# fritzsedlazeck/Sniffles

Hardware: NVIDIA H100
Metric: aligned long-read Gbp/s through lead->cluster->consensus (higher is better)
Workload: dtype int32

## Files before the change

### sniffles_b200/csrc/api.cu

```cuda
#include <algorithm>
#include <climits>
#include <cstdio>
#include <cstdlib>
#include <cstring>
#include <string>
#include <vector>
#include <dlfcn.h>
#include <omp.h>

#include "common.cuh"
#include "prims.cuh"
#include "extract.cuh"
#include "cluster.cuh"
#include "consensus.cuh"
#include "poa.cuh"
#include "combine.cuh"
#include "ingest.cuh"
#include "bgzf_write.cuh"
#include "genotype.cuh"
#include "reference.cuh"

template <bool Pinned> struct Buf {
    void* p = nullptr; size_t cap = 0;
    Buf() = default;
    Buf(const Buf&) = delete; Buf& operator=(const Buf&) = delete;
    ~Buf() { release(); }
    int ensure(size_t bytes) {
        if (bytes <= cap) return 0;
        release();
        size_t want = bytes + bytes / 8 + 256;
        if ((Pinned ? cudaMallocHost(&p, want) : cudaMalloc(&p, want)) != cudaSuccess) { p = nullptr; cudaGetLastError(); return 1; }
        cap = want; return 0;
    }
    template <class T> T* as() { return reinterpret_cast<T*>(p); }
    void reset() { release(); }
private:
    void release() { if (p) { if (Pinned) cudaFreeHost(p); else cudaFree(p); } p = nullptr; cap = 0; }
};
using DevBuf = Buf<false>;
using HostBuf = Buf<true>;
struct Carver {
    uint8_t* base = nullptr; size_t off = 0;
    template <class T> T* take(size_t n) { const size_t o = off; off += (n * sizeof(T) + 255) & ~(size_t)255; return base ? reinterpret_cast<T*>(base + o) : nullptr; }
};
template <bool Pinned, class Lay> static int carve(Buf<Pinned>& buf, Lay&& lay) {
    Carver m; lay(m);
    if (buf.ensure(m.off + 256)) return 1;
    Carver a; a.base = buf.template as<uint8_t>(); lay(a);
    return 0;
}

constexpr int MAX_TIMINGS = 64;

struct Id128 { char b[128]; };
struct NcclApi {
    void* h = nullptr; bool tried = false;
    int (*GetUniqueId)(void*) = nullptr; int (*CommInitRank)(void**, int, Id128, int) = nullptr;
    int (*CommDestroy)(void*) = nullptr; int (*AllGather)(const void*, void*, size_t, int, void*, cudaStream_t) = nullptr; const char* (*GetErrorString)(int) = nullptr;
};
static NcclApi g_nccl;
static bool nccl_load(std::string* err) {
    if (g_nccl.tried) { if (!g_nccl.AllGather && err) *err = "NCCL is not available in this process"; return g_nccl.AllGather != nullptr; }
    g_nccl.tried = true;
    void* h = dlopen(nullptr, RTLD_NOW | RTLD_GLOBAL);
    if (!h || !dlsym(h, "ncclAllGather")) { h = nullptr; const char* names[] = { "libnccl.so.2", "libnccl.so" }; for (const char* n : names) { h = dlopen(n, RTLD_NOW | RTLD_GLOBAL); if (h) break; } }
    if (!h) { if (err) *err = "libnccl.so.2 not found"; return false; }
    g_nccl.h = h;
    g_nccl.GetUniqueId = (int (*)(void*))dlsym(h, "ncclGetUniqueId");
    g_nccl.CommInitRank = (int (*)(void**, int, Id128, int))dlsym(h, "ncclCommInitRank");
    g_nccl.CommDestroy = (int (*)(void*))dlsym(h, "ncclCommDestroy");
    g_nccl.AllGather = (int (*)(const void*, void*, size_t, int, void*, cudaStream_t))dlsym(h, "ncclAllGather");
    g_nccl.GetErrorString = (const char* (*)(int))dlsym(h, "ncclGetErrorString");
    if (!g_nccl.GetUniqueId || !g_nccl.CommInitRank || !g_nccl.CommDestroy || !g_nccl.AllGather) { g_nccl.AllGather = nullptr; if (err) *err = "NCCL symbols missing"; return false; }
    return true;
}

struct Caps { unsigned long long lead = 0, cand = 0, cand_lead = 0, rn = 0, alt = 0, scr16 = 0, item = 0, tile = 0, req = 0, req16 = 0; };

struct snfb_ctx {
    int device = 0; cudaStream_t st = nullptr, st_copy = nullptr, st_side = nullptr; cudaEvent_t ev_b = nullptr, ev_mid = nullptr, ev_fork = nullptr, ev_join = nullptr; std::string err;
    snfb_config cfg{}; bool have_cfg = false;
    bool loaded = false, on_device = false, seq_on_demand = false; const uint8_t* h_seq = nullptr; uint32_t evt_min = 0;
    uint64_t n_rec = 0, n_cigar = 0, n_var = 0, n_seq = 0; uint32_t n_task = 0, n_contig = 0, n_tr = 0, n_mask = 0;
    const snfb_rec* d_rec = nullptr; const uint16_t* d_cigar = nullptr; const uint8_t* d_var = nullptr; const uint8_t* d_seq = nullptr;
    DevBuf b_rec, b_cigar, b_var, b_seq, b_task, b_contig, b_tr, b_trp, b_mask, b_mask_off, b_mask_task;
    HostBuf h_c16, h_rec16;
    DevBuf b_comp, b_raw, b_ing, b_ing_work; HostBuf h_ing; uint64_t ing_sizes[8] = {0, 0, 0, 0, 0, 0, 0, 0}; bool from_bam = false;
    DevBuf b_zin, b_zslot, b_zout, b_zwork;
    DevBuf b_gt;
    DevBuf b_ref, b_ref_work; std::vector<refseq::Contig> ref_ctg; bool have_ref = false;
    HostBuf h_ref_runs, h_ref_coff, h_ref_out; uint64_t ref_n_runs = 0;
    std::vector<snfb_task> tasks;
    Caps cap; bool force_no_cuts = false;
    DevBuf b_ctr, arena_r, arena_l, arena_c;
    int32_t* rec_pos; int32_t* rec_end; uint8_t* rec_flags; double* rec_nm; uint32_t* rec_nlead; uint32_t* rec_lead_off; uint32_t* sa_list; extract::RecScan* scanrec; extract::RecClip* clip; int32_t* rec_big;
    uint32_t* task_first; uint32_t* task_last; uint32_t* task_reads; unsigned long long* task_cov; int32_t* task_span; double* task_nm; double* nm_part; unsigned* nm_cnt; extract::Seg* sa_seg; uint32_t* scan_tmp_r;
    snfb_lead* leads; extract::Event* ev_buf; snfb_lead* sorted_leads; uint32_t* radix_hist;
    cluster::B B{};
    consensus::C Cc{}; consensus::SeqReq* seq_req; uint32_t* arena_off; uint8_t* seq_arena;
    HostBuf h_seq_req, h_seq_arena; uint64_t seq_h2d_bytes = 0;
    bool stage_a_done = false, stage_b_done = false, stage_c_done = false;
    HostBuf h_ctr_buf; DevCounters* h_mid = nullptr; DevCounters* h_fin = nullptr; uint32_t* h_work = nullptr;
    HostBuf h_leads, h_task_reads, h_task_nm, h_rec_nm, h_cand, h_cand_leads, h_rnames, h_rn_off, h_task_cov, h_task_cov_raw, h_alt, h_cov_bins;
    void* comm = nullptr; int rank = 0, nranks = 1; DevBuf b_gsend, b_grecv; HostBuf h_gather, h_gather_out; unsigned long long gather_cap = 0;
    cudaEvent_t ev[MAX_TIMINGS + 1]; const char* ev_name[MAX_TIMINGS + 1]; uint64_t ev_bytes[MAX_TIMINGS + 1]; int n_ev = 0; int n_ev_load = 0; uint64_t launches = 0; uint64_t reruns = 0;
};

static uint32_t evt_need(const snfb_ctx* ctx) {
    if (!ctx->have_cfg) return SNFB_CIGAR16_EVT_MIN;
    int t = ctx->cfg.minsvlen_screen < 1 ? 1 : ctx->cfg.minsvlen_screen;
    if ((ctx->cfg.qc_nm_measure || ctx->cfg.phase) && t > 11) t = 11;
    return (uint32_t)(t < (int)SNFB_CIGAR16_EVT_MIN ? t : (int)SNFB_CIGAR16_EVT_MIN);
}
static void ctx_fail(snfb_ctx* ctx, const char* what, const char* msg) { ctx->err = std::string(what) + ": " + msg; }
static int fail(snfb_ctx* ctx, const std::string& m) { ctx->err = m; return 1; }

static void mark(snfb_ctx* ctx, const char* name, uint64_t bytes = 0) {
    if (ctx->n_ev >= MAX_TIMINGS) return;
    cudaEventRecord(ctx->ev[ctx->n_ev], ctx->st);
    ctx->ev_name[ctx->n_ev] = name; ctx->ev_bytes[ctx->n_ev] = bytes; ++ctx->n_ev;
}
static int grid_for(unsigned long long n, int threads) { unsigned long long g = (n + threads - 1) / threads; if (g < 1) g = 1; if (g > (uint64_t)NUM_SMS * 32) g = (uint64_t)NUM_SMS * 32; return (int)g; }
static int bits_for(uint32_t n) { int b = 0; while ((1ull << b) < n) ++b; return b; }

__global__ void k_gather_leads(const snfb_lead* __restrict__ leads, const uint32_t* __restrict__ sval, snfb_lead* __restrict__ out, const unsigned long long* n_ptr, unsigned long long cap) {
    const unsigned long long n = *n_ptr < cap ? *n_ptr : cap;
    for (unsigned long long i = blockIdx.x * (unsigned long long)blockDim.x + threadIdx.x; i < n; i += (unsigned long long)gridDim.x * blockDim.x) out[i] = leads[sval[i]];
}
__global__ void k_cov_bins(const int32_t* __restrict__ rec_pos, const int32_t* __restrict__ rec_end, const uint8_t* __restrict__ rec_flags, uint32_t lo, uint32_t hi,
                           int binsize, long long contig_len, long long nbins, unsigned long long* __restrict__ acc) {
    for (unsigned long long i = lo + blockIdx.x * (unsigned long long)blockDim.x + threadIdx.x; i < hi; i += (unsigned long long)gridDim.x * blockDim.x) {
        if (!(rec_flags[i] & extract::RF_PASS)) continue;
        long long a = rec_pos[i], e = rec_end[i]; if (a < 0) a = 0; if (e > contig_len) e = contig_len;
        if (e <= a) continue;
        for (long long bb = a / binsize; bb <= (e - 1) / binsize && bb < nbins; ++bb) {
            const long long s0 = bb * binsize, s1 = s0 + binsize;
            const long long o0 = a > s0 ? a : s0, o1 = e < s1 ? e : s1;
            if (o1 > o0) atomicAdd(&acc[bb], (unsigned long long)(o1 - o0));
        }
    }
}


struct GatherHdr { unsigned long long n_cand, n_alt, n_rn, n_leads, need_bytes, overflow, pad0, pad1; };
__host__ __device__ inline void gather_offsets(const GatherHdr& h, unsigned long long off[6]) {
    auto al = [](unsigned long long x) { return (x + 15ull) & ~15ull; };
    off[0] = sizeof(GatherHdr); off[1] = al(off[0] + h.n_cand * sizeof(snfb_cand)); off[2] = al(off[1] + h.n_alt); off[3] = al(off[2] + 8 * h.n_rn);
    off[4] = al(off[3] + 4 * h.n_cand); off[5] = al(off[4] + h.n_leads * sizeof(snfb_lead));
}
__device__ inline void copy16(uint8_t* dst, const uint8_t* src, unsigned long long nbytes) {
    const unsigned long long n16 = (nbytes + 15) >> 4;
    for (unsigned long long i = blockIdx.x * (unsigned long long)blockDim.x + threadIdx.x; i < n16; i += (unsigned long long)gridDim.x * blockDim.x)
        reinterpret_cast<uint4*>(dst)[i] = reinterpret_cast<const uint4*>(src)[i];
}
__global__ void k_gather_pack(const DevCounters* ctr, const snfb_cand* cand, const uint8_t* alt, const uint64_t* rnames, const uint32_t* rn_off, const snfb_lead* leads, int with_leads,
                              uint8_t* slot, unsigned long long cap) {
    GatherHdr h; h.n_cand = ctr->n_cand; h.n_alt = ctr->n_alt_bytes; h.n_rn = ctr->n_rnames; h.n_leads = with_leads ? ctr->n_cand_leads : 0ull; h.pad0 = h.pad1 = 0;
    unsigned long long off[6]; gather_offsets(h, off);
    h.need_bytes = off[5]; h.overflow = off[5] > cap ? 1ull : 0ull;
    if (blockIdx.x == 0 && threadIdx.x == 0) *reinterpret_cast<GatherHdr*>(slot) = h;
    if (h.overflow) return;
    copy16(slot + off[0], reinterpret_cast<const uint8_t*>(cand), h.n_cand * sizeof(snfb_cand));
    copy16(slot + off[1], alt, h.n_alt);
    copy16(slot + off[2], reinterpret_cast<const uint8_t*>(rnames), 8 * h.n_rn);
    copy16(slot + off[3], reinterpret_cast<const uint8_t*>(rn_off), 4 * h.n_cand);
    if (with_leads) copy16(slot + off[4], reinterpret_cast<const uint8_t*>(leads), h.n_leads * sizeof(snfb_lead));
}
__global__ void k_gather_merge(const uint8_t* recv, unsigned long long cap, int nranks, int with_leads, uint8_t* out, unsigned long long out_cap, unsigned long long* out_layout ) {
    GatherHdr tot{}; bool ovf = false;
    for (int r = 0; r < nranks; ++r) { const GatherHdr* h = reinterpret_cast<const GatherHdr*>(recv + (size_t)r * cap); tot.n_cand += h->n_cand; tot.n_alt += h->n_alt; tot.n_rn += h->n_rn; tot.n_leads += h->n_leads; ovf = ovf || h->overflow; }
    auto al = [](unsigned long long x) { return (x + 255ull) & ~255ull; };
    const unsigned long long o_hdr = 0, o_cand = al((unsigned long long)nranks * sizeof(GatherHdr)), o_alt = al(o_cand + tot.n_cand * sizeof(snfb_cand)), o_rn = al(o_alt + tot.n_alt), o_ro = al(o_rn + 8 * tot.n_rn),
                             o_leads = al(o_ro + 4 * (tot.n_cand + 1)), o_end = al(o_leads + tot.n_leads * sizeof(snfb_lead));
    const bool fits = !ovf && o_end <= out_cap;
    if (blockIdx.x == 0 && threadIdx.x == 0) { out_layout[0] = o_cand; out_layout[1] = o_alt; out_layout[2] = o_rn; out_layout[3] = o_ro; out_layout[4] = o_leads; out_layout[5] = o_end; out_layout[6] = fits ? 0 : 1; out_layout[7] = tot.n_cand; }
    if (!fits) return;
    const unsigned long long tid = blockIdx.x * (unsigned long long)blockDim.x + threadIdx.x, nthr = (unsigned long long)gridDim.x * blockDim.x;
    unsigned long long b_cand = 0, b_alt = 0, b_rn = 0, b_leads = 0;
    for (int r = 0; r < nranks; ++r) {
        const uint8_t* slot = recv + (size_t)r * cap; const GatherHdr h = *reinterpret_cast<const GatherHdr*>(slot);
        unsigned long long off[6]; gather_offsets(h, off);
        if (tid == 0) reinterpret_cast<GatherHdr*>(out + o_hdr)[r] = h;
        const snfb_cand* sc = reinterpret_cast<const snfb_cand*>(slot + off[0]); snfb_cand* dc = reinterpret_cast<snfb_cand*>(out + o_cand) + b_cand;
        for (unsigned long long i = tid; i < h.n_cand; i += nthr) { snfb_cand c = sc[i]; if (c.alt_off >= 0) c.alt_off += (int)b_alt; if (with_leads) { c.lead_off += (int)b_leads; c.long_off += (int)b_leads; } dc[i] = c; }
        for (unsigned long long i = tid; i < h.n_alt; i += nthr) (out + o_alt + b_alt)[i] = (slot + off[1])[i];
        const uint64_t* sr = reinterpret_cast<const uint64_t*>(slot + off[2]); uint64_t* dr = reinterpret_cast<uint64_t*>(out + o_rn) + b_rn;
        for (unsigned long long i = tid; i < h.n_rn; i += nthr) dr[i] = sr[i];
        const uint32_t* so = reinterpret_cast<const uint32_t*>(slot + off[3]); uint32_t* dof = reinterpret_cast<uint32_t*>(out + o_ro) + b_cand;
        for (unsigned long long i = tid; i < h.n_cand; i += nthr) dof[i] = so[i] + (uint32_t)b_rn;
        if (with_leads) { const uint4* sl = reinterpret_cast<const uint4*>(slot + off[4]); uint4* dl = reinterpret_cast<uint4*>(out + o_leads) + 4 * b_leads; for (unsigned long long i = tid; i < 4 * h.n_leads; i += nthr) dl[i] = sl[i]; }
        b_cand += h.n_cand; b_alt += h.n_alt; b_rn += h.n_rn; b_leads += h.n_leads;
    }
    if (tid == 0) reinterpret_cast<uint32_t*>(out + o_ro)[tot.n_cand] = (uint32_t)tot.n_rn;
}

static void launch_inflate(snfb_ctx* ctx, const ingest::BgzfBlock* d_blk, unsigned nb, ingest::IngestCounters* d_ctr) {
    const size_t smem = ingest::INF_SMEM_BYTES;
    const unsigned per_block = ingest::INF_WARPS * (32 / ingest::INF_LANES);
    const unsigned resident = (unsigned)std::max<size_t>(1, std::min<size_t>(8, (220 * 1024) / (smem + 1024)));
    const unsigned grid = std::min<unsigned>((nb + per_block - 1) / per_block, (unsigned)NUM_SMS * resident);
    launch(ctx->launches, ingest::k_inflate, grid, ingest::INF_WARPS * 32, smem, ctx->st, ctx->b_comp.as<uint8_t>(), d_blk, nb, ctx->b_raw.as<uint8_t>(), d_ctr);
}

extern "C" {

int snfb_version(void) { return SNFB_ABI_VERSION; }
size_t snfb_sizeof(int which) {
    switch (which) { case 0: return sizeof(snfb_rec); case 1: return sizeof(snfb_task); case 2: return sizeof(snfb_contig); case 3: return sizeof(snfb_records);
                     case 4: return sizeof(snfb_config); case 5: return sizeof(snfb_lead); case 6: return sizeof(snfb_cand); case 7: return sizeof(snfb_gather_view);
                     case 8: return sizeof(snfb_gt_in); case 9: return sizeof(snfb_gt_out);
                     case 10: return sizeof(snfb_ref_contig); case 11: return sizeof(snfb_ref_input); case 12: return sizeof(snfb_ref_query); default: return 0; }
}

uint64_t snfb_hash_name(const char* s, size_t n) {
    uint64_t h = 0xcbf29ce484222325ull; for (size_t i = 0; i < n; ++i) { h ^= (uint8_t)s[i]; h *= 0x100000001b3ull; } return h;
}

int snfb_ctx_create(int device, snfb_ctx** out) {
    if (!out) return 1;
    *out = nullptr;
    int ndev = 0;
    if (cudaGetDeviceCount(&ndev) != cudaSuccess || ndev <= 0 || device < 0 || device >= ndev) return 2;
    if (cudaSetDevice(device) != cudaSuccess) return 3;
    snfb_ctx* ctx = new snfb_ctx();
    ctx->device = device;
    if (cudaStreamCreateWithFlags(&ctx->st, cudaStreamNonBlocking) != cudaSuccess || cudaStreamCreateWithFlags(&ctx->st_copy, cudaStreamNonBlocking) != cudaSuccess
        || cudaStreamCreateWithFlags(&ctx->st_side, cudaStreamNonBlocking) != cudaSuccess) { delete ctx; return 4; }
    cudaEventCreateWithFlags(&ctx->ev_b, cudaEventDisableTiming); cudaEventCreateWithFlags(&ctx->ev_mid, cudaEventDisableTiming);
    cudaEventCreateWithFlags(&ctx->ev_fork, cudaEventDisableTiming); cudaEventCreateWithFlags(&ctx->ev_join, cudaEventDisableTiming);
    for (int i = 0; i <= MAX_TIMINGS; ++i) cudaEventCreate(&ctx->ev[i]);
    if (ctx->h_ctr_buf.ensure(2 * sizeof(DevCounters) + 256) || ctx->b_ctr.ensure(sizeof(DevCounters) + 64)) { delete ctx; return 5; }
    ctx->h_mid = ctx->h_ctr_buf.as<DevCounters>(); ctx->h_fin = ctx->h_mid + 1; ctx->h_work = reinterpret_cast<uint32_t*>(ctx->h_fin + 1);
    memset(ctx->h_ctr_buf.p, 0, 2 * sizeof(DevCounters) + 256);
    cudaFuncSetAttribute(cluster::k_cluster_warp<cluster::SMALL_CAP, cluster::CWS_WARPS, false>, cudaFuncAttributeMaxDynamicSharedMemorySize, (int)cluster::CwCfg<cluster::SMALL_CAP, cluster::CWS_WARPS>::smem);
    cudaFuncSetAttribute(cluster::k_cluster_warp<cluster::WARP_CAP, cluster::CWM_WARPS, true>, cudaFuncAttributeMaxDynamicSharedMemorySize, (int)cluster::CwCfg<cluster::WARP_CAP, cluster::CWM_WARPS>::smem);
    cudaFuncSetAttribute(cluster::k_cluster_block, cudaFuncAttributeMaxDynamicSharedMemorySize, (int)cluster::CB_SMEM);
    cudaFuncSetAttribute(bgzfw::k_deflate, cudaFuncAttributeMaxDynamicSharedMemorySize, (int)bgzfw::DEF_SMEM_BYTES);
    *out = ctx; return 0;
}

void snfb_ctx_destroy(snfb_ctx* ctx) {
    if (!ctx) return;
    cudaSetDevice(ctx->device);
    cudaStreamSynchronize(ctx->st); cudaStreamSynchronize(ctx->st_copy); cudaStreamSynchronize(ctx->st_side);
    if (ctx->comm && g_nccl.CommDestroy) g_nccl.CommDestroy(ctx->comm);
    for (int i = 0; i <= MAX_TIMINGS; ++i) cudaEventDestroy(ctx->ev[i]);
    cudaEventDestroy(ctx->ev_b); cudaEventDestroy(ctx->ev_mid); cudaEventDestroy(ctx->ev_fork); cudaEventDestroy(ctx->ev_join);
    cudaStreamDestroy(ctx->st_side); cudaStreamDestroy(ctx->st_copy); cudaStreamDestroy(ctx->st);
    delete ctx;
}

const char* snfb_last_error(snfb_ctx* ctx) { return ctx ? ctx->err.c_str() : "null context"; }

int snfb_set_config(snfb_ctx* ctx, const snfb_config* cfg) {
    if (!ctx || !cfg) return 1;
    ctx->force_no_cuts = false;
    if (cfg->consensus_kmer_len != 6) return fail(ctx, "consensus_kmer_len must be 6 (the reference fixes it, config.py:550)");
    if (cfg->cluster_binsize <= 0 || cfg->cluster_resplit_binsize <= 0 || cfg->coverage_binsize <= 0) return fail(ctx, "bin sizes must be positive");
    ctx->cfg = *cfg; ctx->have_cfg = true; ctx->stage_a_done = ctx->stage_b_done = ctx->stage_c_done = false; return 0;
}

static bool c16_offsets(const snfb_rec* rec_in, uint64_t n_rec, const uint32_t* cigar32, std::vector<uint64_t>& off) {
    off.assign(n_rec + 1, 0);
    const uint8_t* raw = reinterpret_cast<const uint8_t*>(cigar32);
    bool bad = false;
    #pragma omp parallel for schedule(static) reduction(|| : bad)
    for (long long i = 0; i < (long long)n_rec; ++i) {
        long long ref; int b = 0;
        const uint32_t w = ingest::c16_convert<1>(raw, 4ull * rec_in[i].cigar_off, rec_in[i].n_cigar, nullptr, 0, 0, &ref, &b);
        bad = bad || b; off[i + 1] = (w + 7) & ~7ull;
    }
    if (bad) return false;
    for (uint64_t i = 0; i < n_rec; ++i) off[i + 1] += off[i];
    return true;
}
static void c16_fill(const snfb_rec* rec_in, uint64_t n_rec, const uint32_t* cigar32, const std::vector<uint64_t>& off, snfb_rec* rec_out, uint16_t* out16, uint32_t evt_min) {
    const uint8_t* raw = reinterpret_cast<const uint8_t*>(cigar32);
    #pragma omp parallel for schedule(static)
    for (long long i = 0; i < (long long)n_rec; ++i) {
        uint16_t* dst = out16 + off[i]; const uint64_t span = off[i + 1] - off[i];
        long long ref; int bad = 0;
        const uint64_t k = ingest::c16_convert<1>(raw, 4ull * rec_in[i].cigar_off, rec_in[i].n_cigar, dst, evt_min, 0, &ref, &bad);
        if (k < span) memset(dst + k, 0, 2 * (span - k));
        snfb_rec r = rec_in[i]; r.n_cigar = (uint32_t)k; r.cigar_off = off[i];
        rec_out[i] = r;
    }
    memset(out16 + off[n_rec], 0, 16);
}
uint64_t snfb_pack_cigar16(const snfb_rec* rec_in, uint64_t n_rec, const uint32_t* cigar32, snfb_rec* rec_out, uint16_t* out16, uint64_t out_cap, uint32_t evt_min) {
    if (n_rec && (!rec_in || !cigar32)) return UINT64_MAX;
    if (evt_min == 0) evt_min = SNFB_CIGAR16_EVT_MIN;
    std::vector<uint64_t> off;
    if (!c16_offsets(rec_in, n_rec, cigar32, off)) return UINT64_MAX;
    const uint64_t total = off[n_rec] + 8;
    if (!out16) return total;
    if (!rec_out || out_cap < total) return UINT64_MAX;
    c16_fill(rec_in, n_rec, cigar32, off, rec_out, out16, evt_min);
    return total;
}

static int check_tables(snfb_ctx* ctx, const snfb_records* R) {
    for (uint32_t t = 0; t < R->n_task; ++t) {
        const snfb_task& k = R->task[t];
        if (k.tr_n < 0 || k.tr_off < 0 || (uint64_t)k.tr_off + (uint64_t)k.tr_n > R->n_tr) return fail(ctx, "task table: tandem-repeat range outside tr[]");
        if (R->n_contig && (k.contig < 0 || (uint32_t)k.contig >= R->n_contig)) return fail(ctx, "task table: contig index out of range");
        if (k.contig_len < 0 || k.start > k.end) return fail(ctx, "task table: bad region");
        if ((long long)k.contig_len >= ((long long)1 << 26) * (long long)(ctx->have_cfg ? ctx->cfg.cluster_binsize : 100)) return fail(ctx, "contig too long for the bin field of the sort key (contig_len / cluster_binsize must stay below 2^26)");
    }
    if (R->n_mask && R->mask && R->mask_task_off) {
        for (uint32_t t = 0; t < R->n_task; ++t) if (R->mask_task_off[t] > R->mask_task_off[t + 1] || R->mask_task_off[t + 1] > R->n_mask) return fail(ctx, "mask_task_off must be non-decreasing and end at n_mask");
        for (uint32_t t = 0; t < R->n_task; ++t)
            for (uint32_t m = R->mask_task_off[t]; m < R->mask_task_off[t + 1]; ++m) {
                const uint32_t k = m - R->mask_task_off[t];
                if (R->mask[2 * m] > R->mask[2 * m + 1]) return fail(ctx, "N mask of task " + std::to_string(t) + ": run " + std::to_string(k) + " has start > end");
                if (k && R->mask[2 * m] < R->mask[2 * m - 1]) return fail(ctx, "N mask of task " + std::to_string(t) + ": run " + std::to_string(k) + " starts before run " + std::to_string(k - 1) + " ends (runs must be sorted and disjoint)");
            }
    }
    return 0;
}
static int upload_tables(snfb_ctx* ctx, const snfb_records* R) {
    ctx->tasks.assign(R->task, R->task + R->n_task);
    if (ctx->b_task.ensure(sizeof(snfb_task) * R->n_task) || ctx->b_contig.ensure(sizeof(snfb_contig) * (R->n_contig + 1)) || ctx->b_tr.ensure(8 * ((size_t)R->n_tr + 1)) || ctx->b_trp.ensure(4 * ((size_t)R->n_tr + 1)))
        return fail(ctx, "out of device memory for the task tables");
    CUDA_TRY(cudaMemcpyAsync(ctx->b_task.p, R->task, sizeof(snfb_task) * R->n_task, cudaMemcpyHostToDevice, ctx->st));
    if (R->n_contig) CUDA_TRY(cudaMemcpyAsync(ctx->b_contig.p, R->contig, sizeof(snfb_contig) * R->n_contig, cudaMemcpyHostToDevice, ctx->st));
    if (R->n_tr) {
        std::vector<int32_t> pm(R->n_tr);
        for (uint32_t t = 0; t < R->n_task; ++t) { int32_t m = INT32_MIN; for (int k = 0; k < R->task[t].tr_n; ++k) { const int idx = R->task[t].tr_off + k; if (R->tr[2 * idx + 1] > m) m = R->tr[2 * idx + 1]; pm[idx] = m; } }
        CUDA_TRY(cudaMemcpyAsync(ctx->b_tr.p, R->tr, 8 * (size_t)R->n_tr, cudaMemcpyHostToDevice, ctx->st));
        CUDA_TRY(cudaMemcpyAsync(ctx->b_trp.p, pm.data(), 4 * (size_t)R->n_tr, cudaMemcpyHostToDevice, ctx->st));
        CUDA_TRY(cudaStreamSynchronize(ctx->st));
    }
    ctx->n_mask = (R->mask && R->mask_task_off) ? R->n_mask : 0;
    if (ctx->n_mask) {
        std::vector<uint32_t> mt(ctx->n_mask);
        for (uint32_t t = 0; t < R->n_task; ++t) for (uint32_t m = R->mask_task_off[t]; m < R->mask_task_off[t + 1] && m < ctx->n_mask; ++m) mt[m] = t;
        if (ctx->b_mask.ensure(8 * (size_t)ctx->n_mask) || ctx->b_mask_off.ensure(4 * ((size_t)R->n_task + 1)) || ctx->b_mask_task.ensure(4 * (size_t)ctx->n_mask)) return fail(ctx, "out of device memory (N mask)");
        CUDA_TRY(cudaMemcpyAsync(ctx->b_mask.p, R->mask, 8 * (size_t)ctx->n_mask, cudaMemcpyHostToDevice, ctx->st));
        CUDA_TRY(cudaMemcpyAsync(ctx->b_mask_off.p, R->mask_task_off, 4 * ((size_t)R->n_task + 1), cudaMemcpyHostToDevice, ctx->st));
        CUDA_TRY(cudaMemcpyAsync(ctx->b_mask_task.p, mt.data(), 4 * (size_t)ctx->n_mask, cudaMemcpyHostToDevice, ctx->st));
        CUDA_TRY(cudaStreamSynchronize(ctx->st));
    }
    return 0;
}

int snfb_load_records(snfb_ctx* ctx, const snfb_records* R) {
    if (!ctx || !R) return 1;
    cudaSetDevice(ctx->device);
    ctx->loaded = false; ctx->stage_a_done = ctx->stage_b_done = ctx->stage_c_done = false; ctx->force_no_cuts = false;
    if (R->n_task == 0 || R->n_task > 65535) return fail(ctx, "n_task must be in 1..65535");
    if (R->n_rec >= (1ull << 28)) return fail(ctx, "too many records in one block (2^28)");
    if (!R->task || (R->n_rec && (!R->rec || !R->cigar))) return fail(ctx, "null table in the record block");
    if (check_tables(ctx, R)) return 1;
    ctx->n_rec = R->n_rec; ctx->n_cigar = R->n_cigar; ctx->n_var = R->n_var; ctx->n_seq = R->n_seq;
    ctx->n_task = R->n_task; ctx->n_contig = R->n_contig; ctx->n_tr = R->n_tr; ctx->on_device = R->on_device == SNFB_MEM_DEVICE; ctx->seq_on_demand = R->on_device == SNFB_MEM_HOST_SEQ_ON_DEMAND; ctx->h_seq = ctx->seq_on_demand ? R->seq : nullptr;
    ctx->n_ev = 0;
    const snfb_rec* src_rec = R->rec; const uint16_t* src_cigar = reinterpret_cast<const uint16_t*>(R->cigar); uint64_t n_words = R->n_cigar;
    if (R->cigar_fmt == SNFB_CIGAR_BAM32) {
        if (R->on_device == SNFB_MEM_DEVICE) return fail(ctx, "device-resident records must carry CIGAR16 (convert with snfb_pack_cigar16)");
        for (uint64_t i = 0; i < R->n_rec; ++i) if (R->rec[i].cigar_off + (uint64_t)R->rec[i].n_cigar > R->n_cigar) return fail(ctx, "a record's CIGAR lies outside the cigar arena");
        std::vector<uint64_t> off;
        if (!c16_offsets(R->rec, R->n_rec, reinterpret_cast<const uint32_t*>(R->cigar), off)) return fail(ctx, "a CIGAR holds an operation the path does not know");
        const uint64_t need = off[R->n_rec] + 8;
        if (ctx->h_c16.ensure(2 * need + 16) || ctx->h_rec16.ensure(sizeof(snfb_rec) * (R->n_rec + 1))) return fail(ctx, "out of pinned memory for the CIGAR16 conversion");
        c16_fill(R->rec, R->n_rec, reinterpret_cast<const uint32_t*>(R->cigar), off, ctx->h_rec16.as<snfb_rec>(), ctx->h_c16.as<uint16_t>(), evt_need(ctx));
        src_rec = ctx->h_rec16.as<snfb_rec>(); src_cigar = ctx->h_c16.as<uint16_t>(); n_words = need;
        ctx->evt_min = evt_need(ctx);
    } else if (R->cigar_fmt != SNFB_CIGAR_16) return fail(ctx, "unknown cigar_fmt");
    else ctx->evt_min = R->cigar_evt_min ? R->cigar_evt_min : SNFB_CIGAR16_EVT_MIN;
    if (n_words & 7) return fail(ctx, "a CIGAR16 arena must be padded to a multiple of 8 words");
    ctx->n_cigar = n_words;
    mark(ctx, "h2d_records", sizeof(snfb_rec) * R->n_rec + 2 * n_words + R->n_var + (R->on_device == SNFB_MEM_HOST_SEQ_ON_DEMAND ? 0 : R->n_seq));
    if (ctx->on_device) {
        ctx->d_rec = R->rec; ctx->d_cigar = src_cigar; ctx->d_var = R->var; ctx->d_seq = R->seq;
    } else {
        if (ctx->b_rec.ensure(sizeof(snfb_rec) * (R->n_rec + 1)) || ctx->b_cigar.ensure(2 * (n_words + 16)) || ctx->b_var.ensure(R->n_var + 16) || (!ctx->seq_on_demand && ctx->b_seq.ensure(R->n_seq + 16)))
            return fail(ctx, "out of device memory for the record block");
        CUDA_TRY(cudaMemcpyAsync(ctx->b_rec.p, src_rec, sizeof(snfb_rec) * R->n_rec, cudaMemcpyHostToDevice, ctx->st));
        CUDA_TRY(cudaMemcpyAsync(ctx->b_cigar.p, src_cigar, 2 * n_words, cudaMemcpyHostToDevice, ctx->st));
        CUDA_TRY(cudaMemcpyAsync(ctx->b_var.p, R->var, R->n_var, cudaMemcpyHostToDevice, ctx->st));
        if (!ctx->seq_on_demand) CUDA_TRY(cudaMemcpyAsync(ctx->b_seq.p, R->seq, R->n_seq, cudaMemcpyHostToDevice, ctx->st));
        ctx->d_rec = ctx->b_rec.as<snfb_rec>(); ctx->d_cigar = ctx->b_cigar.as<uint16_t>(); ctx->d_var = ctx->b_var.as<uint8_t>(); ctx->d_seq = ctx->b_seq.as<uint8_t>();
    }
    if (upload_tables(ctx, R)) return 1;
    mark(ctx, nullptr);
    ctx->n_ev_load = ctx->n_ev;
    ctx->loaded = true; return 0;
}


static int walk_bgzf(snfb_ctx* ctx, const uint8_t* z, uint64_t n, std::vector<ingest::BgzfBlock>& blocks, std::vector<uint64_t>& cstart, uint64_t* raw_len) {
    uint64_t o = 0, uo = 0;
    while (o < n) {
        if (o + 18 > n || z[o] != 0x1f || z[o + 1] != 0x8b || z[o + 2] != 8 || !(z[o + 3] & 4)) return fail(ctx, "not a BGZF block (gzip member with an extra field expected)");
        const uint32_t xlen = z[o + 10] | (z[o + 11] << 8);
        if (o + 12 + xlen > n) return fail(ctx, "truncated BGZF header");
        uint32_t bsize = 0; uint64_t e = o + 12; const uint64_t xend = o + 12 + xlen;
        while (e + 4 <= xend) { const uint32_t slen = z[e + 2] | (z[e + 3] << 8); if (z[e] == 66 && z[e + 1] == 67 && slen == 2 && e + 6 <= xend) bsize = (z[e + 4] | (z[e + 5] << 8)) + 1u; e += 4 + slen; }
        if (!bsize || bsize < 12 + xlen + 8 || o + bsize > n) return fail(ctx, "BGZF block without a BC field or truncated");
        ingest::BgzfBlock b; b.in_off = o + 12 + xlen; b.in_len = bsize - 12 - xlen - 8;
        memcpy(&b.crc, z + o + bsize - 8, 4); memcpy(&b.isize, z + o + bsize - 4, 4); b.out_off = uo; b._pad = 0;
        if (b.isize > 65536u) return fail(ctx, "BGZF block claims more than 64 KiB of data");
        blocks.push_back(b); cstart.push_back(o);
        uo += b.isize; o += bsize;
    }
    *raw_len = uo; return 0;
}
static int inflate_to_device(snfb_ctx* ctx, const uint8_t* z, uint64_t n, std::vector<uint64_t>& cstart, std::vector<ingest::BgzfBlock>& blocks, uint64_t* raw_len, const char* h2d_mark = "h2d_bgzf") {
    if (walk_bgzf(ctx, z, n, blocks, cstart, raw_len)) return 1;
    if (*raw_len >= (1ull << 36)) return fail(ctx, "more than 64 GiB of inflated BAM in one ingest call: split the task list");
    if (ctx->b_comp.ensure(n + 64) || ctx->b_raw.ensure(*raw_len + 64)) return fail(ctx, "out of device memory for the BGZF bytes / the inflated stream");
    mark(ctx, h2d_mark, n);
    CUDA_TRY(cudaMemcpyAsync(ctx->b_comp.p, z, n, cudaMemcpyHostToDevice, ctx->st));
    CUDA_TRY(cudaMemsetAsync(ctx->b_comp.as<uint8_t>() + n, 0, 64, ctx->st));
    CUDA_TRY(cudaMemsetAsync(ctx->b_raw.as<uint8_t>() + *raw_len, 0, 64, ctx->st));
    return 0;
}

static int inflate_failed(snfb_ctx* ctx, const ingest::IngestCounters& hc, const std::vector<uint64_t>& cstart) {
    const unsigned long long first = ~hc.first_bad_inv, b = first >> 8, code = first & 255u;
    return fail(ctx, "inflate: " + std::to_string(hc.bad_blocks) + " BGZF block(s) failed to decode (first: block " + std::to_string(b) + ", code " + std::to_string(code)
                     + (code == ingest::INF_CRC_MISMATCH ? ", CRC32 mismatch" : "") + ", at byte " + std::to_string(cstart[b]) + " of the buffer)");
}

int snfb_inflate_bgzf(snfb_ctx* ctx, const uint8_t* bgzf, uint64_t n_bytes, uint8_t* out, uint64_t out_cap, uint64_t* out_len) {
    if (!ctx || !bgzf || !out_len) return 1;
    cudaSetDevice(ctx->device);
    std::vector<ingest::BgzfBlock> blocks; std::vector<uint64_t> cstart; uint64_t raw_len = 0;
    ctx->n_ev = 0;
    if (inflate_to_device(ctx, bgzf, n_bytes, cstart, blocks, &raw_len)) return 1;
    *out_len = raw_len;
    const size_t nb = blocks.size();
    ingest::IngestCounters* d_ctr = nullptr; ingest::BgzfBlock* d_blk = nullptr;
    if (carve(ctx->b_ing, [&](Carver& c) { d_ctr = c.take<ingest::IngestCounters>(1); d_blk = c.take<ingest::BgzfBlock>(nb + 1); })) return fail(ctx, "out of device memory (ingest tables)");
    CUDA_TRY(cudaMemsetAsync(d_ctr, 0, sizeof(ingest::IngestCounters), ctx->st));
    CUDA_TRY(cudaMemcpyAsync(d_blk, blocks.data(), sizeof(ingest::BgzfBlock) * nb, cudaMemcpyHostToDevice, ctx->st));
    mark(ctx, "inflate", n_bytes + raw_len);
    if (nb) launch_inflate(ctx, d_blk, (unsigned)nb, d_ctr);
    mark(ctx, nullptr);
    ingest::IngestCounters hc;
    CUDA_TRY(cudaMemcpyAsync(&hc, d_ctr, sizeof(hc), cudaMemcpyDeviceToHost, ctx->st));
    CUDA_TRY(cudaStreamSynchronize(ctx->st));
    if (hc.bad_blocks) return inflate_failed(ctx, hc, cstart);
    if (out) {
        if (out_cap < raw_len) return fail(ctx, "snfb_inflate_bgzf: output buffer too small");
        CUDA_TRY(cudaMemcpy(out, ctx->b_raw.p, raw_len, cudaMemcpyDeviceToHost));
    }
    return 0;
}

int snfb_deflate_bgzf(snfb_ctx* ctx, const uint8_t* in, uint64_t n_in, uint8_t* out, uint64_t out_cap, uint64_t* out_len, uint64_t* coffset) {
    if (!ctx || !out_len || (n_in && (!in || !out))) return 1;
    cudaSetDevice(ctx->device);
    const uint64_t nb = (n_in + deflate::BLOCK_IN - 1) / deflate::BLOCK_IN;
    if (nb > 65535) return fail(ctx, "snfb_deflate_bgzf: more than 65535 BGZF blocks (~4 GiB) in one call: split the input");
    if (out_cap < nb * deflate::MEMBER_MAX) return fail(ctx, "snfb_deflate_bgzf: out_cap must be at least ceil(n_in / 0xff00) * 65536");
    ctx->n_ev = 0;
    *out_len = 0;
    if (nb == 0) return 0;
    const unsigned grid = (unsigned)std::min<uint64_t>(nb, (uint64_t)NUM_SMS);
    uint32_t *sizes = nullptr, *offs = nullptr, *tmp = nullptr; unsigned long long* total = nullptr; uint16_t* scratch = nullptr;
    auto lay = [&](Carver& c) { sizes = c.take<uint32_t>(nb + 1); offs = c.take<uint32_t>(nb + 1); tmp = c.take<uint32_t>(prims::scan_tmp_elems(nb));
                                total = c.take<unsigned long long>(1); scratch = c.take<uint16_t>(2ull * deflate::BLOCK_IN * grid); };
    if (ctx->b_zin.ensure(n_in + 64) || ctx->b_zslot.ensure(nb * deflate::MEMBER_MAX) || ctx->b_zout.ensure(nb * deflate::MEMBER_MAX) || carve(ctx->b_zwork, lay))
        return fail(ctx, "out of device memory (BGZF compression)");
    cudaStream_t st = ctx->st;
    mark(ctx, "h2d_deflate", n_in);
    CUDA_TRY(cudaMemcpyAsync(ctx->b_zin.p, in, n_in, cudaMemcpyHostToDevice, st));
    mark(ctx, "deflate", n_in);
    launch(ctx->launches, bgzfw::k_deflate, grid, bgzfw::DEF_THREADS, bgzfw::DEF_SMEM_BYTES, st, ctx->b_zin.as<const uint8_t>(), (unsigned long long)n_in, (unsigned)nb, scratch,
           ctx->b_zslot.as<uint8_t>(), sizes);
    prims::exclusive_scan(ctx->launches, sizes, offs, tmp, nullptr, nb, total, st);
    launch(ctx->launches, bgzfw::k_pack, (unsigned)std::min<uint64_t>(nb, (uint64_t)NUM_SMS * 16), 256, 0, st, ctx->b_zslot.as<const uint8_t>(), sizes, offs, (unsigned)nb, ctx->b_zout.as<uint8_t>());
    mark(ctx, "d2h_deflate", 0);
    unsigned long long n_out = 0;
    std::vector<uint32_t> h_offs(nb);
    CUDA_TRY(cudaMemcpyAsync(&n_out, total, sizeof(n_out), cudaMemcpyDeviceToHost, st));
    CUDA_TRY(cudaMemcpyAsync(h_offs.data(), offs, 4 * nb, cudaMemcpyDeviceToHost, st));
    CUDA_TRY(cudaStreamSynchronize(st));
    CUDA_TRY(cudaMemcpyAsync(out, ctx->b_zout.p, n_out, cudaMemcpyDeviceToHost, st));
    mark(ctx, nullptr);
    CUDA_TRY(cudaStreamSynchronize(st));
    CUDA_TRY(cudaGetLastError());
    if (coffset) for (uint64_t k = 0; k < nb; ++k) coffset[k] = h_offs[k];
    *out_len = n_out;
    return 0;
}

int snfb_load_bam(snfb_ctx* ctx, const snfb_bam_input* in) {
    if (!ctx || !in) return 1;
    cudaSetDevice(ctx->device);
    ctx->loaded = false; ctx->from_bam = false; ctx->stage_a_done = ctx->stage_b_done = ctx->stage_c_done = false; ctx->force_no_cuts = false;
    if (in->n_task == 0 || in->n_task > 65535) return fail(ctx, "n_task must be in 1..65535");
    if (!in->task || (in->n_bytes && !in->bgzf) || (in->n_span && !in->span)) return fail(ctx, "null table in the BAM input");
    snfb_records T; memset(&T, 0, sizeof(T));
    T.n_task = in->n_task; T.n_contig = in->n_contig; T.n_tr = in->n_tr; T.n_mask = in->n_mask; T.task = in->task; T.contig = in->contig; T.tr = in->tr; T.mask = in->mask; T.mask_task_off = in->mask_task_off;
    if (check_tables(ctx, &T)) return 1;
    ctx->n_ev = 0;
    std::vector<ingest::BgzfBlock> blocks; std::vector<uint64_t> cstart; uint64_t raw_len = 0;
    if (inflate_to_device(ctx, in->bgzf, in->n_bytes, cstart, blocks, &raw_len)) return 1;
    const size_t nb = blocks.size(); const uint64_t ns = in->n_span;
    std::vector<ingest::Span> spans(ns);
    for (uint64_t i = 0; i < ns; ++i) {
        const snfb_bam_span& sp = in->span[i];
        if (sp.task >= in->n_task) return fail(ctx, "span: task index out of range");
        auto resolve = [&](uint64_t c, uint32_t u, uint64_t* out) -> bool {
            if (c == in->n_bytes) { *out = raw_len; return u == 0; }
            auto it = std::lower_bound(cstart.begin(), cstart.end(), c);
            if (it == cstart.end() || *it != c) return false;
            const ingest::BgzfBlock& b = blocks[(size_t)(it - cstart.begin())];
            if (u > b.isize) return false;
            *out = b.out_off + u; return true;
        };
        uint64_t ub = 0, ue = 0;
        if (!resolve(sp.cbeg, sp.ubeg, &ub) || !resolve(sp.cend, sp.uend, &ue) || ue < ub) return fail(ctx, "span: a virtual offset does not name a BGZF block of the buffer");
        if (i && spans[i - 1].task > sp.task) return fail(ctx, "spans must be listed task by task");
        if (i && spans[i - 1].task == sp.task && spans[i - 1].uend > ub) return fail(ctx, "spans of a task must be in file order and must not overlap");
        spans[i].ubeg = ub; spans[i].uend = ue; spans[i].task = sp.task; spans[i]._pad = 0;
    }
    if (upload_tables(ctx, &T)) return 1;
    ingest::IngestCounters* d_ctr = nullptr; ingest::BgzfBlock* d_blk = nullptr; ingest::Span* d_span = nullptr; uint32_t* span_cnt = nullptr; uint32_t* span_base = nullptr; uint32_t* scan_tmp0 = nullptr;
    if (carve(ctx->b_ing, [&](Carver& c) { d_ctr = c.take<ingest::IngestCounters>(1); d_blk = c.take<ingest::BgzfBlock>(nb + 1); d_span = c.take<ingest::Span>(ns + 1); span_cnt = c.take<uint32_t>(ns + 1);
                                           span_base = c.take<uint32_t>(ns + 1); scan_tmp0 = c.take<uint32_t>(prims::scan_tmp_elems(ns + 1) + 16); }))
        return fail(ctx, "out of device memory (ingest tables)");
    cudaStream_t st = ctx->st; const uint8_t* raw = ctx->b_raw.as<uint8_t>();
    CUDA_TRY(cudaMemsetAsync(d_ctr, 0, sizeof(ingest::IngestCounters), st));
    CUDA_TRY(cudaMemcpyAsync(d_blk, blocks.data(), sizeof(ingest::BgzfBlock) * nb, cudaMemcpyHostToDevice, st));
    if (ns) CUDA_TRY(cudaMemcpyAsync(d_span, spans.data(), sizeof(ingest::Span) * ns, cudaMemcpyHostToDevice, st));
    mark(ctx, "inflate", in->n_bytes + raw_len);
    if (nb) launch_inflate(ctx, d_blk, (unsigned)nb, d_ctr);
    mark(ctx, "walk_records", 0);
    if (ns) {
        launch(ctx->launches, ingest::k_walk, (unsigned)((ns + 127) / 128), 128, 0, st, raw, raw_len, d_span, (unsigned)ns, 0, span_cnt, nullptr, nullptr, 0, d_ctr);
        prims::exclusive_scan(ctx->launches, span_cnt, span_base, scan_tmp0, nullptr, ns, &d_ctr->n_raw, st);
    }
    if (ctx->h_ing.ensure(2 * sizeof(ingest::IngestCounters))) return fail(ctx, "out of pinned memory");
    ingest::IngestCounters* hc = ctx->h_ing.as<ingest::IngestCounters>();
    CUDA_TRY(cudaMemcpyAsync(hc, d_ctr, sizeof(*hc), cudaMemcpyDeviceToHost, st));
    CUDA_TRY(cudaStreamSynchronize(st));
    if (hc->bad_blocks) return inflate_failed(ctx, *hc, cstart);
    if (hc->bad_chain) return fail(ctx, "BAM record chain broken in " + std::to_string(hc->bad_chain) + " span(s): a span does not start or end on a record boundary, or the data is truncated");
    const uint64_t n_raw = hc->n_raw;
    if (n_raw >= (1ull << 28)) return fail(ctx, "too many records in one block (2^28)");
    ingest::RawRec* recs = nullptr; uint32_t *keep = nullptr, *idx = nullptr, *groups = nullptr, *grp_off = nullptr, *var16 = nullptr, *var_off = nullptr, *seq16 = nullptr, *seq_off = nullptr, *scan_tmp = nullptr;
    if (carve(ctx->b_ing_work, [&](Carver& c) { recs = c.take<ingest::RawRec>(n_raw + 1); keep = c.take<uint32_t>(n_raw + 1); idx = c.take<uint32_t>(n_raw + 1); groups = c.take<uint32_t>(n_raw + 1); grp_off = c.take<uint32_t>(n_raw + 1);
                                                var16 = c.take<uint32_t>(n_raw + 1); var_off = c.take<uint32_t>(n_raw + 1); seq16 = c.take<uint32_t>(n_raw + 1); seq_off = c.take<uint32_t>(n_raw + 1); scan_tmp = c.take<uint32_t>(prims::scan_tmp_elems(n_raw + 1) + 16); }))
        return fail(ctx, "out of device memory (ingest work arrays)");
    const uint32_t evt = evt_need(ctx);
    uint64_t n_rec = 0, n_groups = 0, n_var16 = 0, n_seq16 = 0;
    if (n_raw) {
        const unsigned warp_grid = (unsigned)std::min<uint64_t>((n_raw + 7) / 8, (uint64_t)NUM_SMS * 16);
        launch(ctx->launches, ingest::k_walk, (unsigned)((ns + 127) / 128), 128, 0, st, raw, raw_len, d_span, (unsigned)ns, 1, span_cnt, span_base, recs, n_raw, d_ctr);
        mark(ctx, "parse_records", 0);
        launch(ctx->launches, ingest::k_parse, (unsigned)((n_raw + 127) / 128), 128, 0, st, raw, recs, (unsigned)n_raw, ctx->b_task.as<snfb_task>(), d_ctr);
        mark(ctx, "record_sizes", 0);
        launch(ctx->launches, ingest::k_rec_sizes, warp_grid, 256, 0, st, raw, recs, (unsigned)n_raw, ctx->b_task.as<snfb_task>(), evt, keep, groups, var16, seq16, d_ctr);
        prims::exclusive_scan(ctx->launches, keep, idx, scan_tmp, nullptr, n_raw, &d_ctr->n_keep, st);
        prims::exclusive_scan(ctx->launches, groups, grp_off, scan_tmp, nullptr, n_raw, &d_ctr->n_groups, st);
        prims::exclusive_scan(ctx->launches, var16, var_off, scan_tmp, nullptr, n_raw, &d_ctr->n_var, st);
        prims::exclusive_scan(ctx->launches, seq16, seq_off, scan_tmp, nullptr, n_raw, &d_ctr->n_seq16, st);
        CUDA_TRY(cudaMemcpyAsync(hc, d_ctr, sizeof(*hc), cudaMemcpyDeviceToHost, st));
        CUDA_TRY(cudaStreamSynchronize(st));
        if (hc->malformed || hc->bad_cigar) return fail(ctx, std::to_string(hc->malformed) + " malformed BAM record(s), " + std::to_string(hc->bad_cigar) + " with a CIGAR operation the path does not know");
        n_rec = hc->n_keep; n_groups = hc->n_groups; n_var16 = hc->n_var; n_seq16 = hc->n_seq16;
    }
    const uint64_t n_words = 8 * n_groups + 8;
    if (ctx->b_rec.ensure(sizeof(snfb_rec) * (n_rec + 1)) || ctx->b_cigar.ensure(2 * (n_words + 16)) || ctx->b_var.ensure(16 * n_var16 + 16) || ctx->b_seq.ensure(16 * n_seq16 + 16))
        return fail(ctx, "out of device memory for the record block");
    mark(ctx, "pack_records", sizeof(snfb_rec) * n_rec + 2 * n_words + 16 * n_var16 + 16 * n_seq16);
    CUDA_TRY(cudaMemsetAsync(ctx->b_cigar.as<uint16_t>() + 8 * n_groups, 0, 2 * 24, st));
    if (n_raw) {
        const unsigned warp_grid = (unsigned)std::min<uint64_t>((n_raw + 7) / 8, (uint64_t)NUM_SMS * 16);
        launch(ctx->launches, ingest::k_pack, warp_grid, 256, 0, st, raw, recs, (unsigned)n_raw, evt, keep, idx, grp_off, groups, var_off, seq_off, ctx->b_rec.as<snfb_rec>(), ctx->b_cigar.as<uint16_t>(), ctx->b_var.as<uint8_t>(), ctx->b_seq.as<uint8_t>());
    }
    mark(ctx, nullptr);
    ctx->n_ev_load = ctx->n_ev;
    ctx->n_rec = n_rec; ctx->n_cigar = n_words; ctx->n_var = 16 * n_var16; ctx->n_seq = 16 * n_seq16; ctx->n_task = in->n_task; ctx->n_contig = in->n_contig; ctx->n_tr = in->n_tr;
    ctx->on_device = false; ctx->seq_on_demand = false; ctx->h_seq = nullptr; ctx->evt_min = evt;
    ctx->d_rec = ctx->b_rec.as<snfb_rec>(); ctx->d_cigar = ctx->b_cigar.as<uint16_t>(); ctx->d_var = ctx->b_var.as<uint8_t>(); ctx->d_seq = ctx->b_seq.as<uint8_t>();
    ctx->ing_sizes[0] = n_rec; ctx->ing_sizes[1] = n_words; ctx->ing_sizes[2] = 16 * n_var16; ctx->ing_sizes[3] = 16 * n_seq16; ctx->ing_sizes[4] = n_raw; ctx->ing_sizes[5] = nb; ctx->ing_sizes[6] = raw_len; ctx->ing_sizes[7] = in->n_bytes;
    CUDA_TRY(cudaStreamSynchronize(st));
    ctx->loaded = true; ctx->from_bam = true; return 0;
}

int snfb_ingest_sizes(snfb_ctx* ctx, uint64_t out[8]) {
    if (!ctx || !out || !ctx->from_bam) return 1;
    for (int i = 0; i < 8; ++i) out[i] = ctx->ing_sizes[i];
    return 0;
}
int snfb_ingest_fetch(snfb_ctx* ctx, snfb_rec* rec, uint16_t* cigar16, uint8_t* var, uint8_t* seq) {
    if (!ctx || !ctx->from_bam || !ctx->loaded) return ctx ? fail(ctx, "snfb_ingest_fetch: no block built by snfb_load_bam") : 1;
    cudaSetDevice(ctx->device);
    if (rec && ctx->n_rec) CUDA_TRY(cudaMemcpy(rec, ctx->d_rec, sizeof(snfb_rec) * ctx->n_rec, cudaMemcpyDeviceToHost));
    if (cigar16 && ctx->n_cigar) CUDA_TRY(cudaMemcpy(cigar16, ctx->d_cigar, 2 * ctx->n_cigar, cudaMemcpyDeviceToHost));
    if (var && ctx->n_var) CUDA_TRY(cudaMemcpy(var, ctx->d_var, ctx->n_var, cudaMemcpyDeviceToHost));
    if (seq && ctx->n_seq) CUDA_TRY(cudaMemcpy(seq, ctx->d_seq, ctx->n_seq, cudaMemcpyDeviceToHost));
    return 0;
}

}

static void carve_r(snfb_ctx* ctx, Carver& c) {
    const size_t n = ctx->n_rec + 1, nt = ctx->n_task;
    ctx->rec_pos = c.take<int32_t>(n); ctx->rec_end = c.take<int32_t>(n); ctx->rec_flags = c.take<uint8_t>(n); ctx->rec_nm = c.take<double>(n); ctx->rec_nlead = c.take<uint32_t>(n); ctx->rec_lead_off = c.take<uint32_t>(n);
    ctx->sa_list = c.take<uint32_t>(n); ctx->scanrec = c.take<extract::RecScan>(n); ctx->clip = c.take<extract::RecClip>(n); ctx->rec_big = c.take<int32_t>(n);
    ctx->task_first = c.take<uint32_t>(nt); ctx->task_last = c.take<uint32_t>(nt); ctx->task_reads = c.take<uint32_t>(nt); ctx->task_cov = c.take<unsigned long long>(nt); ctx->task_span = c.take<int32_t>(nt); ctx->task_nm = c.take<double>(nt);
    const size_t cpt = (ctx->n_rec + extract::NM_CHUNK - 1) / extract::NM_CHUNK + 1;
    ctx->nm_part = c.take<double>(cpt * nt + 1); ctx->nm_cnt = c.take<unsigned>(cpt * nt + 1);
    ctx->sa_seg = c.take<extract::Seg>((size_t)extract::MAXSEG * extract::SA_THREADS * extract::SA_BLOCKS);
    ctx->scan_tmp_r = c.take<uint32_t>(prims::scan_tmp_elems(n) + 16);
}
static void carve_l(snfb_ctx* ctx, Carver& c) {
    const size_t n = (size_t)ctx->cap.lead + 8; cluster::B& b = ctx->B;
    ctx->leads = c.take<snfb_lead>(n); ctx->ev_buf = c.take<extract::Event>(n); ctx->sorted_leads = c.take<snfb_lead>(n);
    b.key0 = c.take<uint64_t>(n); b.val0 = c.take<uint32_t>(n); b.key1 = c.take<uint64_t>(n); b.val1 = c.take<uint32_t>(n); b.flag = c.take<uint32_t>(n); b.scan = c.take<uint32_t>(n);
    b.scan_tmp = c.take<uint32_t>(prims::scan_tmp_elems(std::max<unsigned long long>(n, prims::radix_hist_elems(n))) + 16);
    ctx->radix_hist = c.take<uint32_t>(prims::radix_hist_elems(n) + 16);
    b.bin_start = c.take<uint32_t>(n); b.bin_nl = c.take<uint32_t>(n); b.bin_nlong = c.take<uint32_t>(n); b.bin_kept = c.take<uint32_t>(n); b.bin_hap = c.take<uint32_t>(3 * n);
    b.kl_off = c.take<uint32_t>(n); b.kll_off = c.take<uint32_t>(n); b.kb_idx = c.take<uint32_t>(n); b.kl = c.take<uint32_t>(n); b.kll = c.take<uint32_t>(n); b.kleads = c.take<snfb_lead>(n); b.klleads = c.take<snfb_lead>(n);
    b.kb_bin = c.take<uint32_t>(n); b.kb_lead_off = c.take<uint32_t>(n); b.kb_lead_n = c.take<uint32_t>(n); b.kb_long_off = c.take<uint32_t>(n); b.kb_long_n = c.take<uint32_t>(n); b.kb_seed = c.take<int32_t>(n); b.kb_chain = c.take<uint32_t>(n); b.kb_repeat = c.take<uint8_t>(n);
    b.seg_start = c.take<uint32_t>(n); b.c_next = c.take<uint32_t>(n); b.c_last = c.take<uint32_t>(n); b.c_sd = c.take<double>(n); b.c_mean = c.take<double>(n); b.c_rep = c.take<uint8_t>(n);
    b.seg_sd_last = c.take<double>(n); b.seg_maxsd_first = c.take<double>(n); b.cl_first = c.take<uint32_t>(n); b.cl_last = c.take<uint32_t>(n); b.cl_rep = c.take<uint8_t>(n); b.big_list = c.take<uint32_t>(n); b.mid_list = c.take<uint32_t>(n);
    b.g_khi = c.take<uint64_t>(n); b.g_klo = c.take<uint64_t>(n); b.g_u32 = c.take<uint32_t>((size_t)cluster::coop::NU32 * n);
    b.ord = c.take<uint32_t>(n); b.st_leads = c.take<snfb_lead>(n); b.st_plo = c.take<uint32_t>(n); b.st_pn = c.take<uint32_t>(n); b.st_rn = c.take<uint64_t>(n); b.cand_tmp = c.take<snfb_cand>(n); b.sub_valid = c.take<uint8_t>(n);
    b.cl_nsub = c.take<uint32_t>(n); b.cl_nvalid = c.take<uint32_t>(n); b.cl_nlead = c.take<uint32_t>(n); b.cl_nrn = c.take<uint32_t>(n); b.cl_cand_base = c.take<uint32_t>(n); b.cl_lead_base = c.take<uint32_t>(n); b.cl_rn_base = c.take<uint32_t>(n);
    ctx->arena_off = c.take<uint32_t>(n);
}
static void carve_c(snfb_ctx* ctx, Carver& c) {
    const Caps& k = ctx->cap; cluster::B& b = ctx->B; consensus::C& cc = ctx->Cc;
    b.cand = c.take<snfb_cand>(k.cand + 1); b.cand_leads = c.take<snfb_lead>(k.cand_lead + 1); b.out_plo = c.take<uint32_t>(k.cand_lead + 1); b.out_pn = c.take<uint32_t>(k.cand_lead + 1);
    b.rnames = c.take<uint64_t>(k.rn + 1); b.rn_off_out = c.take<uint32_t>(k.cand + 2);
    cc.plan_best = c.take<uint32_t>(k.cand + 1); cc.plan_nother = c.take<uint32_t>(k.cand + 1); cc.plan_otot = c.take<uint32_t>(k.cand + 1); cc.alt_len = c.take<uint32_t>(k.cand + 1); cc.scr_len = c.take<uint32_t>(k.cand + 1);
    cc.alt_off = c.take<uint32_t>(k.cand + 1); cc.scr_off = c.take<uint32_t>(k.cand + 1); cc.work_big = c.take<uint32_t>(k.cand + 1); cc.work_small = c.take<uint32_t>(k.cand + 1); cc.work_ctr = c.take<uint32_t>(64);
    cc.items_big = c.take<consensus::C::Item>(k.item + 1); cc.items_small = c.take<consensus::C::Item>(k.item + 1); cc.tiles = c.take<uint2>(k.tile + 1);
    cc.alt = c.take<uint8_t>(k.alt + 64); cc.scr = c.take<uint8_t>(k.scr16 * 16 + 64);
    ctx->seq_req = c.take<consensus::SeqReq>(k.req + 1); ctx->seq_arena = c.take<uint8_t>(k.req16 * 16 + 64);
}
static int ensure_arenas(snfb_ctx* ctx) {
    if (carve(ctx->arena_r, [&](Carver& c) { carve_r(ctx, c); })) return fail(ctx, "out of device memory (per-record arrays)");
    if (carve(ctx->arena_l, [&](Carver& c) { carve_l(ctx, c); })) return fail(ctx, "out of device memory (per-lead arrays)");
    if (carve(ctx->arena_c, [&](Carver& c) { carve_c(ctx, c); })) return fail(ctx, "out of device memory (candidate / consensus arrays)");
    return 0;
}

static void bind_inputs(snfb_ctx* ctx) {
    cluster::B& b = ctx->B;
    b.leads = ctx->leads; b.rec = ctx->d_rec; b.task = ctx->b_task.as<snfb_task>(); b.contig = ctx->b_contig.as<snfb_contig>();
    b.tr = ctx->n_tr ? ctx->b_tr.as<int32_t>() : nullptr; b.tr_pmax = ctx->b_trp.as<int32_t>();
    b.rec_pos = ctx->rec_pos; b.rec_end = ctx->rec_end; b.rec_flags = ctx->rec_flags; b.rec_nm = ctx->rec_nm; b.rec_nlead = ctx->rec_nlead; b.rec_lead_off = ctx->rec_lead_off;
    b.task_first = ctx->task_first; b.task_last = ctx->task_last; b.task_maxspan = ctx->task_span;
    b.mask = ctx->n_mask ? ctx->b_mask.as<int32_t>() : nullptr; b.mask_task_off = ctx->n_mask ? ctx->b_mask_off.as<uint32_t>() : nullptr;
    b.n_task = ctx->n_task; b.n_bound = ctx->cap.lead; b.ctr = ctx->b_ctr.as<DevCounters>(); b.cfg = ctx->cfg;
    b.cut_gap = ctx->force_no_cuts ? INT_MAX : cluster::break_gap(ctx->cfg);
    b.cand_cap = ctx->cap.cand; b.cand_lead_cap = ctx->cap.cand_lead; b.rn_cap = ctx->cap.rn;
    consensus::C& c = ctx->Cc;
    c.cand = b.cand; c.cand_rw = b.cand; c.cand_leads = b.cand_leads; c.out_plo = b.out_plo; c.out_pn = b.out_pn; c.ord = b.ord; c.kleads = b.kleads; c.rec = ctx->d_rec; c.seq = ctx->d_seq; c.arena_off = nullptr;
    c.cand_cap = ctx->cap.cand; c.ctr = b.ctr; c.cfg = ctx->cfg; c.item_cap = ctx->cap.item; c.tile_cap = ctx->cap.tile; c.alt_cap = ctx->cap.alt; c.scr_cap16 = ctx->cap.scr16;
}

static int enqueue_stage_a(snfb_ctx* ctx) {
    const uint64_t nrec = ctx->n_rec; const uint32_t nt = ctx->n_task; const snfb_config& cf = ctx->cfg; cluster::B& b = ctx->B;
    DevCounters* ctr = b.ctr; cudaStream_t st = ctx->st;
    CUDA_TRY(cudaMemsetAsync(ctr, 0, sizeof(DevCounters), st));
    CUDA_TRY(cudaMemsetAsync(ctx->task_first, 0, 4 * nt, st)); CUDA_TRY(cudaMemsetAsync(ctx->task_last, 0, 4 * nt, st));
    CUDA_TRY(cudaMemsetAsync(ctx->task_reads, 0, 4 * nt, st)); CUDA_TRY(cudaMemsetAsync(ctx->task_cov, 0, 8 * nt, st)); CUDA_TRY(cudaMemsetAsync(ctx->task_span, 0, 4 * nt, st));
    CUDA_TRY(cudaMemsetAsync(ctx->task_nm, 0, 8 * nt, st));
    extract::WalkParams S{};
    S.scan = ctx->scanrec; S.n_rec = (uint32_t)nrec; S.cigar = ctx->d_cigar; S.task = b.task;
    S.rec_end = ctx->rec_end; S.rec_nlead = ctx->rec_nlead; S.rec_big = ctx->rec_big;
    S.ev = ctx->ev_buf; S.ev_cap = ctx->cap.lead; S.n_ev = &ctr->n_ev; S.ctr = ctr; S.minsv = cf.minsvlen_screen;
    if (evt_need(ctx) < ctx->evt_min) {
        if (ctx->on_device) return fail(ctx, "the device-resident CIGAR16 arena was packed with a larger event length than the configuration needs: repack with snfb_pack_cigar16(evt_min)");
        launch(ctx->launches, extract::k_reflag, NUM_SMS * 8, 256, 0, st, const_cast<uint16_t*>(ctx->d_cigar), ctx->n_cigar, evt_need(ctx));
        ctx->evt_min = evt_need(ctx);
    }
    mark(ctx, "k_rec_index");
    if (nrec) {
        extract::IndexParams I{};
        I.rec = ctx->d_rec; I.cigar = ctx->d_cigar; I.task = b.task; I.n_rec = (uint32_t)nrec; I.n_task = nt; I.rec_pos = ctx->rec_pos; I.task_first = ctx->task_first; I.task_last = ctx->task_last;
        I.scan = ctx->scanrec; I.clip = ctx->clip; I.rec_end = ctx->rec_end; I.rec_flags = ctx->rec_flags; I.rec_nm = ctx->rec_nm; I.rec_nlead = ctx->rec_nlead; I.ctr = ctr;
        I.mapq_min = cf.mapq; I.alen_min = cf.min_alignment_length; I.excl = cf.exclude_flags; I.want_nm = (cf.qc_nm_measure || cf.phase) ? 1 : 0;
        I.n_cigar = ctx->n_cigar; I.n_var = ctx->n_var; I.n_seq = ctx->n_seq; I.check_seq = ctx->seq_on_demand ? 0 : 1;
        I.sa_list = ctx->sa_list; I.n_sa = &ctr->n_sa;
        launch(ctx->launches, extract::k_rec_index, (unsigned)((nrec + 255) / 256), 256, 0, st, I);
        mark(ctx, "k_scan", 2 * ctx->n_cigar);
        if (nrec >= extract::WALK_WIDE_MIN) launch(ctx->launches, extract::k_cigar_walk<32>, extract::WALK_BLOCKS, extract::WALK_THREADS, 0, st, S);
        else launch(ctx->launches, extract::k_cigar_walk<1>, extract::WALK_BLOCKS, extract::WALK_THREADS, 0, st, S);
        mark(ctx, "k_rec_post");
        extract::PostParams Q{};
        Q.scan = I.scan; Q.clip = I.clip; Q.task = b.task; Q.n_rec = (uint32_t)nrec; Q.rec_end = ctx->rec_end; Q.rec_big = ctx->rec_big; Q.rec_nm = ctx->rec_nm;
        Q.task_reads = ctx->task_reads; Q.task_cov_bp = ctx->task_cov; Q.task_maxspan = ctx->task_span;
        launch(ctx->launches, extract::k_rec_post, (unsigned)((nrec + 255) / 256), 256, 0, st, Q);
        mark(ctx, "k_emit");
        extract::EmitParams E{};
        E.rec = ctx->d_rec; E.clip = ctx->clip; E.var = ctx->d_var; E.ev = S.ev; E.n_ev = S.n_ev; E.ev_cap = ctx->cap.lead;
        E.leads = ctx->leads; E.ctr = ctr; E.maxlen = cf.dev_seq_cache_maxlen; E.detect_large_ins = cf.detect_large_ins; E.longinslen = (double)cf.long_ins_length / 2.0;
        launch(ctx->launches, extract::k_emit, NUM_SMS * 16, 128, 0, st, E);
        mark(ctx, "k_sa");
        extract::SaParams A{};
        A.rec = ctx->d_rec; A.clip = ctx->clip; A.var = ctx->d_var; A.task = b.task; A.contig = b.contig; A.n_contig = ctx->n_contig;
        A.sa_list = ctx->sa_list; A.n_sa = &ctr->n_sa; A.rec_end = ctx->rec_end; A.rec_nlead = ctx->rec_nlead; A.leads = E.leads; A.lead_cap = ctx->cap.lead; A.ctr = ctr; A.cfg = cf; A.seg_scratch = ctx->sa_seg;
        launch(ctx->launches, extract::k_sa, extract::SA_BLOCKS, extract::SA_THREADS, 0, st, A);
        mark(ctx, "k_task_nm");
        const int cpt = (int)((nrec + extract::NM_CHUNK - 1) / extract::NM_CHUNK);
        launch(ctx->launches, extract::k_nm_partial, dim3(cpt, nt), 256, 0, st, ctx->rec_flags, ctx->rec_nm, ctx->task_first, ctx->task_last, ctx->nm_part, ctx->nm_cnt);
        launch(ctx->launches, extract::k_task_nm, nt, 256, 0, st, ctx->task_first, ctx->task_last, ctx->nm_part, ctx->nm_cnt, cpt, ctx->task_nm);
    }
    mark(ctx, "scan_rec_leads");
    prims::exclusive_scan(ctx->launches, ctx->rec_nlead, ctx->rec_lead_off, ctx->scan_tmp_r, nullptr, nrec, &ctr->n_leads, st);
    const unsigned long long nb = b.n_bound; const int g = grid_for(nb, 256);
    mark(ctx, "sort_leads");
    launch(ctx->launches, cluster::k_scatter_keys, g, 256, 0, st, b);
    prims::RadixTemp rt{ ctx->radix_hist, b.scan_tmp };
    bool first = true;
    prims::radix_sort(ctx->launches, b.key0, b.val0, b.key1, b.val1, rt, &ctr->n_leads, nb, cluster::TASK_SHIFT + bits_for(ctx->n_task), &first, st);
    b.skey = first ? b.key0 : b.key1; b.sval = first ? b.val0 : b.val1;
    mark(ctx, "bins");
    launch(ctx->launches, cluster::k_bin_heads, g, 256, 0, st, b);
    prims::exclusive_scan(ctx->launches, b.flag, b.scan, b.scan_tmp, &ctr->n_leads, nb, &ctr->n_bins, st);
    launch(ctx->launches, cluster::k_bin_build, g, 256, 0, st, b);
    launch(ctx->launches, cluster::k_bin_stats, g, 256, 0, st, b);
    mark(ctx, nullptr);
    CUDA_TRY(cudaGetLastError());
    return 0;
}

static int enqueue_stage_b(snfb_ctx* ctx) {
    cluster::B& b = ctx->B; DevCounters* ctr = b.ctr; cudaStream_t st = ctx->st;
    const unsigned long long nb = b.n_bound; const int g = grid_for(nb, 128);
    mark(ctx, "kept_bins");
    prims::exclusive_scan(ctx->launches, b.bin_nl, b.kl_off, b.scan_tmp, &ctr->n_bins, nb, &ctr->n_kl, st);
    prims::exclusive_scan(ctx->launches, b.bin_nlong, b.kll_off, b.scan_tmp, &ctr->n_bins, nb, &ctr->n_kll, st);
    prims::exclusive_scan(ctx->launches, b.bin_kept, b.kb_idx, b.scan_tmp, &ctr->n_bins, nb, &ctr->n_kbins, st);
    launch(ctx->launches, cluster::k_kbin_build, g, 128, 0, st, b);
    launch(ctx->launches, cluster::k_gather_kept, grid_for(nb, 256), 256, 0, st, b);
    mark(ctx, "merge_chains");
    launch(ctx->launches, cluster::k_seg_heads, g, 128, 0, st, b);
    prims::exclusive_scan(ctx->launches, b.flag, b.scan, b.scan_tmp, &ctr->n_kbins, nb, &ctr->n_segs, st);
    launch(ctx->launches, cluster::k_seg_build, g, 128, 0, st, b);
    launch(ctx->launches, cluster::k_merge, g, 128, 0, st, b);
    launch(ctx->launches, cluster::k_verify_cuts, g, 128, 0, st, b);
    prims::exclusive_scan(ctx->launches, b.flag, b.scan, b.scan_tmp, &ctr->n_kbins, nb, &ctr->n_clusters, st);
    launch(ctx->launches, cluster::k_cluster_build, g, 128, 0, st, b);
    mark(ctx, "cluster_call");
    CUDA_TRY(cudaEventRecord(ctx->ev_fork, st)); CUDA_TRY(cudaStreamWaitEvent(ctx->st_side, ctx->ev_fork, 0));
    launch(ctx->launches, cluster::k_cluster_block, NUM_SMS, cluster::CB_THREADS, cluster::CB_SMEM, ctx->st_side, b);
    launch(ctx->launches, cluster::k_cluster_warp<cluster::WARP_CAP, cluster::CWM_WARPS, true>, NUM_SMS * 2, cluster::CWM_WARPS * 32, cluster::CwCfg<cluster::WARP_CAP, cluster::CWM_WARPS>::smem, ctx->st_side, b);
    CUDA_TRY(cudaEventRecord(ctx->ev_join, ctx->st_side));
    launch(ctx->launches, cluster::k_cluster_warp<cluster::SMALL_CAP, cluster::CWS_WARPS, false>, NUM_SMS * 4, cluster::CWS_WARPS * 32, cluster::CwCfg<cluster::SMALL_CAP, cluster::CWS_WARPS>::smem, st, b);
    CUDA_TRY(cudaStreamWaitEvent(st, ctx->ev_join, 0));
    mark(ctx, "emit_cands");
    prims::exclusive_scan(ctx->launches, b.cl_nvalid, b.cl_cand_base, b.scan_tmp, &ctr->n_clusters, nb, &ctr->n_cand, st);
    prims::exclusive_scan(ctx->launches, b.cl_nlead, b.cl_lead_base, b.scan_tmp, &ctr->n_clusters, nb, &ctr->n_cand_leads, st);
    prims::exclusive_scan(ctx->launches, b.cl_nrn, b.cl_rn_base, b.scan_tmp, &ctr->n_clusters, nb, &ctr->n_rnames, st);
    launch(ctx->launches, cluster::k_emit_cands, NUM_SMS * 8, 128, 0, st, b);
    mark(ctx, "coverage");
    if (ctx->n_mask) launch(ctx->launches, cluster::k_mask_bp, grid_for((unsigned long long)ctx->n_mask * 32, 128), 128, 0, st, b, ctx->b_mask_task.as<uint32_t>(), ctx->n_mask, ctx->task_cov);
    launch(ctx->launches, cluster::k_coverage, NUM_SMS * 32, 128, 0, st, b);
    consensus::C& c = ctx->Cc;
    CUDA_TRY(cudaMemsetAsync(c.work_ctr, 0, 64, st));
    mark(ctx, "consensus_plan");
    launch(ctx->launches, consensus::k_plan, grid_for(ctx->cap.cand, 128), 128, 0, st, c);
    prims::exclusive_scan(ctx->launches, c.alt_len, c.alt_off, b.scan_tmp, &ctr->n_cand, ctx->cap.cand, &ctr->n_alt_bytes, st);
    prims::exclusive_scan(ctx->launches, c.scr_len, c.scr_off, b.scan_tmp, &ctr->n_cand, ctx->cap.cand, &ctr->n_seq_bytes, st);
    launch(ctx->launches, consensus::k_plan_finish, grid_for(ctx->cap.cand, 128), 128, 0, st, c);
    mark(ctx, nullptr);
    CUDA_TRY(cudaGetLastError());
    return 0;
}

static int enqueue_stage_c(snfb_ctx* ctx) {
    cluster::B& b = ctx->B; consensus::C& c = ctx->Cc; DevCounters* ctr = b.ctr; cudaStream_t st = ctx->st;
    c.seq = ctx->d_seq; c.arena_off = nullptr; ctx->seq_h2d_bytes = 0;
    if (ctx->seq_on_demand) {
        mark(ctx, "seq_requests");
        launch(ctx->launches, consensus::k_seq_requests, grid_for(ctx->cap.cand, 128), 128, 0, st, c, ctx->seq_req, ctx->cap.req, ctx->arena_off, &ctr->n_req, &ctr->n_req_units);
        mark(ctx, nullptr);
        CUDA_TRY(cudaMemcpyAsync(ctx->h_fin, ctr, sizeof(DevCounters), cudaMemcpyDeviceToHost, st));
        CUDA_TRY(cudaStreamSynchronize(st));
        const unsigned long long nreq = ctx->h_fin->n_req, nunits = ctx->h_fin->n_req_units;
        if (nreq <= ctx->cap.req && nunits <= ctx->cap.req16 && nreq) {
            if (ctx->h_seq_req.ensure(sizeof(consensus::SeqReq) * (nreq + 1)) || ctx->h_seq_arena.ensure(nunits * 16 + 64)) return fail(ctx, "out of pinned memory (seq arena)");
            CUDA_TRY(cudaMemcpyAsync(ctx->h_seq_req.p, ctx->seq_req, sizeof(consensus::SeqReq) * nreq, cudaMemcpyDeviceToHost, st));
            CUDA_TRY(cudaStreamSynchronize(st));
            const consensus::SeqReq* rq = ctx->h_seq_req.as<consensus::SeqReq>(); uint8_t* dst = ctx->h_seq_arena.as<uint8_t>(); const uint8_t* src = ctx->h_seq; const uint64_t nseq = ctx->n_seq;
            #pragma omp parallel for schedule(static, 256)
            for (long long i = 0; i < (long long)nreq; ++i) {
                unsigned long long s0 = rq[i].src; unsigned long long nbytes = rq[i].nbytes; if (s0 > nseq) s0 = nseq; if (s0 + nbytes > nseq) nbytes = nseq - s0;
                memcpy(dst + (size_t)rq[i].dst16 * 16, src + s0, (size_t)nbytes);
            }
            mark(ctx, "h2d_seq_slices", nunits * 16);
            CUDA_TRY(cudaMemcpyAsync(ctx->seq_arena, ctx->h_seq_arena.p, nunits * 16, cudaMemcpyHostToDevice, st));
            mark(ctx, nullptr);
            ctx->seq_h2d_bytes = nunits * 16;
        }
        c.seq = ctx->seq_arena; c.arena_off = ctx->arena_off;
    }
    mark(ctx, "consensus");
    launch(ctx->launches, consensus::k_prep, NUM_SMS * 8, 128, 0, st, c);
    mark(ctx, "consensus_align");
    launch(ctx->launches, consensus::k_align, NUM_SMS * 7, consensus::ALIGN_WARPS * 32, 0, st, c);
    mark(ctx, "consensus_vote");
    launch(ctx->launches, consensus::k_vote, NUM_SMS * 16, consensus::VOTE_THREADS, 0, st, c);
    mark(ctx, nullptr);
    CUDA_TRY(cudaGetLastError());
    return 0;
}

static void initial_caps(snfb_ctx* ctx) {
    Caps& k = ctx->cap;
    const unsigned long long nrec = ctx->n_rec;
    const unsigned long long lead = std::max<unsigned long long>(1ull << 16, nrec) + (unsigned long long)extract::WALK_BLOCKS * (extract::WALK_THREADS / 32) * extract::WALK_SLOTS
                                    + (unsigned long long)extract::SA_BLOCKS * extract::SA_THREADS * extract::SLOT_CHUNK / 4;
    if (k.lead < lead) k.lead = lead;
    if (k.cand < k.lead / 8 + 1024) k.cand = k.lead / 8 + 1024;
    if (k.cand_lead < k.lead / 2 + 1024) k.cand_lead = k.lead / 2 + 1024;
    if (k.rn < k.lead / 2 + 1024) k.rn = k.lead / 2 + 1024;
    if (k.alt < (4ull << 20)) k.alt = 4ull << 20;
    if (k.scr16 < (2ull << 20)) k.scr16 = 2ull << 20;
    if (k.item < k.cand_lead / 2 + 1024) k.item = k.cand_lead / 2 + 1024;
    if (k.tile < k.cand + 4096) k.tile = k.cand + 4096;
    if (ctx->seq_on_demand) { if (k.req < k.cand_lead / 2 + 1024) k.req = k.cand_lead / 2 + 1024; if (k.req16 < (1ull << 20)) k.req16 = 1ull << 20; }
    else { if (k.req < 16) k.req = 16; if (k.req16 < 16) k.req16 = 16; }
}
static unsigned long long grown(unsigned long long need) { return need + need / 4 + 1024; }
static bool caps_fit(snfb_ctx* ctx, const DevCounters& c, const uint32_t* work, int upto) {
    Caps& k = ctx->cap; bool ok = true;
    const unsigned long long need_lead = std::max(c.n_slots, c.n_leads);
    if (need_lead > k.lead || c.lead_overflow) { k.lead = std::max(grown(need_lead), k.lead + k.lead / 2); ok = false; }
    if (upto >= 2) {
        if (c.n_cand > k.cand) { k.cand = grown(c.n_cand); ok = false; }
        if (c.n_cand_leads > k.cand_lead) { k.cand_lead = grown(c.n_cand_leads); ok = false; }
        if (c.n_rnames > k.rn) { k.rn = grown(c.n_rnames); ok = false; }
        if (c.n_alt_bytes > k.alt) { k.alt = grown(c.n_alt_bytes); ok = false; }
        if (c.n_seq_bytes > k.scr16) { k.scr16 = grown(c.n_seq_bytes); ok = false; }
        const unsigned long long items = std::max(work[4], work[5]);
        if (items > k.item) { k.item = grown(items); ok = false; }
        if (work[8] > k.tile) { k.tile = grown(work[8]); ok = false; }
    }
    if (upto >= 3) {
        if (c.n_req > k.req) { k.req = grown(c.n_req); ok = false; }
        if (c.n_req_units > k.req16) { k.req16 = grown(c.n_req_units); ok = false; }
        if (ok && c.scratch_overflow) { ok = false; k.alt = grown(k.alt); k.scr16 = grown(k.scr16); }
    } else if (ok && c.scratch_overflow) { ok = false; k.cand_lead = grown(k.cand_lead); k.rn = grown(k.rn); }
    return ok;
}

static int fill_lead_view(snfb_ctx* ctx, snfb_lead_view* out) {
    const DevCounters& c = *ctx->h_fin; const unsigned long long nl = c.n_leads; const uint32_t nt = ctx->n_task;
    if (ctx->h_leads.ensure(sizeof(snfb_lead) * (nl + 1)) || ctx->h_task_reads.ensure(4 * nt) || ctx->h_task_nm.ensure(8 * nt) || ctx->h_rec_nm.ensure(8 * (ctx->n_rec + 1)))
        return fail(ctx, "out of memory for the lead view");
    if (nl) {
        launch(ctx->launches, k_gather_leads, grid_for(nl, 256), 256, 0, ctx->st, ctx->leads, ctx->B.sval, ctx->sorted_leads, &ctx->B.ctr->n_leads, ctx->cap.lead);
        CUDA_TRY(cudaMemcpyAsync(ctx->h_leads.p, ctx->sorted_leads, sizeof(snfb_lead) * nl, cudaMemcpyDeviceToHost, ctx->st));
    }
    CUDA_TRY(cudaMemcpyAsync(ctx->h_task_reads.p, ctx->task_reads, 4 * nt, cudaMemcpyDeviceToHost, ctx->st));
    CUDA_TRY(cudaMemcpyAsync(ctx->h_task_nm.p, ctx->task_nm, 8 * nt, cudaMemcpyDeviceToHost, ctx->st));
    if (ctx->n_rec) CUDA_TRY(cudaMemcpyAsync(ctx->h_rec_nm.p, ctx->rec_nm, 8 * ctx->n_rec, cudaMemcpyDeviceToHost, ctx->st));
    CUDA_TRY(cudaStreamSynchronize(ctx->st));
    out->n_leads = nl; out->leads = ctx->h_leads.as<snfb_lead>();
    out->task_read_count = ctx->h_task_reads.as<uint32_t>(); out->task_mean_nm = ctx->h_task_nm.as<double>(); out->rec_nm = ctx->h_rec_nm.as<double>();
    uint64_t np = 0; for (uint32_t t = 0; t < nt; ++t) np += out->task_read_count[t];
    out->n_pass = np; out->soft_errors = c.soft_errors;
    return 0;
}
static int enqueue_cand_copies(snfb_ctx* ctx, const DevCounters& c, cudaStream_t stream) {
    cluster::B& b = ctx->B; const uint32_t nt = ctx->n_task;
    if (ctx->h_cand.ensure(sizeof(snfb_cand) * (c.n_cand + 1)) || ctx->h_cand_leads.ensure(sizeof(snfb_lead) * (c.n_cand_leads + 1)) || ctx->h_rnames.ensure(8 * (c.n_rnames + 1)) || ctx->h_rn_off.ensure(4 * (c.n_cand + 2))
        || ctx->h_task_cov.ensure(8 * nt) || ctx->h_task_cov_raw.ensure(8 * nt)) return fail(ctx, "out of pinned memory for the candidate view");
    if (c.n_cand) { CUDA_TRY(cudaMemcpyAsync(ctx->h_cand.p, b.cand, sizeof(snfb_cand) * c.n_cand, cudaMemcpyDeviceToHost, stream)); CUDA_TRY(cudaMemcpyAsync(ctx->h_rn_off.p, b.rn_off_out, 4 * c.n_cand, cudaMemcpyDeviceToHost, stream)); }
    if (c.n_cand_leads) CUDA_TRY(cudaMemcpyAsync(ctx->h_cand_leads.p, b.cand_leads, sizeof(snfb_lead) * c.n_cand_leads, cudaMemcpyDeviceToHost, stream));
    if (c.n_rnames) CUDA_TRY(cudaMemcpyAsync(ctx->h_rnames.p, b.rnames, 8 * c.n_rnames, cudaMemcpyDeviceToHost, stream));
    CUDA_TRY(cudaMemcpyAsync(ctx->h_task_cov_raw.p, ctx->task_cov, 8 * nt, cudaMemcpyDeviceToHost, stream));
    return 0;
}
static void finish_cand_view(snfb_ctx* ctx, const DevCounters& c, snfb_cand_view* out) {
    const uint32_t nt = ctx->n_task;
    ctx->h_rn_off.as<uint32_t>()[c.n_cand] = (uint32_t)c.n_rnames;
    double* cm = ctx->h_task_cov.as<double>(); const unsigned long long* cov = ctx->h_task_cov_raw.as<unsigned long long>();
    for (uint32_t t = 0; t < nt; ++t) cm[t] = ctx->tasks[t].contig_len > 0 ? (double)cov[t] / (double)ctx->tasks[t].contig_len : 0.0;
    out->n_cand = c.n_cand; out->cand = ctx->h_cand.as<snfb_cand>(); out->n_cand_leads = c.n_cand_leads; out->cand_leads = ctx->h_cand_leads.as<snfb_lead>();
    out->rnames = ctx->h_rnames.as<uint64_t>(); out->rnames_off = ctx->h_rn_off.as<uint32_t>(); out->task_coverage_mean = cm; out->unverified_breaks = c.unverified_breaks;
}

static const char* fatal_counter(const DevCounters& c) {
    if (c.bad_records) return "the record block is malformed: a record points outside its task table or arenas";
    if (c.unsorted) return "records are not coordinate sorted inside a task";
    if (c.ordinal_overflow) return "a read carries more than 65535 SV signatures (16-bit lead ordinal)";
    return nullptr;
}
static int run_pipeline(snfb_ctx* ctx, int upto, snfb_lead_view* leads, snfb_cand_view* cands, snfb_seq_view* seqs) {
    if (!ctx->loaded) return fail(ctx, "no records loaded");
    if (!ctx->have_cfg) return fail(ctx, "snfb_set_config was not called");
    cudaSetDevice(ctx->device);
    for (uint32_t t = 0; t < ctx->n_task; ++t) if ((long long)ctx->tasks[t].contig_len / ctx->cfg.cluster_binsize >= (1ll << 26)) return fail(ctx, "contig_len / cluster_binsize must stay below 2^26 (bin field of the sort key)");
    initial_caps(ctx);
    ctx->stage_a_done = ctx->stage_b_done = ctx->stage_c_done = false;
    for (int attempt = 0; ; ++attempt) {
        if (attempt == 6) return fail(ctx, "buffer capacities did not converge");
        if (ensure_arenas(ctx)) return 1;
        bind_inputs(ctx);
        ctx->n_ev = ctx->n_ev_load;
        cudaStream_t st = ctx->st; DevCounters* ctr = ctx->B.ctr;
        if (enqueue_stage_a(ctx)) return 1;
        bool mid = false, copies = false;
        if (upto >= 2) {
            if (enqueue_stage_b(ctx)) return 1;
            CUDA_TRY(cudaEventRecord(ctx->ev_b, st)); CUDA_TRY(cudaStreamWaitEvent(ctx->st_copy, ctx->ev_b, 0));
            CUDA_TRY(cudaMemcpyAsync(ctx->h_mid, ctr, sizeof(DevCounters), cudaMemcpyDeviceToHost, ctx->st_copy));
            CUDA_TRY(cudaMemcpyAsync(ctx->h_work, ctx->Cc.work_ctr, 64, cudaMemcpyDeviceToHost, ctx->st_copy));
            CUDA_TRY(cudaEventRecord(ctx->ev_mid, ctx->st_copy));
            mid = true;
        }
        if (upto >= 3 && !ctx->seq_on_demand) { if (enqueue_stage_c(ctx)) return 1; }
        if (mid) {
            CUDA_TRY(cudaEventSynchronize(ctx->ev_mid));
            if (const char* m = fatal_counter(*ctx->h_mid)) { cudaStreamSynchronize(st); return fail(ctx, m); }
            if (!caps_fit(ctx, *ctx->h_mid, ctx->h_work, 2)) { CUDA_TRY(cudaStreamSynchronize(st)); ++ctx->reruns; continue; }
            if (ctx->h_mid->unverified_breaks && !ctx->force_no_cuts) { CUDA_TRY(cudaStreamSynchronize(st)); ctx->force_no_cuts = true; ++ctx->reruns; continue; }
            if (cands) { if (enqueue_cand_copies(ctx, *ctx->h_mid, ctx->st_copy)) return 1; copies = true; }
            if (upto >= 3 && ctx->seq_on_demand) { if (enqueue_stage_c(ctx)) return 1; }
        }
        if (upto >= 3 && seqs) {
            const unsigned long long na = ctx->h_mid->n_alt_bytes;
            if (ctx->h_alt.ensure(na + 16)) return fail(ctx, "out of pinned memory for the ALT arena");
            if (na) CUDA_TRY(cudaMemcpyAsync(ctx->h_alt.p, ctx->Cc.alt, na, cudaMemcpyDeviceToHost, st));
        }
        CUDA_TRY(cudaMemcpyAsync(ctx->h_fin, ctr, sizeof(DevCounters), cudaMemcpyDeviceToHost, st));
        CUDA_TRY(cudaMemcpyAsync(ctx->h_work + 16, ctx->Cc.work_ctr, 64, cudaMemcpyDeviceToHost, st));
        CUDA_TRY(cudaStreamSynchronize(st));
        if (copies) CUDA_TRY(cudaStreamSynchronize(ctx->st_copy));
        CUDA_TRY(cudaGetLastError());
        if (const char* m = fatal_counter(*ctx->h_fin)) return fail(ctx, m);
        if (!caps_fit(ctx, *ctx->h_fin, upto >= 2 ? ctx->h_work + 16 : ctx->h_work, upto)) { ++ctx->reruns; continue; }
        break;
    }
    ctx->stage_a_done = true; ctx->stage_b_done = upto >= 2; ctx->stage_c_done = upto >= 3;
    if (leads) { memset(leads, 0, sizeof *leads); if (fill_lead_view(ctx, leads)) return 1; }
    if (cands) { memset(cands, 0, sizeof *cands); finish_cand_view(ctx, *ctx->h_fin, cands); }
    if (seqs) { memset(seqs, 0, sizeof *seqs); seqs->n_alt_bytes = ctx->h_fin->n_alt_bytes; seqs->alt = ctx->h_alt.as<uint8_t>(); }
    return 0;
}

extern "C" {

int snfb_extract_leads(snfb_ctx* ctx, snfb_lead_view* out) {
    if (!ctx) return 1;
    return run_pipeline(ctx, 1, out, nullptr, nullptr);
}
int snfb_cluster_call(snfb_ctx* ctx, snfb_cand_view* out) {
    if (!ctx) return 1;
    if (!ctx->stage_a_done) return fail(ctx, "snfb_extract_leads must run first");
    return run_pipeline(ctx, 2, nullptr, out, nullptr);
}
int snfb_consensus(snfb_ctx* ctx, snfb_seq_view* out) {
    if (!ctx) return 1;
    if (!ctx->stage_b_done) return fail(ctx, "snfb_cluster_call must run first");
    snfb_seq_view tmp; return run_pipeline(ctx, 3, nullptr, nullptr, out ? out : &tmp);
}
int snfb_run(snfb_ctx* ctx, snfb_lead_view* leads, snfb_cand_view* cands, snfb_seq_view* seqs) {
    if (!ctx) return 1;
    snfb_seq_view tmp; return run_pipeline(ctx, 3, leads, cands, seqs ? seqs : &tmp);
}

int snfb_last_timings(snfb_ctx* ctx, const char** names, float* ms, uint64_t* bytes, int cap) {
    if (!ctx) return 0;
    cudaSetDevice(ctx->device);
    cudaStreamSynchronize(ctx->st);
    int n = 0;
    for (int i = 0; i + 1 < ctx->n_ev && n < cap; ++i) {
        if (!ctx->ev_name[i]) continue;
        float t = 0; if (cudaEventElapsedTime(&t, ctx->ev[i], ctx->ev[i + 1]) != cudaSuccess) t = -1.f;
        names[n] = ctx->ev_name[i]; ms[n] = t; if (bytes) bytes[n] = ctx->ev_bytes[i]; ++n;
    }
    if (ctx->n_ev - ctx->n_ev_load >= 2 && n < cap) {
        float t = 0; if (cudaEventElapsedTime(&t, ctx->ev[ctx->n_ev_load], ctx->ev[ctx->n_ev - 1]) != cudaSuccess) t = -1.f;
        names[n] = "total"; ms[n] = t; if (bytes) bytes[n] = 0; ++n;
    }
    return n;
}

int snfb_device_candidates(snfb_ctx* ctx, void** dptr, uint64_t* n_cand) {
    if (!ctx || !ctx->stage_b_done) return 1;
    if (dptr) *dptr = ctx->B.cand; if (n_cand) *n_cand = ctx->h_fin->n_cand; return 0;
}
int snfb_device_alt(snfb_ctx* ctx, void** dptr, uint64_t* n_bytes) {
    if (!ctx || !ctx->stage_c_done) return 1;
    if (dptr) *dptr = ctx->Cc.alt; if (n_bytes) *n_bytes = ctx->h_fin->n_alt_bytes; return 0;
}
uint64_t snfb_launch_count(snfb_ctx* ctx) { return ctx ? ctx->launches : 0; }
double snfb_selftest_sqrt_frac(uint64_t p_hi, uint64_t p_lo, uint64_t q, int slow) { const u128 P = ((u128)p_hi << 64) | p_lo; return slow ? sqrt_frac_rn_slow(P, q) : sqrt_frac_rn(P, q); }
uint64_t snfb_rerun_count(snfb_ctx* ctx) { return ctx ? ctx->reruns : 0; }
int snfb_pin_host(void* p, size_t bytes) { return cudaHostRegister(p, bytes, cudaHostRegisterDefault) == cudaSuccess ? 0 : 1; }
int snfb_unpin_host(void* p) { return cudaHostUnregister(p) == cudaSuccess ? 0 : 1; }

int snfb_nccl_unique_id(void* out128) {
    std::string e; if (!out128 || !nccl_load(&e)) return 1;
    Id128 id; memset(&id, 0, sizeof id);
    if (g_nccl.GetUniqueId(&id) != 0) return 2;
    memcpy(out128, &id, 128); return 0;
}
int snfb_comm_init(snfb_ctx* ctx, const void* unique_id128, int rank, int nranks) {
    if (!ctx || !unique_id128 || nranks < 1 || rank < 0 || rank >= nranks) return 1;
    std::string e; if (!nccl_load(&e)) return fail(ctx, "NCCL: " + e);
    cudaSetDevice(ctx->device);
    if (ctx->comm) { g_nccl.CommDestroy(ctx->comm); ctx->comm = nullptr; }
    Id128 id; memcpy(&id, unique_id128, 128);
    const int rc = g_nccl.CommInitRank(&ctx->comm, nranks, id, rank);
    if (rc != 0) { ctx->comm = nullptr; return fail(ctx, std::string("ncclCommInitRank: ") + (g_nccl.GetErrorString ? g_nccl.GetErrorString(rc) : "error")); }
    ctx->rank = rank; ctx->nranks = nranks; ctx->gather_cap = 0; return 0;
}
int snfb_allgather_candidates(snfb_ctx* ctx, uint32_t flags, snfb_gather_view* out) {
    if (!ctx || !out) return 1;
    if (!ctx->stage_c_done) return fail(ctx, "snfb_run must run first");
    if (ctx->nranks > 1 && !ctx->comm) return fail(ctx, "snfb_comm_init was not called");
    cudaSetDevice(ctx->device);
    const int nr = ctx->nranks, with_leads = (flags & SNFB_GATHER_LEADS) ? 1 : 0; cudaStream_t st = ctx->st; cluster::B& b = ctx->B;
    memset(out, 0, sizeof *out);
    unsigned long long* h_layout = nullptr; GatherHdr* h_hdr = nullptr; uint64_t* rank_n = nullptr;
    if (carve(ctx->h_gather, [&](Carver& c) { h_layout = c.take<unsigned long long>(8); h_hdr = c.take<GatherHdr>(nr); rank_n = c.take<uint64_t>(nr); })) return fail(ctx, "out of pinned memory (gather)");
    for (int attempt = 0; attempt < 4; ++attempt) {
        if (ctx->gather_cap == 0) {
            const DevCounters& c = *ctx->h_fin; GatherHdr h{}; h.n_cand = c.n_cand; h.n_alt = c.n_alt_bytes; h.n_rn = c.n_rnames; h.n_leads = with_leads ? c.n_cand_leads : 0;
            unsigned long long off[6]; gather_offsets(h, off);
            unsigned long long mx = off[5];
            if (nr > 1) {
                if (ctx->b_gsend.ensure(256) || ctx->b_grecv.ensure(8 * (size_t)nr + 256)) return fail(ctx, "out of device memory (gather)");
                CUDA_TRY(cudaMemcpyAsync(ctx->b_gsend.p, &off[5], 8, cudaMemcpyHostToDevice, st));
                if (g_nccl.AllGather(ctx->b_gsend.p, ctx->b_grecv.p, 8, 0 , ctx->comm, st) != 0) return fail(ctx, "ncclAllGather (sizes) failed");
                std::vector<unsigned long long> all(nr);
                CUDA_TRY(cudaMemcpyAsync(all.data(), ctx->b_grecv.p, 8 * (size_t)nr, cudaMemcpyDeviceToHost, st)); CUDA_TRY(cudaStreamSynchronize(st));
                for (int r = 0; r < nr; ++r) mx = std::max(mx, all[r]);
            }
            ctx->gather_cap = (grown(mx) + 255ull) & ~255ull;
        }
        const unsigned long long cap = ctx->gather_cap, out_cap = (unsigned long long)nr * cap + 4096ull * 8;
        uint8_t* recv = nullptr; uint8_t* merged = nullptr; unsigned long long* d_layout = nullptr;
        if (ctx->b_gsend.ensure(cap + 256) || carve(ctx->b_grecv, [&](Carver& c) { recv = c.take<uint8_t>((size_t)nr * cap); merged = c.take<uint8_t>(out_cap); d_layout = c.take<unsigned long long>(8); }))
            return fail(ctx, "out of device memory (gather)");
        mark(ctx, "allgather");
        launch(ctx->launches, k_gather_pack, NUM_SMS * 4, 256, 0, st, b.ctr, b.cand, ctx->Cc.alt, b.rnames, b.rn_off_out, b.cand_leads, with_leads, nr > 1 ? ctx->b_gsend.as<uint8_t>() : recv, cap);
        if (nr > 1 && g_nccl.AllGather(ctx->b_gsend.p, recv, cap, 0 , ctx->comm, st) != 0) return fail(ctx, "ncclAllGather failed");
        launch(ctx->launches, k_gather_merge, NUM_SMS * 4, 256, 0, st, recv, cap, nr, with_leads, merged, out_cap, d_layout);
        mark(ctx, nullptr);
        CUDA_TRY(cudaMemcpyAsync(h_layout, d_layout, 64, cudaMemcpyDeviceToHost, st));
        CUDA_TRY(cudaMemcpyAsync(h_hdr, recv, sizeof(GatherHdr), cudaMemcpyDeviceToHost, st));
        for (int r = 1; r < nr; ++r) CUDA_TRY(cudaMemcpyAsync(h_hdr + r, recv + (size_t)r * cap, sizeof(GatherHdr), cudaMemcpyDeviceToHost, st));
        CUDA_TRY(cudaStreamSynchronize(st));
        unsigned long long mx = 0; for (int r = 0; r < nr; ++r) mx = std::max(mx, h_hdr[r].need_bytes);
        if (h_layout[6]) { ctx->gather_cap = (grown(mx) + 255ull) & ~255ull; ++ctx->reruns; continue; }
        if (grown(mx) > cap) ctx->gather_cap = (grown(mx) + 255ull) & ~255ull;
        GatherHdr tot{}; for (int r = 0; r < nr; ++r) { tot.n_cand += h_hdr[r].n_cand; tot.n_alt += h_hdr[r].n_alt; tot.n_rn += h_hdr[r].n_rn; tot.n_leads += h_hdr[r].n_leads; }
        for (int r = 0; r < nr; ++r) rank_n[r] = h_hdr[r].n_cand;
        out->n_cand = tot.n_cand; out->n_alt_bytes = tot.n_alt; out->n_rnames = tot.n_rn; out->n_cand_leads = tot.n_leads; out->rank_n_cand = rank_n;
        out->dev_buffer = merged; out->dev_bytes_per_rank = cap;
        if (!(flags & SNFB_GATHER_DEVICE_ONLY)) {
            const unsigned long long total = h_layout[5];
            if (ctx->h_gather_out.ensure(total)) return fail(ctx, "out of pinned memory (gather result)");
            uint8_t* hm = ctx->h_gather_out.as<uint8_t>();
            CUDA_TRY(cudaMemcpyAsync(hm, merged, total, cudaMemcpyDeviceToHost, st)); CUDA_TRY(cudaStreamSynchronize(st));
            out->cand = reinterpret_cast<const snfb_cand*>(hm + h_layout[0]); out->alt = hm + h_layout[1]; out->rnames = reinterpret_cast<const uint64_t*>(hm + h_layout[2]);
            out->rnames_off = reinterpret_cast<const uint32_t*>(hm + h_layout[3]); out->cand_leads = with_leads ? reinterpret_cast<const snfb_lead*>(hm + h_layout[4]) : nullptr;
        }
        return 0;
    }
    return fail(ctx, "gather buffer sizes did not converge");
}

int snfb_poa(snfb_ctx* ctx, const snfb_poa_job* jobs, uint32_t n_jobs, const uint8_t* seqs, uint64_t n_seq_bytes, const int32_t* offs, uint64_t n_offs, uint8_t* out, uint64_t out_bytes, int32_t* out_len) {
    if (!ctx || (n_jobs && (!jobs || !seqs || !offs || !out || !out_len))) return ctx ? fail(ctx, "snfb_poa: null argument") : 1;
    if (n_jobs == 0) return 0;
    cudaSetDevice(ctx->device);
    size_t smax = 0;
    for (uint32_t k = 0; k < n_jobs; ++k) {
        const snfb_poa_job& j = jobs[k];
        if ((uint64_t)j.offs_off + j.n_seq + 1 > n_offs) return fail(ctx, "snfb_poa: offsets outside offs[]");
        const int32_t* o = offs + j.offs_off; int total = 0, maxl = 0;
        for (uint32_t i = 0; i < j.n_seq; ++i) { const int l = o[i + 1] - o[i]; if (l < 0) return fail(ctx, "snfb_poa: decreasing offsets"); total += l; if (l > maxl) maxl = l; }
        if (j.seq_off + (uint64_t)(j.n_seq ? o[j.n_seq] : 0) > n_seq_bytes) return fail(ctx, "snfb_poa: sequences outside seqs[]");
        if (j.out_off + (uint64_t)j.out_cap * (j.mode == 1 ? 2 : 1) > out_bytes) return fail(ctx, "snfb_poa: output outside out[]");
        if (j.mode == 1 && j.n_seq != 2) return fail(ctx, "snfb_poa: the MSA mode takes exactly two sequences");
        const int bw = 2 * j.band + 1 < maxl ? 2 * j.band + 1 : (maxl > 0 ? maxl : 1);
        smax = std::max(smax, poa::scratch_bytes(total, maxl, bw));
    }
    size_t free_b = 0, total_b = 0; cudaMemGetInfo(&free_b, &total_b);
    size_t nblk = std::min<size_t>(n_jobs, NUM_SMS * 2);
    while (nblk > 1 && nblk * smax > free_b / 3) --nblk;
    if (smax > free_b / 2) return fail(ctx, "snfb_poa: a job needs more scratch than the device has free");
    DevBuf d_jobs, d_seqs, d_offs, d_out, d_len, d_scr, d_ctr;
    if (d_jobs.ensure(sizeof(snfb_poa_job) * n_jobs) || d_seqs.ensure(n_seq_bytes + 16) || d_offs.ensure(4 * n_offs + 16) || d_out.ensure(out_bytes + 16) || d_len.ensure(4 * (size_t)n_jobs) || d_scr.ensure(nblk * smax) || d_ctr.ensure(64))
        return fail(ctx, "snfb_poa: out of device memory");
    cudaStream_t st = ctx->st;
    CUDA_TRY(cudaMemcpyAsync(d_jobs.p, jobs, sizeof(snfb_poa_job) * n_jobs, cudaMemcpyHostToDevice, st)); CUDA_TRY(cudaMemcpyAsync(d_seqs.p, seqs, n_seq_bytes, cudaMemcpyHostToDevice, st));
    CUDA_TRY(cudaMemcpyAsync(d_offs.p, offs, 4 * n_offs, cudaMemcpyHostToDevice, st)); CUDA_TRY(cudaMemsetAsync(d_ctr.p, 0, 64, st)); CUDA_TRY(cudaMemsetAsync(d_out.p, 0, out_bytes, st));
    poa::Params P{}; P.jobs = d_jobs.as<poa::Job>(); P.n_jobs = n_jobs; P.seqs = d_seqs.as<uint8_t>(); P.offs = d_offs.as<int>(); P.out = d_out.as<uint8_t>(); P.out_len = d_len.as<int>();
    P.scratch = d_scr.as<uint8_t>(); P.scratch_per_block = smax; P.next_job = d_ctr.as<unsigned>();
    mark(ctx, "poa");
    launch(ctx->launches, poa::k_poa, (unsigned)nblk, poa::THREADS, 0, st, P);
    mark(ctx, nullptr);
    CUDA_TRY(cudaMemcpyAsync(out, d_out.p, out_bytes, cudaMemcpyDeviceToHost, st)); CUDA_TRY(cudaMemcpyAsync(out_len, d_len.p, 4 * (size_t)n_jobs, cudaMemcpyDeviceToHost, st));
    const cudaError_t e = cudaStreamSynchronize(st);
    if (e != cudaSuccess) return fail(ctx, std::string("snfb_poa: ") + cudaGetErrorString(e));
    return 0;
}

int snfb_combine_groups(snfb_ctx* ctx, const snfb_combine_in* in, snfb_combine_out* out) {
    if (!ctx || !in || !out) return ctx ? fail(ctx, "snfb_combine_groups: null argument") : 1;
    if (in->n_cand == 0 || in->n_chain == 0) return 0;
    if (!in->chains || !in->chunks || !in->pos || !in->svlen || !in->sample || !out->cand_group || !out->emit_chunk || !out->emit_ord || !out->cov_non)
        return fail(ctx, "snfb_combine_groups: null array");
    if (in->n_samples == 0 || in->bins_per_block <= 0 || in->cov_binsize <= 0) return fail(ctx, "snfb_combine_groups: bad sample count / coverage geometry");
    { uint64_t c = 0, k = 0;
      for (uint32_t i = 0; i < in->n_chain; ++i) { const snfb_combine_chain& ch = in->chains[i];
          if (ch.cand_off != c || ch.chunk_off != k || ch.n_chunk == 0) return fail(ctx, "snfb_combine_groups: chains do not tile the candidates / chunks");
          uint64_t cc = c;
          for (uint32_t j = 0; j < ch.n_chunk; ++j) { if (k + j >= in->n_chunk) return fail(ctx, "snfb_combine_groups: chunk index out of range"); const snfb_combine_chunk& ck = in->chunks[k + j];
              if ((uint64_t)ck.cand_off != cc || ck.n_cand <= 0 || ck.cov_block < -1 || ck.cov_block >= (int64_t)in->n_cov_block) return fail(ctx, "snfb_combine_groups: bad chunk"); cc += ck.n_cand; }
          if (cc != c + ch.n_cand) return fail(ctx, "snfb_combine_groups: chunk sizes do not add up to the chain");
          if (ch.is_bnd && (!in->mate_contig || !in->mate_pos)) return fail(ctx, "snfb_combine_groups: BND chain without mate arrays");
          c += ch.n_cand; k += ch.n_chunk; }
      if (c != in->n_cand || k != in->n_chunk) return fail(ctx, "snfb_combine_groups: plan does not cover n_cand / n_chunk");
      for (uint32_t i = 0; i < in->n_cand; ++i) if (in->sample[i] >= in->n_samples) return fail(ctx, "snfb_combine_groups: sample index out of range"); }
    cudaSetDevice(ctx->device);
    const size_t n = in->n_cand, S = in->n_samples, W = (S + 31) / 32, ncov = (size_t)in->n_cov_block * S * in->bins_per_block;
    const bool use_alt = in->combine_pctseq != 0.0 && in->alt && in->alt_off && in->alt_len;
    uint32_t max_alt = 16;
    if (use_alt) for (uint32_t i = 0; i < in->n_cand; ++i) { if (in->alt_off[i] + in->alt_len[i] > in->n_alt_bytes) return fail(ctx, "snfb_combine_groups: ALT outside alt[]"); max_alt = std::max(max_alt, in->alt_len[i]); }
    max_alt = (max_alt + 15u) & ~15u;
    const unsigned blocks = (unsigned)std::min<size_t>((in->n_chain + 3) / 4, NUM_SMS * 4);
    DevBuf b_in, b_state, b_out;
    combine::P P{};
    auto lay_in = [&](Carver& c) {
        P.chains = c.take<snfb_combine_chain>(in->n_chain); P.chunks = c.take<snfb_combine_chunk>(in->n_chunk); P.pos = c.take<int32_t>(n); P.svlen = c.take<int32_t>(n); P.sample = c.take<uint32_t>(n);
        P.mate_contig = c.take<int32_t>(n); P.mate_pos = c.take<int32_t>(n); P.block_start = c.take<long long>(in->n_cov_block + 1); P.cov = c.take<int32_t>(ncov + 1);
        if (use_alt) { P.alt = c.take<uint8_t>(in->n_alt_bytes + 16); P.alt_off = c.take<unsigned long long>(n); P.alt_len = c.take<uint32_t>(n); }
    };
    auto lay_state = [&](Carver& c) {
        P.g_pos = c.take<double>(n); P.g_len = c.take<double>(n); P.g_mate = c.take<double>(n); P.g_n = c.take<uint32_t>(n); P.g_mc = c.take<int32_t>(n); P.g_incl = c.take<uint32_t>(n * W); P.act = c.take<uint32_t>(n);
        P.next_chain = c.take<unsigned int>(4); P.g_first = c.take<uint32_t>(n); P.ex_stamp = c.take<uint32_t>(n); if (use_alt) P.hs = c.take<int8_t>((size_t)blocks * 4 * max_alt + 16);
    };
    auto lay_out = [&](Carver& c) { P.cand_group = c.take<uint32_t>(n); P.emit_chunk = c.take<int32_t>(n); P.emit_ord = c.take<uint32_t>(n); P.cov_non = c.take<int32_t>(n * S); };
    if (carve(b_in, lay_in) || carve(b_state, lay_state) || carve(b_out, lay_out)) return fail(ctx, "snfb_combine_groups: out of device memory");
    P.n_chain = in->n_chain; P.n_chunk = in->n_chunk; P.n_cand = in->n_cand; P.n_samples = in->n_samples; P.words = (uint32_t)W;
    P.bins_per_block = in->bins_per_block; P.cov_binsize = in->cov_binsize;
    P.combine_match = in->combine_match; P.combine_match_max = in->combine_match_max; P.cluster_merge_bnd = in->cluster_merge_bnd; P.separate_intra = in->combine_separate_intra; P.overlap_abs = in->combine_overlap_abs;
    cudaStream_t st = ctx->st;
    auto up = [&](const void* dst, const void* src, size_t bytes) { if (bytes && src) CUDA_TRY(cudaMemcpyAsync(const_cast<void*>(dst), src, bytes, cudaMemcpyHostToDevice, st)); return 0; };
    if (up(P.chains, in->chains, sizeof(snfb_combine_chain) * in->n_chain) || up(P.chunks, in->chunks, sizeof(snfb_combine_chunk) * in->n_chunk)
        || up(P.pos, in->pos, 4 * n) || up(P.svlen, in->svlen, 4 * n) || up(P.sample, in->sample, 4 * n) || up(P.mate_contig, in->mate_contig, 4 * n) || up(P.mate_pos, in->mate_pos, 4 * n)
        || up(P.block_start, in->block_start, 8 * (size_t)in->n_cov_block) || up(P.cov, in->cov, 4 * ncov)) return 1;
    P.pctseq = use_alt ? in->combine_pctseq : 0.0; P.max_alt = max_alt;
    if (use_alt && (up(P.alt, in->alt, in->n_alt_bytes) || up(P.alt_off, in->alt_off, 8 * n) || up(P.alt_len, in->alt_len, 4 * n))) return 1;
    CUDA_TRY(cudaMemsetAsync(P.next_chain, 0, 16, st));
    mark(ctx, "combine_groups");
    launch(ctx->launches, combine::k_combine, blocks, 128, 0, st, P);
    mark(ctx, nullptr);
    CUDA_TRY(cudaMemcpyAsync(out->cand_group, P.cand_group, 4 * n, cudaMemcpyDeviceToHost, st)); CUDA_TRY(cudaMemcpyAsync(out->emit_chunk, P.emit_chunk, 4 * n, cudaMemcpyDeviceToHost, st));
    CUDA_TRY(cudaMemcpyAsync(out->emit_ord, P.emit_ord, 4 * n, cudaMemcpyDeviceToHost, st)); CUDA_TRY(cudaMemcpyAsync(out->cov_non, P.cov_non, 4 * n * S, cudaMemcpyDeviceToHost, st));
    const cudaError_t e = cudaStreamSynchronize(st);
    if (e != cudaSuccess) return fail(ctx, std::string("snfb_combine_groups: ") + cudaGetErrorString(e));
    return 0;
}

int snfb_selftest_edit_distance(snfb_ctx* ctx, const uint8_t* bytes, uint64_t n_bytes, const uint64_t* a_off, const uint32_t* a_len, const uint64_t* b_off, const uint32_t* b_len, uint32_t n_pairs, int32_t* out) {
    if (!ctx || !bytes || !a_off || !a_len || !b_off || !b_len || !out) return ctx ? fail(ctx, "snfb_selftest_edit_distance: null argument") : 1;
    if (n_pairs == 0) return 0;
    uint32_t max_len = 16;
    for (uint32_t i = 0; i < n_pairs; ++i) { if (a_off[i] + a_len[i] > n_bytes || b_off[i] + b_len[i] > n_bytes) return fail(ctx, "snfb_selftest_edit_distance: string outside bytes[]"); max_len = std::max(max_len, std::max(a_len[i], b_len[i])); }
    max_len = (max_len + 15u) & ~15u;
    cudaSetDevice(ctx->device);
    const unsigned blocks = (unsigned)std::min<uint32_t>((n_pairs + 3) / 4, NUM_SMS * 4);
    DevBuf d_b, d_o, d_hs, d_out;
    if (d_b.ensure(n_bytes + 16) || d_o.ensure((size_t)n_pairs * 24 + 64) || d_hs.ensure((size_t)blocks * 4 * max_len + 16) || d_out.ensure((size_t)n_pairs * 4)) return fail(ctx, "snfb_selftest_edit_distance: out of device memory");
    unsigned long long* ao = d_o.as<unsigned long long>(); unsigned long long* bo = ao + n_pairs; uint32_t* al = reinterpret_cast<uint32_t*>(bo + n_pairs); uint32_t* bl = al + n_pairs;
    cudaStream_t st = ctx->st;
    CUDA_TRY(cudaMemcpyAsync(d_b.p, bytes, n_bytes, cudaMemcpyHostToDevice, st)); CUDA_TRY(cudaMemcpyAsync(ao, a_off, 8 * (size_t)n_pairs, cudaMemcpyHostToDevice, st)); CUDA_TRY(cudaMemcpyAsync(bo, b_off, 8 * (size_t)n_pairs, cudaMemcpyHostToDevice, st));
    CUDA_TRY(cudaMemcpyAsync(al, a_len, 4 * (size_t)n_pairs, cudaMemcpyHostToDevice, st)); CUDA_TRY(cudaMemcpyAsync(bl, b_len, 4 * (size_t)n_pairs, cudaMemcpyHostToDevice, st));
    launch(ctx->launches, combine::k_edit_selftest, blocks, 128, 0, st, d_b.as<uint8_t>(), ao, al, bo, bl, n_pairs, d_hs.as<int8_t>(), max_len, d_out.as<int>());
    CUDA_TRY(cudaMemcpyAsync(out, d_out.p, 4 * (size_t)n_pairs, cudaMemcpyDeviceToHost, st));
    const cudaError_t e = cudaStreamSynchronize(st);
    if (e != cudaSuccess) return fail(ctx, std::string("snfb_selftest_edit_distance: ") + cudaGetErrorString(e));
    return 0;
}

int snfb_coverage_bins(snfb_ctx* ctx, uint32_t task, int binsize, const double** out, uint64_t* n_bins) {
    if (!ctx || !ctx->stage_a_done) return ctx ? fail(ctx, "snfb_extract_leads must run first") : 1;
    if (task >= ctx->n_task || binsize <= 0 || !out || !n_bins) return fail(ctx, "bad arguments");
    cudaSetDevice(ctx->device);
    const snfb_task& tk = ctx->tasks[task];
    const long long L = tk.contig_len; const long long nb = L > 0 ? (L + binsize - 1) / binsize : 0;
    if (ctx->h_cov_bins.ensure(16 * (size_t)(nb + 1))) return fail(ctx, "out of pinned memory (coverage bins)");
    DevBuf acc; if (acc.ensure(8 * (size_t)(nb + 1))) return fail(ctx, "out of device memory (coverage bins)");
    CUDA_TRY(cudaMemsetAsync(acc.p, 0, 8 * (size_t)(nb + 1), ctx->st));
    uint32_t lohi[2], runs[2] = { 0, 0 };
    CUDA_TRY(cudaMemcpyAsync(&lohi[0], ctx->task_first + task, 4, cudaMemcpyDeviceToHost, ctx->st)); CUDA_TRY(cudaMemcpyAsync(&lohi[1], ctx->task_last + task, 4, cudaMemcpyDeviceToHost, ctx->st));
    if (ctx->n_mask) CUDA_TRY(cudaMemcpyAsync(runs, ctx->b_mask_off.as<uint32_t>() + task, 8, cudaMemcpyDeviceToHost, ctx->st));
    CUDA_TRY(cudaStreamSynchronize(ctx->st));
    if (nb && lohi[1] > lohi[0]) {
        launch(ctx->launches, k_cov_bins, grid_for(lohi[1] - lohi[0], 256), 256, 0, ctx->st, ctx->rec_pos, ctx->rec_end, ctx->rec_flags, lohi[0], lohi[1], binsize, L, nb, acc.as<unsigned long long>());
        if (runs[1] > runs[0]) launch(ctx->launches, cluster::k_mask_bins, grid_for((unsigned long long)(runs[1] - runs[0]) * 32, 128), 128, 0, ctx->st, ctx->B, (int)task, binsize, acc.as<unsigned long long>());
    }
    unsigned long long* raw = reinterpret_cast<unsigned long long*>(ctx->h_cov_bins.as<uint8_t>() + 8 * (size_t)(nb + 1));
    CUDA_TRY(cudaMemcpyAsync(raw, acc.p, 8 * (size_t)nb, cudaMemcpyDeviceToHost, ctx->st));
    CUDA_TRY(cudaStreamSynchronize(ctx->st));
    double* o = ctx->h_cov_bins.as<double>();
    for (long long i = 0; i < nb; ++i) o[i] = (double)raw[i] / (double)binsize;
    *out = o; *n_bins = (uint64_t)nb; return 0;
}

int snfb_genotype_targets(snfb_ctx* ctx, const snfb_gt_in* in, snfb_gt_out* out) {
    if (!ctx || !in || !out) return ctx ? fail(ctx, "snfb_genotype_targets: null argument") : 1;
    if (!ctx->stage_b_done) return fail(ctx, "snfb_genotype_targets: snfb_run or snfb_cluster_call must run first");
    const uint64_t n = in->n;
    if (n == 0) return 0;
    if (!in->task || !in->svtype || !in->pos || !in->svlen || !in->bnd_is_first || !in->mate_contig || !out->match || !out->cov_start || !out->cov_center || !out->cov_end || !out->bnd_no_prev)
        return fail(ctx, "snfb_genotype_targets: null array");
    std::vector<int64_t> prev(n);
    int64_t last = -1;
    for (uint64_t i = 0; i < n; ++i) {
        if (in->task[i] < 0 || (uint32_t)in->task[i] >= ctx->n_task) return fail(ctx, "snfb_genotype_targets: target task out of range");
        if (i && in->task[i] < in->task[i - 1]) return fail(ctx, "snfb_genotype_targets: targets are not ordered by task");
        if (in->svtype[i] < -1 || in->svtype[i] > SNFB_BND) return fail(ctx, "snfb_genotype_targets: target svtype must be SNFB_INS .. SNFB_BND or -1");
        if (i && in->task[i] != in->task[i - 1]) last = -1;
        prev[i] = last;
        if (in->svtype[i] != SNFB_BND) last = (int64_t)i;
    }
    cudaSetDevice(ctx->device);
    const unsigned long long nc = ctx->h_fin->n_cand;
    genotype::P G{}; uint64_t* k1 = nullptr; uint32_t* v1 = nullptr; prims::RadixTemp rt{};
    int32_t* t_in = nullptr; uint64_t* k0 = nullptr; uint32_t* v0 = nullptr;
    auto lay = [&](Carver& c) {
        k0 = c.take<uint64_t>(nc + 1); v0 = c.take<uint32_t>(nc + 1); k1 = c.take<uint64_t>(nc + 1); v1 = c.take<uint32_t>(nc + 1);
        rt.hist = c.take<uint32_t>(prims::radix_hist_elems(nc)); rt.scan_tmp = c.take<uint32_t>(prims::scan_tmp_elems(prims::radix_hist_elems(nc)) + 16);
        t_in = c.take<int32_t>(6 * n); G.prev = c.take<int64_t>(n); G.match = c.take<long long>(n); G.cov_start = c.take<int32_t>(4 * n);
    };
    if (carve(ctx->b_gt, lay)) return fail(ctx, "snfb_genotype_targets: out of device memory");
    G.task = t_in; G.svtype = t_in + n; G.pos = t_in + 2 * n; G.svlen = t_in + 3 * n; G.bnd_is_first = t_in + 4 * n; G.mate_contig = t_in + 5 * n;
    G.cov_center = G.cov_start + n; G.cov_end = G.cov_start + 2 * n; G.bnd_no_prev = G.cov_start + 3 * n;
    cudaStream_t st = ctx->st;
    const int32_t* src[6] = { in->task, in->svtype, in->pos, in->svlen, in->bnd_is_first, in->mate_contig };
    for (int k = 0; k < 6; ++k) CUDA_TRY(cudaMemcpyAsync(t_in + (size_t)k * n, src[k], 4 * n, cudaMemcpyHostToDevice, st));
    CUDA_TRY(cudaMemcpyAsync(const_cast<int64_t*>(G.prev), prev.data(), 8 * n, cudaMemcpyHostToDevice, st));
    ctx->n_ev = 0;
    mark(ctx, "genotype");
    bool first = true;
    if (nc) {
        launch(ctx->launches, genotype::k_cand_keys, grid_for(nc, 256), 256, 0, st, ctx->B.cand, nc, k0, v0);
        prims::radix_sort(ctx->launches, k0, v0, k1, v1, rt, &ctx->B.ctr->n_cand, nc, genotype::KEY_BITS + bits_for(ctx->n_task), &first, st);
    }
    G.b = ctx->B; G.key = first ? k0 : k1; G.val = first ? v0 : v1; G.n_cand = nc; G.n = n;
    G.combine_match = in->combine_match; G.combine_match_max = in->combine_match_max; G.cluster_merge_bnd = ctx->cfg.cluster_merge_bnd;
    launch(ctx->launches, genotype::k_genotype, grid_for(n * 32, 128), 128, 0, st, G);
    mark(ctx, nullptr);
    CUDA_TRY(cudaMemcpyAsync(out->match, G.match, 8 * n, cudaMemcpyDeviceToHost, st));
    int32_t* dst[4] = { out->cov_start, out->cov_center, out->cov_end, out->bnd_no_prev };
    for (int k = 0; k < 4; ++k) CUDA_TRY(cudaMemcpyAsync(dst[k], G.cov_start + (size_t)k * n, 4 * n, cudaMemcpyDeviceToHost, st));
    const cudaError_t e = cudaStreamSynchronize(st);
    if (e != cudaSuccess) return fail(ctx, std::string("snfb_genotype_targets: ") + cudaGetErrorString(e));
    return 0;
}

int snfb_load_reference(snfb_ctx* ctx, const snfb_ref_input* in) {
    if (!ctx || !in) return ctx ? fail(ctx, "snfb_load_reference: null argument") : 1;
    if ((in->n_bytes && !in->bytes) || (in->n_contig && !in->contig)) return fail(ctx, "snfb_load_reference: null table");
    cudaSetDevice(ctx->device);
    ctx->have_ref = false; ctx->ref_n_runs = 0; ctx->n_ev = 0;
    cudaStream_t st = ctx->st;
    uint64_t raw_len = 0;
    if (in->is_bgzf) {
        std::vector<ingest::BgzfBlock> blocks; std::vector<uint64_t> cstart;
        if (inflate_to_device(ctx, in->bytes, in->n_bytes, cstart, blocks, &raw_len, "h2d_ref")) return 1;
        const size_t nb = blocks.size();
        ingest::IngestCounters* d_ctr = nullptr; ingest::BgzfBlock* d_blk = nullptr;
        if (carve(ctx->b_ref_work, [&](Carver& c) { d_ctr = c.take<ingest::IngestCounters>(1); d_blk = c.take<ingest::BgzfBlock>(nb + 1); })) return fail(ctx, "out of device memory (reference inflate tables)");
        CUDA_TRY(cudaMemsetAsync(d_ctr, 0, sizeof(ingest::IngestCounters), st));
        CUDA_TRY(cudaMemcpyAsync(d_blk, blocks.data(), sizeof(ingest::BgzfBlock) * nb, cudaMemcpyHostToDevice, st));
        mark(ctx, "inflate", in->n_bytes + raw_len);
        if (nb) launch_inflate(ctx, d_blk, (unsigned)nb, d_ctr);
        mark(ctx, nullptr);
        ingest::IngestCounters hc;
        CUDA_TRY(cudaMemcpyAsync(&hc, d_ctr, sizeof(hc), cudaMemcpyDeviceToHost, st));
        CUDA_TRY(cudaStreamSynchronize(st));
        if (hc.bad_blocks) { ctx->b_raw.reset(); ctx->b_comp.reset(); inflate_failed(ctx, hc, cstart); ctx->err = "reference " + ctx->err; return 1; }
        ctx->b_comp.reset();
    } else {
        raw_len = in->n_bytes;
        if (ctx->b_raw.ensure(raw_len + 64)) return fail(ctx, "out of device memory for the reference FASTA bytes");
        mark(ctx, "h2d_ref", raw_len);
        CUDA_TRY(cudaMemcpyAsync(ctx->b_raw.p, in->bytes, raw_len, cudaMemcpyHostToDevice, st));
        CUDA_TRY(cudaMemsetAsync(ctx->b_raw.as<uint8_t>() + raw_len, 0, 64, st));
    }
    const uint32_t nc = in->n_contig;
    std::vector<refseq::Contig> ctg(nc); std::vector<refseq::Tile> ut, nt; std::vector<int64_t> first_nt(nc, -1);
    uint64_t total = 0;
    for (uint32_t c = 0; c < nc; ++c) {
        const snfb_ref_contig& k = in->contig[c];
        const std::string who = "snfb_load_reference: contig " + std::to_string(c);
        if (k.length >= (1ull << 31)) { ctx->b_raw.reset(); return fail(ctx, who + " is 2^31 bases or longer"); }
        if (k.length) {
            if (k.linebases == 0) { ctx->b_raw.reset(); return fail(ctx, who + ": LINEBASES is 0"); }
            const bool multi = k.length > k.linebases;
            if (k.linewidth != k.linebases + 1 && k.linewidth != k.linebases + 2 && (multi || k.linewidth != k.linebases)) { ctx->b_raw.reset(); return fail(ctx, who + ": LINEWIDTH must be LINEBASES + 1 or + 2"); }
            const uint64_t last = k.length - 1, end = k.offset + (last / k.linebases) * k.linewidth + last % k.linebases + 1;
            if (end > raw_len || end < k.offset) { ctx->b_raw.reset(); return fail(ctx, who + ": the .fai geometry reaches byte " + std::to_string(end) + " of a " + std::to_string(raw_len) + "-byte file"); }
        }
        total = (total + 15) & ~15ull;
        ctg[c] = refseq::Contig{ k.offset, k.length, total, k.linebases, k.linewidth };
        for (uint64_t p = 0; p < k.length; p += refseq::UNW_TILE) ut.push_back(refseq::Tile{ c, 0, p });
        if (k.length) first_nt[c] = (int64_t)nt.size();
        for (uint64_t p = 0; p < k.length; p += refseq::NR_TILE) nt.push_back(refseq::Tile{ c, 0, p });
        total += k.length;
    }
    if (nt.size() >= (1ull << 31)) { ctx->b_raw.reset(); return fail(ctx, "snfb_load_reference: genome too large"); }
    if (ctx->b_ref.ensure(total + 256)) { ctx->b_raw.reset(); return fail(ctx, "out of device memory for the reference genome"); }
    const size_t nu = ut.size(), nn = nt.size();
    refseq::Contig* d_ctg = nullptr; refseq::Tile* d_ut = nullptr; refseq::Tile* d_nt = nullptr; refseq::Bad* d_bad = nullptr;
    uint32_t *n_s = nullptr, *n_e = nullptr, *o_s = nullptr, *o_e = nullptr, *tmp = nullptr; unsigned long long* tot = nullptr;
    if (carve(ctx->b_ref_work, [&](Carver& c) { d_ctg = c.take<refseq::Contig>(nc + 1); d_ut = c.take<refseq::Tile>(nu + 1); d_nt = c.take<refseq::Tile>(nn + 1); d_bad = c.take<refseq::Bad>(1);
                                                n_s = c.take<uint32_t>(nn + 1); n_e = c.take<uint32_t>(nn + 1); o_s = c.take<uint32_t>(nn + 1); o_e = c.take<uint32_t>(nn + 1);
                                                tmp = c.take<uint32_t>(prims::scan_tmp_elems(nn + 1) + 16); tot = c.take<unsigned long long>(2); }))
        { ctx->b_raw.reset(); return fail(ctx, "out of device memory (reference tables)"); }
    if (nc) CUDA_TRY(cudaMemcpyAsync(d_ctg, ctg.data(), sizeof(refseq::Contig) * nc, cudaMemcpyHostToDevice, st));
    if (nu) CUDA_TRY(cudaMemcpyAsync(d_ut, ut.data(), sizeof(refseq::Tile) * nu, cudaMemcpyHostToDevice, st));
    if (nn) CUDA_TRY(cudaMemcpyAsync(d_nt, nt.data(), sizeof(refseq::Tile) * nn, cudaMemcpyHostToDevice, st));
    const refseq::Bad bad0{ 0ull, ~0ull };
    CUDA_TRY(cudaMemcpyAsync(d_bad, &bad0, sizeof(bad0), cudaMemcpyHostToDevice, st));
    mark(ctx, "ref_unwrap", raw_len + total);
    if (nu) launch(ctx->launches, refseq::k_ref_unwrap, (unsigned)std::min<size_t>(nu, (size_t)NUM_SMS * 8), refseq::UNW_THREADS, 0, st, ctx->b_raw.as<const uint8_t>(), d_ctg, d_ut, (unsigned)nu, ctx->b_ref.as<uint8_t>(), d_bad);
    mark(ctx, "ref_nruns", 2 * total);
    if (nn) {
        launch(ctx->launches, refseq::k_ref_nruns_count, (unsigned)nn, refseq::NR_THREADS, 0, st, ctx->b_ref.as<const uint8_t>(), d_ctg, d_nt, n_s, n_e);
        prims::exclusive_scan(ctx->launches, n_s, o_s, tmp, nullptr, nn, tot, st);
        prims::exclusive_scan(ctx->launches, n_e, o_e, tmp, nullptr, nn, tot + 1, st);
    } else CUDA_TRY(cudaMemsetAsync(tot, 0, 16, st));
    refseq::Bad hb; unsigned long long ht[2];
    CUDA_TRY(cudaMemcpyAsync(&hb, d_bad, sizeof(hb), cudaMemcpyDeviceToHost, st));
    CUDA_TRY(cudaMemcpyAsync(ht, tot, sizeof(ht), cudaMemcpyDeviceToHost, st));
    CUDA_TRY(cudaStreamSynchronize(st));
    ctx->b_raw.reset();
    if (hb.n) return fail(ctx, "snfb_load_reference: " + std::to_string(hb.n) + " line(s) do not match the .fai geometry (first: contig " + std::to_string(hb.first >> 40)
                               + ", line " + std::to_string(hb.first & ((1ull << 40) - 1)) + "): the index does not describe this file");
    if (ht[0] != ht[1]) return fail(ctx, "snfb_load_reference: N-run starts and ends do not pair up");
    const uint64_t nr = ht[0];
    if (ctx->h_ref_runs.ensure(8 * (nr + 1)) || ctx->h_ref_coff.ensure(8 * ((size_t)nc + 1)) || ctx->h_ref_out.ensure(4 * (nn + 1))) return fail(ctx, "out of pinned memory (reference N runs)");
    DevBuf d_runs;
    if (d_runs.ensure(8 * (nr + 1))) return fail(ctx, "out of device memory (reference N runs)");
    if (nn && nr) launch(ctx->launches, refseq::k_ref_nruns_write, (unsigned)nn, refseq::NR_THREADS, 0, st, ctx->b_ref.as<const uint8_t>(), d_ctg, d_nt, o_s, o_e, d_runs.as<int32_t>());
    mark(ctx, nullptr);
    if (nr) CUDA_TRY(cudaMemcpyAsync(ctx->h_ref_runs.p, d_runs.p, 8 * nr, cudaMemcpyDeviceToHost, st));
    uint32_t* h_os = ctx->h_ref_out.as<uint32_t>();
    if (nn) CUDA_TRY(cudaMemcpyAsync(h_os, o_s, 4 * nn, cudaMemcpyDeviceToHost, st));
    CUDA_TRY(cudaStreamSynchronize(st));
    uint64_t* coff = ctx->h_ref_coff.as<uint64_t>();
    coff[nc] = nr;
    for (int64_t c = (int64_t)nc - 1; c >= 0; --c) coff[c] = first_nt[c] >= 0 ? h_os[first_nt[c]] : coff[c + 1];
    ctx->ref_ctg = std::move(ctg); ctx->ref_n_runs = nr; ctx->have_ref = true;
    return 0;
}

int snfb_reference_runs(snfb_ctx* ctx, const int32_t** runs, const uint64_t** contig_off, uint64_t* n_runs) {
    if (!ctx || !runs || !contig_off || !n_runs) return ctx ? fail(ctx, "snfb_reference_runs: null argument") : 1;
    if (!ctx->have_ref) return fail(ctx, "snfb_reference_runs: no reference is loaded (snfb_load_reference)");
    *runs = ctx->h_ref_runs.as<int32_t>(); *contig_off = ctx->h_ref_coff.as<uint64_t>(); *n_runs = ctx->ref_n_runs;
    return 0;
}

int snfb_fetch_reference(snfb_ctx* ctx, const snfb_ref_query* q, uint64_t n, uint8_t* out, uint64_t out_cap) {
    if (!ctx || (n && (!q || !out))) return ctx ? fail(ctx, "snfb_fetch_reference: null argument") : 1;
    if (!ctx->have_ref) return fail(ctx, "snfb_fetch_reference: no reference is loaded (snfb_load_reference)");
    std::vector<refseq::Query> hq(n); uint64_t span = 0;
    for (uint64_t i = 0; i < n; ++i) {
        const snfb_ref_query& x = q[i];
        if (x.contig >= ctx->ref_ctg.size()) return fail(ctx, "snfb_fetch_reference: query " + std::to_string(i) + ": contig index out of range");
        const refseq::Contig& c = ctx->ref_ctg[x.contig];
        if (x.start > c.len || x.length > c.len - x.start) return fail(ctx, "snfb_fetch_reference: query " + std::to_string(i) + " reaches past the end of contig " + std::to_string(x.contig));
        if (x.out_off > out_cap || x.length > out_cap - x.out_off) return fail(ctx, "snfb_fetch_reference: query " + std::to_string(i) + " does not fit out_cap");
        hq[i] = refseq::Query{ c.out_off + x.start, x.length, x.out_off };
        span = std::max<uint64_t>(span, x.out_off + x.length);
    }
    ctx->n_ev = 0;
    if (n == 0) return 0;
    cudaSetDevice(ctx->device);
    refseq::Query* d_q = nullptr; uint8_t* d_out = nullptr;
    if (carve(ctx->b_ref_work, [&](Carver& c) { d_q = c.take<refseq::Query>(n); d_out = c.take<uint8_t>(span + 16); })) return fail(ctx, "snfb_fetch_reference: out of device memory");
    cudaStream_t st = ctx->st;
    CUDA_TRY(cudaMemcpyAsync(d_q, hq.data(), sizeof(refseq::Query) * n, cudaMemcpyHostToDevice, st));
    mark(ctx, "ref_gather", 2 * span);
    launch(ctx->launches, refseq::k_ref_gather, grid_for(n * 32, 256), 256, 0, st, ctx->b_ref.as<const uint8_t>(), d_q, (unsigned long long)n, d_out);
    mark(ctx, nullptr);
    CUDA_TRY(cudaMemcpyAsync(out, d_out, span, cudaMemcpyDeviceToHost, st));
    const cudaError_t e = cudaStreamSynchronize(st);
    if (e != cudaSuccess) return fail(ctx, std::string("snfb_fetch_reference: ") + cudaGetErrorString(e));
    return 0;
}

}
```

### sniffles_b200/csrc/consensus.cuh

```cuda
#pragma once
#include "common.cuh"

namespace consensus {

constexpr int THREADS = 128;
constexpr int TAB = 2048;
constexpr uint8_t DASH = 0xff;
constexpr int MAXHIT = 512, MAXHIT_LIGHT = 384; constexpr uint32_t HEAVY_L = 3000;

struct C {
    const snfb_cand* cand; snfb_cand* cand_rw; const snfb_lead* cand_leads;
    const uint32_t* out_plo; const uint32_t* out_pn;
    const uint32_t* ord; const snfb_lead* kleads;
    const snfb_rec* rec; const uint8_t* seq;
    const uint32_t* arena_off;
    uint32_t* plan_best; uint32_t* plan_nother; uint32_t* plan_otot; uint32_t* alt_len; uint32_t* scr_len; uint32_t* alt_off; uint32_t* scr_off;
    uint8_t* alt; uint8_t* scr; unsigned long long alt_cap, scr_cap16, cand_cap;
    uint32_t* work_big; uint32_t* work_small; uint32_t* work_ctr;
    struct Item { uint32_t cand; uint32_t k; uint32_t row; uint32_t rd_off; };
    Item* items_big; Item* items_small; uint2* tiles; unsigned long long item_cap, tile_cap;
    DevCounters* ctr; snfb_config cfg;
};

__device__ __forceinline__ uint8_t seq_code(const uint8_t* sq, long long q) { const uint8_t v = sq[q >> 1]; return (q & 1) ? (v & 15) : (v >> 4); }

__global__ void k_plan(C c) {
    const unsigned long long nc = c.ctr->n_cand < c.cand_cap ? c.ctr->n_cand : c.cand_cap;
    for (unsigned long long i = blockIdx.x * (unsigned long long)blockDim.x + threadIdx.x; i < nc; i += (unsigned long long)gridDim.x * blockDim.x) {
        uint32_t al = 0, sl = 0;
        if (c.cand[i].svtype == SNFB_INS && !c.cfg.symbolic) {
            const snfb_cand* cd = &c.cand[i]; long nm = 0, bi = -1; long long bd = 0; long long tot = 0;
            for (int k = 0; k < cd->lead_n; ++k) { const snfb_lead* l = &c.cand_leads[cd->lead_off + k]; if (!(l->flags & SNFB_LF_HAS_SEQ)) continue;
                long long a = (long long)l->seq_len - cd->svlen; if (a < 0) a = -a; long long p = (long long)l->ref_start - cd->pos; if (p < 0) p = -p;
                const long long d = 2 * a + 3 * p; if (nm == 0 || d < bd) { bd = d; bi = k; } ++nm; tot += ((long long)l->seq_len + 7) & ~7ll; }
            if (nm > 0) {
                const uint32_t L = (uint32_t)c.cand_leads[cd->lead_off + bi].seq_len; al = L;
                const bool cons = (nm - 1 >= c.cfg.consensus_min_reads) && !c.cfg.no_consensus;
                c.plan_best[i] = (uint32_t)bi; c.plan_nother[i] = cons ? (uint32_t)(nm - 1) : 0u; c.plan_otot[i] = (uint32_t)(tot - ((L + 7u) & ~7u));
                const unsigned long long bytes = cons ? (unsigned long long)tot + 8 + (unsigned long long)(nm - 1) * ((L + 3u) & ~3u) + (unsigned long long)(nm - 1) * 16 + 64 + 16 + TAB * 8 : (unsigned long long)L + 24;
                sl = (uint32_t)((bytes + 15) / 16);
                c.cand_rw[i].alt_len = (int)L;
                const unsigned long long work = (unsigned long long)L * (unsigned long long)nm;
                if (work > 60000ull) c.work_big[atomicAdd(&c.work_ctr[0], 1u)] = (uint32_t)i; else c.work_small[atomicAdd(&c.work_ctr[1], 1u)] = (uint32_t)i;
                if (cons) {
                    const bool heavy = L > HEAVY_L; C::Item* dst = heavy ? c.items_big : c.items_small;
                    const uint32_t base = atomicAdd(&c.work_ctr[heavy ? 4 : 5], (uint32_t)(nm - 1));
                    uint32_t row = 0, ro = 0;
                    for (int k = 0; k < cd->lead_n; ++k) { const snfb_lead* l = &c.cand_leads[cd->lead_off + k]; if (!(l->flags & SNFB_LF_HAS_SEQ) || k == bi) continue;
                        if ((unsigned long long)base + row < c.item_cap) { C::Item it; it.cand = (uint32_t)i; it.k = (uint32_t)k; it.row = row; it.rd_off = ro; dst[base + row] = it; }
                        ++row; ro += ((uint32_t)l->seq_len + 7u) & ~7u; }
                    const uint32_t nt = (L + 4095u) / 4096u; const uint32_t tb = atomicAdd(&c.work_ctr[8], nt);
                    for (uint32_t t = 0; t < nt; ++t) if ((unsigned long long)tb + t < c.tile_cap) c.tiles[tb + t] = make_uint2((uint32_t)i, t);
                }
            }
        }
        c.alt_len[i] = al; c.scr_len[i] = sl;
    }
}

__global__ void k_plan_finish(C c) {
    const unsigned long long nc = c.ctr->n_cand < c.cand_cap ? c.ctr->n_cand : c.cand_cap;
    for (unsigned long long i = blockIdx.x * (unsigned long long)blockDim.x + threadIdx.x; i < nc; i += (unsigned long long)gridDim.x * blockDim.x)
        if (c.scr_len[i]) c.cand_rw[i].alt_off = (int)c.alt_off[i];
}

__device__ __forceinline__ uint32_t nib_swap(uint32_t w) { return ((w & 0x0f0f0f0fu) << 4) | ((w >> 4) & 0x0f0f0f0fu); }
__device__ __forceinline__ uint32_t spread4(uint32_t x) { const uint32_t t = (x | (x << 8)) & 0x00ff00ffu; return (t | (t << 4)) & 0x0f0f0f0fu; }
__device__ __forceinline__ uint2 unpack8(const uint8_t* __restrict__ sq, long long q, int n) {
    const uintptr_t A = (uintptr_t)(sq + (q >> 1));
    const uint32_t* w = reinterpret_cast<const uint32_t*>(A & ~(uintptr_t)3);
    const int qn = (int)((A & 3) << 1) | (int)(q & 1);
    const uint32_t lo = nib_swap(__ldg(w)), hi = qn + n > 8 ? nib_swap(__ldg(w + 1)) : 0u;
    const uint32_t x = __funnelshift_r(lo, hi, 4 * qn);
    return make_uint2(spread4(x & 0xffffu), spread4(x >> 16));
}
__device__ __forceinline__ void unpack_span(const uint8_t* __restrict__ sq, long long off, int len, uint8_t* __restrict__ dst, int tid, int nthr) {
    const int full = ((uintptr_t)dst & 7) == 0 ? (len & ~7) : 0;
    int jb = tid * 8;
    for (; jb + 7 * nthr * 8 < full; jb += 8 * nthr * 8) {
        uint2 v[8];
        #pragma unroll
        for (int u = 0; u < 8; ++u) v[u] = unpack8(sq, off + jb + u * nthr * 8, 8);
        #pragma unroll
        for (int u = 0; u < 8; ++u) *reinterpret_cast<uint2*>(dst + jb + u * nthr * 8) = v[u];
    }
    for (; jb < full; jb += nthr * 8) *reinterpret_cast<uint2*>(dst + jb) = unpack8(sq, off + jb, 8);
    for (; jb < len; jb += nthr * 8) {
        const int n = min(8, len - jb); const uint2 v = unpack8(sq, off + jb, n);
        for (int t = 0; t < n; ++t) dst[jb + t] = (uint8_t)(((t < 4 ? v.x : v.y) >> (8 * (t & 3))) & 15u);
    }
}
__device__ inline void unpack_lead(const C& c, uint32_t cl_index, uint8_t* dst, int tid, int nthr) {
    const uint32_t plo = c.out_plo[cl_index], pn = c.out_pn[cl_index];
    long long o = 0;
    for (uint32_t p = 0; p < pn; ++p) {
        const uint32_t slot = c.ord[plo + p]; const snfb_lead* l = &c.kleads[slot];
        const uint8_t* sq = c.arena_off ? c.seq + (size_t)c.arena_off[slot] * 16 : c.seq + c.rec[l->rec].seq_off;
        unpack_span(sq, c.arena_off ? (l->seq_off & 1) : l->seq_off, l->seq_len, dst + o, tid, nthr);
        o += l->seq_len;
    }
}

__device__ __forceinline__ uint32_t kmer6(const uint8_t* s) { return (uint32_t)s[0] | ((uint32_t)s[1] << 4) | ((uint32_t)s[2] << 8) | ((uint32_t)s[3] << 12) | ((uint32_t)s[4] << 16) | ((uint32_t)s[5] << 20); }
__device__ __forceinline__ uint32_t kmer6_u(const uint8_t* s) {
    const uintptr_t A = (uintptr_t)s; const uint32_t* w = reinterpret_cast<const uint32_t*>(A & ~(uintptr_t)3); const uint32_t sh = (uint32_t)(A & 3) * 8;
    const uint32_t l0 = w[0], l1 = w[1], l2 = sh > 16 ? w[2] : 0u;
    const uint32_t x0 = __funnelshift_r(l0, l1, sh), x1 = __funnelshift_r(l1, l2, sh);
    uint32_t t = x0 & 0x0f0f0f0fu; t = (t | (t >> 4)) & 0x00ff00ffu; t = (t | (t >> 8)) & 0xffffu;
    return t | ((x1 & 15u) << 16) | (((x1 >> 8) & 15u) << 20);
}
__device__ __forceinline__ uint32_t kslot(uint32_t key) { return (key * 2654435761u) >> 21; }

struct SeqReq { unsigned long long src; uint32_t nbytes; uint32_t dst16; };
__global__ void k_seq_requests(C c, SeqReq* req, unsigned long long req_cap, uint32_t* arena_off_rw, unsigned long long* n_req, unsigned long long* n_units) {
    const unsigned long long nc = c.ctr->n_cand < c.cand_cap ? c.ctr->n_cand : c.cand_cap;
    for (unsigned long long i = blockIdx.x * (unsigned long long)blockDim.x + threadIdx.x; i < nc; i += (unsigned long long)gridDim.x * blockDim.x) {
        if (c.scr_len[i] == 0) continue;
        const snfb_cand* cd = &c.cand[i]; const bool cons = c.plan_nother[i] > 0;
        for (int k = 0; k < cd->lead_n; ++k) {
            const snfb_lead* cl = &c.cand_leads[cd->lead_off + k];
            if (!(cl->flags & SNFB_LF_HAS_SEQ) || (!cons && (uint32_t)k != c.plan_best[i])) continue;
            const uint32_t plo = c.out_plo[cd->lead_off + k], pn = c.out_pn[cd->lead_off + k];
            for (uint32_t p = 0; p < pn; ++p) {
                const uint32_t slot = c.ord[plo + p]; const snfb_lead* l = &c.kleads[slot];
                const unsigned long long b0 = (unsigned long long)l->seq_off >> 1, b1 = ((unsigned long long)l->seq_off + l->seq_len + 1) >> 1;
                const uint32_t nb = (uint32_t)(b1 - b0) + 1;
                const unsigned long long u = atomicAdd(n_units, (unsigned long long)((nb + 15) / 16));
                const unsigned long long r = atomicAdd(n_req, 1ULL);
                arena_off_rw[slot] = (uint32_t)u;
                if (r < req_cap) { req[r].src = c.rec[l->rec].seq_off + b0; req[r].nbytes = nb; req[r].dst16 = (uint32_t)u; }
            }
        }
    }
}



__device__ __forceinline__ int match_count(const uint8_t* a, const uint8_t* b, long n) {
    const uint32_t sa = ((uintptr_t)a & 3) * 8, sb = ((uintptr_t)b & 3) * 8;
    const uint32_t* wa = reinterpret_cast<const uint32_t*>((uintptr_t)a & ~(uintptr_t)3); const uint32_t* wb = reinterpret_cast<const uint32_t*>((uintptr_t)b & ~(uintptr_t)3);
    uint32_t alo = wa[0], blo = wb[0]; int mt = 0;
    long q = 0;
    #pragma unroll 2
    for (; q + 4 <= n; q += 4) {
        const uint32_t ahi = *++wa, bhi = *++wb;
        const uint32_t x = __funnelshift_r(alo, ahi, sa) ^ __funnelshift_r(blo, bhi, sb);
        mt += __popc(~(((x & 0x7f7f7f7fu) + 0x7f7f7f7fu) | x) & 0x80808080u);
        alo = ahi; blo = bhi;
    }
    if (q < n) {
        const uint32_t ahi = *++wa, bhi = *++wb;
        const uint32_t x = __funnelshift_r(alo, ahi, sa) ^ __funnelshift_r(blo, bhi, sb);
        mt += __popc(~(((x & 0x7f7f7f7fu) + 0x7f7f7f7fu) | x) & 0x80808080u & ((1u << (8 * (n - q))) - 1u));
    }
    return mt;
}
__device__ __forceinline__ void copy_bytes(uint8_t* dst, const uint8_t* src, long n) {
    long q = 0;
    while (q < n && ((uintptr_t)(dst + q) & 3)) { dst[q] = src[q]; ++q; }
    if (q + 4 <= n) {
        const uint8_t* s0 = src + q; const uint32_t sh = ((uintptr_t)s0 & 3) * 8;
        const uint32_t* ws = reinterpret_cast<const uint32_t*>((uintptr_t)s0 & ~(uintptr_t)3); uint32_t lo = ws[0];
        uint32_t* wd = reinterpret_cast<uint32_t*>(dst + q);
        #pragma unroll 4
        for (; q + 4 <= n; q += 4) { const uint32_t hi = *++ws; *wd++ = __funnelshift_r(lo, hi, sh); lo = hi; }
    }
    for (; q < n; ++q) dst[q] = src[q];
}
__device__ __forceinline__ void fill_dash(uint8_t* dst, long n) {
    long q = 0;
    while (q < n && ((uintptr_t)(dst + q) & 3)) dst[q++] = DASH;
    for (; q + 4 <= n; q += 4) *reinterpret_cast<uint32_t*>(dst + q) = 0xffffffffu;
    for (; q < n; ++q) dst[q] = DASH;
}

__device__ __forceinline__ uint32_t load_u32_unaligned(const uint8_t* p) {
    const uintptr_t A = (uintptr_t)p; const uint32_t* w = reinterpret_cast<const uint32_t*>(A & ~(uintptr_t)3);
    return __funnelshift_r(w[0], w[1], (uint32_t)(A & 3) * 8);
}
template <int G>
__device__ __forceinline__ int group_match(const uint8_t* a, const uint8_t* b, long n, int sub) {
    int mt = 0;
    #pragma unroll 2
    for (long q = 4L * sub; q < n; q += 4L * G) {
        const uint32_t x = load_u32_unaligned(a + q) ^ load_u32_unaligned(b + q);
        uint32_t eq = ~(((x & 0x7f7f7f7fu) + 0x7f7f7f7fu) | x) & 0x80808080u;
        if (n - q < 4) eq &= (1u << (8 * (n - q))) - 1u;
        mt += __popc(eq);
    }
    return mt;
}
template <int G> __device__ __forceinline__ int group_sum(int v) {
    #pragma unroll
    for (int o = G / 2; o > 0; o >>= 1) v += __shfl_xor_sync(FULL, v, o);
    return v;
}
struct WarpGrp {
    static constexpr int NTHR = 32; int tid;
    __device__ __forceinline__ void sync() const { __syncwarp(); }
    __device__ __forceinline__ int excl(int v, int& tot) const {
        int inc = v;
        #pragma unroll
        for (int o = 1; o < 32; o <<= 1) { const int t = __shfl_up_sync(FULL, inc, o); if (tid >= o) inc += t; }
        tot = __shfl_sync(FULL, inc, 31); return inc - v;
    }
    __device__ __forceinline__ int exclmax(int v, int& tot) const {
        int inc = v;
        #pragma unroll
        for (int o = 1; o < 32; o <<= 1) { const int t = __shfl_up_sync(FULL, inc, o); if (tid >= o) inc = max(inc, t); }
        tot = __shfl_sync(FULL, inc, 31); int e = __shfl_up_sync(FULL, inc, 1); if (tid == 0) e = -1; return e;
    }
    __device__ __forceinline__ long sum(long v) const { return (long)__reduce_add_sync(FULL, (unsigned)v); }
};
template <int WARPS>
struct BlockGrp {
    static constexpr int NTHR = WARPS * 32; int tid; int* red;
    __device__ __forceinline__ void sync() const { __syncthreads(); }
    __device__ __forceinline__ int excl(int v, int& tot) const {
        const int lane = tid & 31, w = tid >> 5; int inc = v;
        #pragma unroll
        for (int o = 1; o < 32; o <<= 1) { const int t = __shfl_up_sync(FULL, inc, o); if (lane >= o) inc += t; }
        if (lane == 31) red[w] = inc;
        __syncthreads();
        int base = 0, all = 0;
        #pragma unroll
        for (int k = 0; k < WARPS; ++k) { const int t = red[k]; if (k < w) base += t; all += t; }
        __syncthreads();
        tot = all; return base + inc - v;
    }
    __device__ __forceinline__ int exclmax(int v, int& tot) const {
        const int lane = tid & 31, w = tid >> 5; int inc = v;
        #pragma unroll
        for (int o = 1; o < 32; o <<= 1) { const int t = __shfl_up_sync(FULL, inc, o); if (lane >= o) inc = max(inc, t); }
        int e = __shfl_up_sync(FULL, inc, 1); if (lane == 0) e = -1;
        if (lane == 31) red[w] = inc;
        __syncthreads();
        int all = -1;
        #pragma unroll
        for (int k = 0; k < WARPS; ++k) { const int t = red[k]; if (k < w) e = max(e, t); all = max(all, t); }
        __syncthreads();
        tot = all; return e;
    }
    __device__ __forceinline__ long sum(long v) const {
        const int lane = tid & 31, w = tid >> 5; const int sv = (int)__reduce_add_sync(FULL, (unsigned)v);
        if (lane == 0) red[w] = sv;
        __syncthreads();
        int all = 0;
        #pragma unroll
        for (int k = 0; k < WARPS; ++k) all += red[k];
        __syncthreads();
        return (long)all;
    }
};

template <int G>
__device__ __forceinline__ long segments_pass(const int* hi, const int* hj, int* hcl, int na, long c0, long j0, long L, const uint8_t* rd, const uint8_t* best, int tid, int nthr) {
    const int PER = nthr / G; const int grp = tid / G, sub = tid % G; long span = 0;
    for (int mb = 1; mb < na; mb += PER) {
        const int m = mb + grp; const bool v = m < na;
        long li = 0, lj = 0, i = 0, j = 0; if (v) { li = hi[m - 1]; lj = hj[m - 1]; i = hi[m]; j = hj[m]; }
        long cs = c0 + lj - j0; if (cs > L) cs = L;
        const long d = j - lj; long fwd_j = d; if (cs + fwd_j > L) fwd_j = L - cs;
        const bool el = v && i - li == fwd_j && fwd_j > 0;
        long nc = 0; if (el) { nc = L - 1 - li; if (nc > d) nc = d; if (nc < 0) nc = 0; }
        const int mt = group_sum<G>(group_match<G>(rd + lj + 1, best + li + 1, nc, sub));
        int st = -1; bool second = false;
        if (el) { if (sub == 0) span += d; if (__ddiv_rn((double)mt, (double)d) >= 0.5) { if (cs == li && fwd_j == d && nc == d) st = mt; else second = true; } }
        const int m2 = group_sum<G>(group_match<G>(rd + lj, best + cs, second ? fwd_j : 0, sub));
        if (second) st = m2;
        if (v && sub == 0) hcl[m] = st;
    }
    return span;
}

struct Layout { uint8_t* best; uint8_t* oth; uint8_t* rows; uint8_t* acc; uint32_t Ls; };
__device__ __forceinline__ Layout cand_layout(const C& c, uint32_t ci, uint32_t L, uint32_t no) {
    Layout y; y.best = c.scr + (size_t)c.scr_off[ci] * 16; y.oth = y.best + ((L + 7u) & ~7u);
    y.rows = reinterpret_cast<uint8_t*>(((uintptr_t)(y.oth + c.plan_otot[ci]) + 3) & ~(uintptr_t)3); y.Ls = (L + 3u) & ~3u; y.acc = y.rows + (size_t)no * y.Ls;
    return y;
}
__device__ __forceinline__ uint8_t* cand_table(const C& c, uint32_t ci, uint32_t** keys, int** pos) {
    uint8_t* scr = c.scr + (size_t)c.scr_off[ci] * 16;
    uint8_t* end = scr + (size_t)c.scr_len[ci] * 16;
    *keys = reinterpret_cast<uint32_t*>(end - TAB * 8); *pos = reinterpret_cast<int*>(end - TAB * 4);
    return scr;
}

__global__ void __launch_bounds__(128) k_prep(C c) {
    __shared__ uint32_t s_cand;
    static const char CODE[17] = "=ACMGRSVTWYHKDBN";
    for (;;) {
        __syncthreads();
        if (threadIdx.x == 0) { const uint32_t q = atomicAdd(&c.work_ctr[2], 1u); const uint32_t nb = c.work_ctr[0], ns = c.work_ctr[1];
            s_cand = q < nb ? c.work_big[q] : (q < nb + ns ? c.work_small[q - nb] : 0xffffffffu); }
        __syncthreads();
        const uint32_t ci = s_cand; if (ci == 0xffffffffu) break;
        const uint32_t L = c.alt_len[ci];
        if ((unsigned long long)c.alt_off[ci] + L > c.alt_cap || (unsigned long long)c.scr_off[ci] + c.scr_len[ci] > c.scr_cap16) { if (threadIdx.x == 0) atomicAdd(&c.ctr->scratch_overflow, 1ULL); continue; }
        const snfb_cand cd = c.cand[ci];
        uint32_t* tk; int* tp; uint8_t* best = cand_table(c, ci, &tk, &tp);
        unpack_lead(c, cd.lead_off + c.plan_best[ci], best, threadIdx.x, blockDim.x);
        const uint32_t no = c.plan_nother[ci];
        if (no == 0 || L == 0) { __syncthreads(); uint8_t* out = c.alt + c.alt_off[ci]; for (uint32_t h = threadIdx.x; h < L; h += blockDim.x) out[h] = (uint8_t)CODE[best[h]]; continue; }
        for (int i = threadIdx.x; i < TAB; i += blockDim.x) { tk[i] = 0xffffffffu; tp[i] = -1; }
        __syncthreads();
        const long skip = c.cfg.consensus_kmer_skip_base + (long)__dmul_rn((double)L, c.cfg.consensus_kmer_skip_seqlen_mult);
        for (long i = (long)threadIdx.x * skip; i < (long)L - 6; i += (long)blockDim.x * skip) {
            const uint32_t key = kmer6_u(best + i); uint32_t s = kslot(key);
            for (;;) { const uint32_t old = atomicCAS(&tk[s], 0xffffffffu, key); if (old == 0xffffffffu || old == key) break; s = (s + 1) & (TAB - 1); }
            if (atomicCAS(&tp[s], -1, (int)i) != -1) tp[s] = -2;
        }
    }
}

template <typename G>
__device__ __forceinline__ void align_item(const C& c, const C::Item it, const G g, int* hi, int* hj, int* hcl, int* run_st, int* run_len, int cap) {
    const int tid = g.tid; constexpr int NT = G::NTHR; const int klen = 6;
    const uint32_t ci = it.cand; const uint32_t L = c.alt_len[ci];
    if ((unsigned long long)c.scr_off[ci] + c.scr_len[ci] > c.scr_cap16) return;
    const snfb_cand* cd = &c.cand[ci];
    uint32_t* t_key; int* t_pos; cand_table(c, ci, &t_key, &t_pos);
    const uint32_t no = c.plan_nother[ci];
    const Layout y = cand_layout(c, ci, L, no);
    uint8_t* best = y.best; uint8_t* acc = y.acc;
    const snfb_lead* l = &c.cand_leads[cd->lead_off + it.k];
    const long Lo = l->seq_len; uint8_t* rd = y.oth + it.rd_off; uint8_t* row = y.rows + (size_t)it.row * y.Ls;
    const long skip = c.cfg.consensus_kmer_skip_base + (long)__dmul_rn((double)L, c.cfg.consensus_kmer_skip_seqlen_mult);
    unpack_lead(c, cd->lead_off + it.k, rd, tid, NT);
    g.sync();
    int nh = 0;
    const long nk = Lo - klen > 0 ? (Lo - klen + skip - 1) / skip : 0;
    for (long kb = 0; kb < nk; kb += 4 * NT) {
        uint32_t key[4], sl[4], tk[4]; int ai[4];
        #pragma unroll
        for (int u = 0; u < 4; ++u) { const long kk = kb + u * NT + tid; key[u] = kk < nk ? kmer6_u(rd + kk * skip) : 0u; sl[u] = kslot(key[u]); }
        #pragma unroll
        for (int u = 0; u < 4; ++u) tk[u] = kb + u * NT + tid < nk ? t_key[sl[u]] : 0xffffffffu;
        #pragma unroll
        for (int u = 0; u < 4; ++u) while (tk[u] != 0xffffffffu && tk[u] != key[u]) { sl[u] = (sl[u] + 1) & (TAB - 1); tk[u] = t_key[sl[u]]; }
        #pragma unroll
        for (int u = 0; u < 4; ++u) ai[u] = tk[u] != 0xffffffffu ? t_pos[sl[u]] : -1;
        #pragma unroll
        for (int u = 0; u < 4; ++u) {
            if (kb + (long)u * NT >= nk) break;
            const long j = (kb + u * NT + tid) * skip;
            if (ai[u] >= 0) { long d = ai[u] - j; if (d < 0) d = -d; if (d > klen) ai[u] = -1; }
            int tot; const int off = g.excl(ai[u] >= 0 ? 1 : 0, tot);
            if (ai[u] >= 0) { const int p = nh + off; if (p < cap) { hi[p] = ai[u]; hj[p] = (int)j; } }
            nh += tot;
        }
    }
    if (nh > cap) nh = cap;
    g.sync();
    int na = 0, pm = -1;
    for (int hb = 0; hb < nh; hb += NT) {
        const int h = hb + tid; const int vi = h < nh ? hi[h] : -1, vj = h < nh ? hj[h] : 0;
        int tmax; const int exc = max(g.exclmax(vi, tmax), pm);
        const bool accp = h < nh && vi > exc;
        int tot; const int off = g.excl(accp ? 1 : 0, tot);
        g.sync();
        if (accp) { hi[na + off] = vi; hj[na + off] = vj; }
        na += tot; pm = max(pm, tmax);
        g.sync();
    }
    const long j0 = na ? hj[0] : 0, c0 = (na && j0 > 0) ? hi[0] : 0;
    long span = skip > 12 ? segments_pass<8>(hi, hj, hcl, na, c0, j0, (long)L, rd, best, tid, NT) : segments_pass<1>(hi, hj, hcl, na, c0, j0, (long)L, rd, best, tid, NT);
    span = g.sum(span);
    g.sync();
    {
        int* hr = hi;
        for (int m = tid; m < na; m += NT) { run_st[m] = 0; run_len[m] = 0; }
        g.sync();
        int run_base = 0;
        for (int mb = 1; mb < na; mb += NT) {
            const int m = mb + tid; int st = -1; long len = 0;
            if (m < na) { const long lj = hj[m - 1]; long cs = c0 + lj - j0; if (cs > (long)L) cs = (long)L; len = hj[m] - lj; if (cs + len > (long)L) len = (long)L - cs; st = hcl[m]; }
            int tot; const int rid = run_base + g.excl((m < na && st < 0 && len > 0) ? 1 : 0, tot);
            g.sync();
            if (m < na) { hr[m] = rid; if (st >= 0) { atomicAdd(&run_st[rid], st); atomicAdd(&run_len[rid], (int)len); } }
            run_base += tot;
        }
        g.sync();
        for (int m = 1 + tid; m < na; m += NT) {
            if (hcl[m] < 0) continue;
            const int r = hr[m], ident = run_st[r];
            if (!(__ddiv_rn((double)ident, (double)run_len[r]) > 0.5 && ident > 5)) hcl[m] = -1;
        }
        g.sync();
    }
    {
        long cl = 0; if (na) { cl = c0 + hj[na - 1] - j0; if (cl > (long)L) cl = (long)L; }
        const uint8_t* src0 = rd + (j0 - c0);
        #pragma unroll 4
        for (long X = 4L * tid; X < (long)L; X += 4L * NT) {
            uint32_t v = 0xffffffffu;
            if (X + 4 > c0 && X < cl) {
                v = load_u32_unaligned(src0 + X);
                if (X < c0) v |= (1u << (8 * (c0 - X))) - 1u;
                if (X + 4 > cl) v |= ~((1u << (8 * (cl - X))) - 1u);
            }
            *reinterpret_cast<uint32_t*>(row + X) = v;
        }
        g.sync();
        for (int m = 1 + tid; m < na; m += NT) {
            if (hcl[m] >= 0) continue;
            const long lj = hj[m - 1]; long cs = c0 + lj - j0; if (cs > (long)L) cs = (long)L;
            long len = hj[m] - lj; if (cs + len > (long)L) len = (long)L - cs;
            if (len > 0) fill_dash(row + cs, len);
        }
    }
    if (tid == 0) acc[it.row] = __ddiv_rn((double)span, (double)L) > 0.2;
    g.sync();
}

constexpr int ALIGN_WARPS = 4;
__global__ void __launch_bounds__(ALIGN_WARPS * 32, 7) k_align(C c) {
    __shared__ int sm[5][ALIGN_WARPS * MAXHIT_LIGHT]; __shared__ int s_red[2 * ALIGN_WARPS]; __shared__ uint32_t s_q;
    static_assert(ALIGN_WARPS * MAXHIT_LIGHT >= MAXHIT, "a block item needs MAXHIT entries");
    const int lane = lane_id(), warp = threadIdx.x >> 5;
    const uint32_t nb = (uint32_t)min((unsigned long long)c.work_ctr[4], c.item_cap), ns = (uint32_t)min((unsigned long long)c.work_ctr[5], c.item_cap);
    for (;;) {
        __syncthreads();
        if (threadIdx.x == 0) s_q = atomicAdd(&c.work_ctr[6], 1u);
        __syncthreads();
        const uint32_t q = s_q; if (q >= nb) break;
        BlockGrp<ALIGN_WARPS> g; g.tid = threadIdx.x; g.red = s_red;
        align_item(c, c.items_big[q], g, sm[0], sm[1], sm[2], sm[3], sm[4], ALIGN_WARPS * MAXHIT_LIGHT);
    }
    __syncthreads();
    for (;;) {
        uint32_t q = 0; if (lane == 0) q = atomicAdd(&c.work_ctr[7], 1u);
        q = __shfl_sync(FULL, q, 0);
        if (q >= ns) break;
        WarpGrp g; g.tid = lane; const int o = warp * MAXHIT_LIGHT;
        align_item(c, c.items_small[q], g, sm[0] + o, sm[1] + o, sm[2] + o, sm[3] + o, sm[4] + o, MAXHIT_LIGHT);
    }
}

constexpr int VOTE_LIST = 256;
__device__ __forceinline__ void vote_add(unsigned long long (&cnt)[4], uint32_t code) {
    const unsigned long long inc = 1ull << (16 * (code & 3u)); const uint32_t sel = (code >> 2) & 3u;
    #pragma unroll
    for (int k = 0; k < 4; ++k) cnt[k] += sel == (uint32_t)k ? inc : 0ull;
}
constexpr int VOTE_THREADS = 64;
__global__ void __launch_bounds__(VOTE_THREADS) k_vote(C c) {
    __shared__ uint2 s_tile; __shared__ int s_nacc, s_nlist; __shared__ uint16_t s_rows[VOTE_LIST];
    static const char CODE[17] = "=ACMGRSVTWYHKDBN";
    for (;;) {
        __syncthreads();
        if (threadIdx.x == 0) { const uint32_t q = atomicAdd(&c.work_ctr[9], 1u); s_tile = q < c.work_ctr[8] && q < c.tile_cap ? c.tiles[q] : make_uint2(0xffffffffu, 0); }
        __syncthreads();
        const uint32_t ci = s_tile.x; if (ci == 0xffffffffu) break;
        const uint32_t L = c.alt_len[ci], no = c.plan_nother[ci];
        if ((unsigned long long)c.alt_off[ci] + L > c.alt_cap || (unsigned long long)c.scr_off[ci] + c.scr_len[ci] > c.scr_cap16) continue;
        const Layout y = cand_layout(c, ci, L, no);
        const uint8_t* best = y.best; const uint8_t* rows = y.rows; const uint8_t* acc = y.acc; const uint32_t Ls = y.Ls;
        if (threadIdx.x < 32) {
            int cnt = 0, extra = 0; const uint32_t lim = no < (uint32_t)VOTE_LIST ? no : (uint32_t)VOTE_LIST;
            for (uint32_t r0 = 0; r0 < lim; r0 += 32) { const uint32_t r = r0 + threadIdx.x; const bool a = r < lim && acc[r]; const unsigned bm = __ballot_sync(FULL, a);
                if (a) s_rows[cnt + __popc(bm & lanemask_lt())] = (uint16_t)r; cnt += __popc(bm); }
            for (uint32_t r = lim + threadIdx.x; r < no; r += 32) extra += acc[r] ? 1 : 0;
            extra = (int)__reduce_add_sync(FULL, (unsigned)extra);
            if (threadIdx.x == 0) { s_nlist = cnt; s_nacc = cnt + extra; }
        }
        __syncthreads();
        const double maxal = (double)(1 + s_nacc); const int nlist = s_nlist;
        uint8_t* out = c.alt + c.alt_off[ci];
        const uint32_t h_end = min(L, (s_tile.y + 1u) * 4096u);
        for (uint32_t h = s_tile.y * 4096u + threadIdx.x * 4u; h < h_end; h += blockDim.x * 4u) {
            const uint32_t bw = *reinterpret_cast<const uint32_t*>(best + h);
            if (nlist == s_nacc && nlist < 255) {
                uint32_t cA = 0, cC = 0, cG = 0, cT = 0, cD = 0, multi = 0;
                for (int r0 = 0; r0 < nlist; r0 += 8) {
                    uint32_t cv[8];
                    #pragma unroll
                    for (int u = 0; u < 8; ++u) cv[u] = r0 + u < nlist ? *reinterpret_cast<const uint32_t*>(rows + (size_t)s_rows[r0 + u] * Ls + h) : 0xffffffffu;
                    #pragma unroll
                    for (int u = 0; u < 8; ++u) {
                        const uint32_t hb = cv[u] & 0x80808080u, d1 = hb >> 7, t = cv[u] & ~(hb | (hb - d1));
                        cD += d1; multi |= ((t | 0x10101010u) - 0x01010101u) & t;
                        cA += t & 0x01010101u; cC += (t >> 1) & 0x01010101u; cG += (t >> 2) & 0x01010101u; cT += (t >> 3) & 0x01010101u;
                    }
                }
                const uint32_t padded = (uint32_t)((nlist + 7) & ~7);
                const uint32_t tot = cA + cC + cG + cT + cD;
                const bool best_ok = (((bw | 0x10101010u) - 0x01010101u) & bw) == 0 && ((bw - 0x01010101u) & ~bw & 0x80808080u) == 0;
                if (multi == 0 && best_ok && padded <= 248 && tot == padded * 0x01010101u) {
                    #pragma unroll
                    for (int b2 = 0; b2 < 4; ++b2) {
                        if (h + b2 >= h_end) break;
                        const uint32_t bc = (bw >> (8 * b2)) & 255u; uint32_t res = bc;
                        const int nal = (int)padded - (int)((cD >> (8 * b2)) & 255u);
                        if (!(nal < 2 || __ddiv_rn((double)nal, maxal) < 0.25)) {
                            int v4[4] = { (int)((cA >> (8 * b2)) & 255u), (int)((cC >> (8 * b2)) & 255u), (int)((cG >> (8 * b2)) & 255u), (int)((cT >> (8 * b2)) & 255u) };
                            int t0 = -1, t1 = -1, c0 = 0, nd = 0;
                            #pragma unroll
                            for (int k = 0; k < 4; ++k) { const int v = v4[k] + ((bc >> k) & 1u); if (!v) continue; ++nd; if (v > t0) { t1 = t0; t0 = v; c0 = 1 << k; } else if (v > t1) t1 = v; }
                            if (nd > 1 && t0 - t1 >= 3) res = (uint32_t)c0;
                        }
                        out[h + b2] = (uint8_t)CODE[res];
                    }
                    continue;
                }
            }
            unsigned long long cnt[4][4]; int nal[4];
            #pragma unroll
            for (int b2 = 0; b2 < 4; ++b2) { nal[b2] = 0; cnt[b2][0] = cnt[b2][1] = cnt[b2][2] = cnt[b2][3] = 0; }
            for (int r0 = 0; r0 < nlist; r0 += 8) {
                uint32_t cv[8];
                #pragma unroll
                for (int u = 0; u < 8; ++u) cv[u] = r0 + u < nlist ? *reinterpret_cast<const uint32_t*>(rows + (size_t)s_rows[r0 + u] * Ls + h) : 0xffffffffu;
                #pragma unroll
                for (int u = 0; u < 8; ++u) {
                    #pragma unroll
                    for (int b2 = 0; b2 < 4; ++b2) { const uint32_t cc = (cv[u] >> (8 * b2)) & 255u; if (cc != DASH) { vote_add(cnt[b2], cc); ++nal[b2]; } }
                }
            }
            for (uint32_t r = VOTE_LIST; r < no; ++r) if (acc[r]) {
                const uint32_t v = *reinterpret_cast<const uint32_t*>(rows + (size_t)r * Ls + h);
                #pragma unroll
                for (int b2 = 0; b2 < 4; ++b2) { const uint32_t cc = (v >> (8 * b2)) & 255u; if (cc != DASH) { vote_add(cnt[b2], cc); ++nal[b2]; } }
            }
            #pragma unroll
            for (int b2 = 0; b2 < 4; ++b2) {
                if (h + b2 >= h_end) break;
                const uint32_t bc = (bw >> (8 * b2)) & 255u; uint32_t res = bc;
                if (!(nal[b2] < 2 || __ddiv_rn((double)nal[b2], maxal) < 0.25)) {
                    vote_add(cnt[b2], bc);
                    int t0 = -1, t1 = -1, c0 = 0, nd = 0;
                    #pragma unroll
                    for (int code = 0; code < 16; ++code) { const int v = (int)((cnt[b2][code >> 2] >> (16 * (code & 3))) & 0xffff); if (!v) continue; ++nd; if (v > t0) { t1 = t0; t0 = v; c0 = code; } else if (v > t1) t1 = v; }
                    if (nd > 1 && t0 - t1 >= 3) res = (uint32_t)c0;
                }
                out[h + b2] = (uint8_t)CODE[res];
            }
        }
    }
}

}
```

Baseline: 9749.

## Store consensus reads as 4-bit packed words with per-row dash bitmasks

Consensus scratch now keeps the best and other reads as nibble-packed 32-bit words instead of unpacked bytes. Each aligned row is no longer materialised as a full byte copy; it is described by a per-row descriptor plus a dash bitmask, and bytes are rebuilt on the fly during voting. Matching compares eight bases per word, and voting works on 8-base groups. The aim is to cut scratch memory traffic and footprint, at the cost of extra bit manipulation and atomics when building masks. Consensus kernels are also skipped when the sequence request overflows capacity.

```diff
diff --git a/sniffles_b200/csrc/api.cu b/sniffles_b200/csrc/api.cu
--- a/sniffles_b200/csrc/api.cu
+++ b/sniffles_b200/csrc/api.cu
@@ -772,6 +772,7 @@
 static int enqueue_stage_c(snfb_ctx* ctx) {
     cluster::B& b = ctx->B; consensus::C& c = ctx->Cc; DevCounters* ctr = b.ctr; cudaStream_t st = ctx->st;
     c.seq = ctx->d_seq; c.arena_off = nullptr; ctx->seq_h2d_bytes = 0;
+    bool fits = true;
     if (ctx->seq_on_demand) {
         mark(ctx, "seq_requests");
         launch(ctx->launches, consensus::k_seq_requests, grid_for(ctx->cap.cand, 128), 128, 0, st, c, ctx->seq_req, ctx->cap.req, ctx->arena_off, &ctr->n_req, &ctr->n_req_units);
@@ -779,7 +780,8 @@
         CUDA_TRY(cudaMemcpyAsync(ctx->h_fin, ctr, sizeof(DevCounters), cudaMemcpyDeviceToHost, st));
         CUDA_TRY(cudaStreamSynchronize(st));
         const unsigned long long nreq = ctx->h_fin->n_req, nunits = ctx->h_fin->n_req_units;
-        if (nreq <= ctx->cap.req && nunits <= ctx->cap.req16 && nreq) {
+        fits = nreq <= ctx->cap.req && nunits <= ctx->cap.req16;
+        if (fits && nreq) {
             if (ctx->h_seq_req.ensure(sizeof(consensus::SeqReq) * (nreq + 1)) || ctx->h_seq_arena.ensure(nunits * 16 + 64)) return fail(ctx, "out of pinned memory (seq arena)");
             CUDA_TRY(cudaMemcpyAsync(ctx->h_seq_req.p, ctx->seq_req, sizeof(consensus::SeqReq) * nreq, cudaMemcpyDeviceToHost, st));
             CUDA_TRY(cudaStreamSynchronize(st));
@@ -797,11 +799,11 @@
         c.seq = ctx->seq_arena; c.arena_off = ctx->arena_off;
     }
     mark(ctx, "consensus");
-    launch(ctx->launches, consensus::k_prep, NUM_SMS * 8, 128, 0, st, c);
+    if (fits) launch(ctx->launches, consensus::k_prep, NUM_SMS * 8, 128, 0, st, c);
     mark(ctx, "consensus_align");
-    launch(ctx->launches, consensus::k_align, NUM_SMS * 7, consensus::ALIGN_WARPS * 32, 0, st, c);
+    if (fits) launch(ctx->launches, consensus::k_align, NUM_SMS * 7, consensus::ALIGN_WARPS * 32, 0, st, c);
     mark(ctx, "consensus_vote");
-    launch(ctx->launches, consensus::k_vote, NUM_SMS * 16, consensus::VOTE_THREADS, 0, st, c);
+    if (fits) launch(ctx->launches, consensus::k_vote, NUM_SMS * 16, consensus::VOTE_THREADS, 0, st, c);
     mark(ctx, nullptr);
     CUDA_TRY(cudaGetLastError());
     return 0;
diff --git a/sniffles_b200/csrc/consensus.cuh b/sniffles_b200/csrc/consensus.cuh
--- a/sniffles_b200/csrc/consensus.cuh
+++ b/sniffles_b200/csrc/consensus.cuh
@@ -7,6 +7,7 @@
 constexpr int TAB = 2048;
 constexpr uint8_t DASH = 0xff;
 constexpr int MAXHIT = 512, MAXHIT_LIGHT = 384; constexpr uint32_t HEAVY_L = 3000;
+constexpr uint32_t VOTE_TILE = 4096;
 
 struct C {
     const snfb_cand* cand; snfb_cand* cand_rw; const snfb_lead* cand_leads;
@@ -22,7 +23,7 @@
     DevCounters* ctr; snfb_config cfg;
 };
 
-__device__ __forceinline__ uint8_t seq_code(const uint8_t* sq, long long q) { const uint8_t v = sq[q >> 1]; return (q & 1) ? (v & 15) : (v >> 4); }
+__host__ __device__ __forceinline__ uint32_t pk_bytes(uint32_t len) { return ((len + 7u) / 8u + 1u) * 4u; }
 
 __global__ void k_plan(C c) {
     const unsigned long long nc = c.ctr->n_cand < c.cand_cap ? c.ctr->n_cand : c.cand_cap;
@@ -32,12 +33,13 @@
             const snfb_cand* cd = &c.cand[i]; long nm = 0, bi = -1; long long bd = 0; long long tot = 0;
             for (int k = 0; k < cd->lead_n; ++k) { const snfb_lead* l = &c.cand_leads[cd->lead_off + k]; if (!(l->flags & SNFB_LF_HAS_SEQ)) continue;
                 long long a = (long long)l->seq_len - cd->svlen; if (a < 0) a = -a; long long p = (long long)l->ref_start - cd->pos; if (p < 0) p = -p;
-                const long long d = 2 * a + 3 * p; if (nm == 0 || d < bd) { bd = d; bi = k; } ++nm; tot += ((long long)l->seq_len + 7) & ~7ll; }
+                const long long d = 2 * a + 3 * p; if (nm == 0 || d < bd) { bd = d; bi = k; } ++nm; tot += pk_bytes((uint32_t)l->seq_len); }
             if (nm > 0) {
                 const uint32_t L = (uint32_t)c.cand_leads[cd->lead_off + bi].seq_len; al = L;
                 const bool cons = (nm - 1 >= c.cfg.consensus_min_reads) && !c.cfg.no_consensus;
-                c.plan_best[i] = (uint32_t)bi; c.plan_nother[i] = cons ? (uint32_t)(nm - 1) : 0u; c.plan_otot[i] = (uint32_t)(tot - ((L + 7u) & ~7u));
-                const unsigned long long bytes = cons ? (unsigned long long)tot + 8 + (unsigned long long)(nm - 1) * ((L + 3u) & ~3u) + (unsigned long long)(nm - 1) * 16 + 64 + 16 + TAB * 8 : (unsigned long long)L + 24;
+                c.plan_best[i] = (uint32_t)bi; c.plan_nother[i] = cons ? (uint32_t)(nm - 1) : 0u; c.plan_otot[i] = (uint32_t)(tot - pk_bytes(L));
+                const unsigned long long per_row = 16 + 4ull * ((L + 31u) / 32u) + 1;
+                const unsigned long long bytes = cons ? (unsigned long long)tot + 16 + (unsigned long long)(nm - 1) * per_row + 64 + 16 + TAB * 8 : (unsigned long long)pk_bytes(L) + 16;
                 sl = (uint32_t)((bytes + 15) / 16);
                 c.cand_rw[i].alt_len = (int)L;
                 const unsigned long long work = (unsigned long long)L * (unsigned long long)nm;
@@ -48,8 +50,8 @@
                     uint32_t row = 0, ro = 0;
                     for (int k = 0; k < cd->lead_n; ++k) { const snfb_lead* l = &c.cand_leads[cd->lead_off + k]; if (!(l->flags & SNFB_LF_HAS_SEQ) || k == bi) continue;
                         if ((unsigned long long)base + row < c.item_cap) { C::Item it; it.cand = (uint32_t)i; it.k = (uint32_t)k; it.row = row; it.rd_off = ro; dst[base + row] = it; }
-                        ++row; ro += ((uint32_t)l->seq_len + 7u) & ~7u; }
-                    const uint32_t nt = (L + 4095u) / 4096u; const uint32_t tb = atomicAdd(&c.work_ctr[8], nt);
+                        ++row; ro += pk_bytes((uint32_t)l->seq_len); }
+                    const uint32_t nt = (L + VOTE_TILE - 1u) / VOTE_TILE; const uint32_t tb = atomicAdd(&c.work_ctr[8], nt);
                     for (uint32_t t = 0; t < nt; ++t) if ((unsigned long long)tb + t < c.tile_cap) c.tiles[tb + t] = make_uint2((uint32_t)i, t);
                 }
             }
@@ -66,49 +68,42 @@
 
 __device__ __forceinline__ uint32_t nib_swap(uint32_t w) { return ((w & 0x0f0f0f0fu) << 4) | ((w >> 4) & 0x0f0f0f0fu); }
 __device__ __forceinline__ uint32_t spread4(uint32_t x) { const uint32_t t = (x | (x << 8)) & 0x00ff00ffu; return (t | (t << 4)) & 0x0f0f0f0fu; }
-__device__ __forceinline__ uint2 unpack8(const uint8_t* __restrict__ sq, long long q, int n) {
+__device__ __forceinline__ uint32_t arena8(const uint8_t* __restrict__ sq, long long q, int n) {
     const uintptr_t A = (uintptr_t)(sq + (q >> 1));
     const uint32_t* w = reinterpret_cast<const uint32_t*>(A & ~(uintptr_t)3);
     const int qn = (int)((A & 3) << 1) | (int)(q & 1);
     const uint32_t lo = nib_swap(__ldg(w)), hi = qn + n > 8 ? nib_swap(__ldg(w + 1)) : 0u;
     const uint32_t x = __funnelshift_r(lo, hi, 4 * qn);
-    return make_uint2(spread4(x & 0xffffu), spread4(x >> 16));
-}
-__device__ __forceinline__ void unpack_span(const uint8_t* __restrict__ sq, long long off, int len, uint8_t* __restrict__ dst, int tid, int nthr) {
-    const int full = ((uintptr_t)dst & 7) == 0 ? (len & ~7) : 0;
-    int jb = tid * 8;
-    for (; jb + 7 * nthr * 8 < full; jb += 8 * nthr * 8) {
-        uint2 v[8];
-        #pragma unroll
-        for (int u = 0; u < 8; ++u) v[u] = unpack8(sq, off + jb + u * nthr * 8, 8);
-        #pragma unroll
-        for (int u = 0; u < 8; ++u) *reinterpret_cast<uint2*>(dst + jb + u * nthr * 8) = v[u];
-    }
-    for (; jb < full; jb += nthr * 8) *reinterpret_cast<uint2*>(dst + jb) = unpack8(sq, off + jb, 8);
-    for (; jb < len; jb += nthr * 8) {
-        const int n = min(8, len - jb); const uint2 v = unpack8(sq, off + jb, n);
-        for (int t = 0; t < n; ++t) dst[jb + t] = (uint8_t)(((t < 4 ? v.x : v.y) >> (8 * (t & 3))) & 15u);
-    }
-}
-__device__ inline void unpack_lead(const C& c, uint32_t cl_index, uint8_t* dst, int tid, int nthr) {
-    const uint32_t plo = c.out_plo[cl_index], pn = c.out_pn[cl_index];
-    long long o = 0;
-    for (uint32_t p = 0; p < pn; ++p) {
-        const uint32_t slot = c.ord[plo + p]; const snfb_lead* l = &c.kleads[slot];
-        const uint8_t* sq = c.arena_off ? c.seq + (size_t)c.arena_off[slot] * 16 : c.seq + c.rec[l->rec].seq_off;
-        unpack_span(sq, c.arena_off ? (l->seq_off & 1) : l->seq_off, l->seq_len, dst + o, tid, nthr);
-        o += l->seq_len;
-    }
-}
-
-__device__ __forceinline__ uint32_t kmer6(const uint8_t* s) { return (uint32_t)s[0] | ((uint32_t)s[1] << 4) | ((uint32_t)s[2] << 8) | ((uint32_t)s[3] << 12) | ((uint32_t)s[4] << 16) | ((uint32_t)s[5] << 20); }
-__device__ __forceinline__ uint32_t kmer6_u(const uint8_t* s) {
-    const uintptr_t A = (uintptr_t)s; const uint32_t* w = reinterpret_cast<const uint32_t*>(A & ~(uintptr_t)3); const uint32_t sh = (uint32_t)(A & 3) * 8;
-    const uint32_t l0 = w[0], l1 = w[1], l2 = sh > 16 ? w[2] : 0u;
-    const uint32_t x0 = __funnelshift_r(l0, l1, sh), x1 = __funnelshift_r(l1, l2, sh);
-    uint32_t t = x0 & 0x0f0f0f0fu; t = (t | (t >> 4)) & 0x00ff00ffu; t = (t | (t >> 8)) & 0xffffu;
-    return t | ((x1 & 15u) << 16) | (((x1 >> 8) & 15u) << 20);
-}
+    return n < 8 ? x & ((1u << (4 * n)) - 1u) : x;
+}
+__device__ __forceinline__ uint32_t pk8(const uint32_t* w, int p) { const int i = p >> 3; return __funnelshift_r(w[i], w[i + 1], 4u * (uint32_t)(p & 7)); }
+__device__ __forceinline__ const uint8_t* lead_bases(const C& c, uint32_t slot, long long& q0) {
+    const snfb_lead* l = &c.kleads[slot];
+    if (c.arena_off) { q0 = l->seq_off & 1; return c.seq + (size_t)c.arena_off[slot] * 16; }
+    q0 = l->seq_off; return c.seq + c.rec[l->rec].seq_off;
+}
+__device__ inline void pack_lead(const C& c, uint32_t cl_index, uint32_t len, uint32_t* __restrict__ dst, int tid, int nthr) {
+    const uint32_t plo = c.out_plo[cl_index], pn = c.out_pn[cl_index], nw = (len + 7u) / 8u;
+    if (pn == 1) {
+        long long q0; const uint8_t* sq = lead_bases(c, c.ord[plo], q0);
+        for (uint32_t w = tid; w < nw; w += nthr) dst[w] = arena8(sq, q0 + 8ll * w, (int)min(8u, len - 8u * w));
+    } else {
+        for (uint32_t w = tid; w < nw; w += nthr) {
+            const long long b0 = 8ll * w, b1 = min((long long)len, b0 + 8); uint32_t x = 0; long long o = 0;
+            for (uint32_t p = 0; p < pn && o < b1; ++p) {
+                const uint32_t slot = c.ord[plo + p]; const long long n = c.kleads[slot].seq_len;
+                if (o + n > b0) {
+                    const long long lo = max(b0, o), hi = min(b1, o + n); long long q0; const uint8_t* sq = lead_bases(c, slot, q0);
+                    x |= arena8(sq, q0 + (lo - o), (int)(hi - lo)) << (4 * (lo - b0));
+                }
+                o += n;
+            }
+            dst[w] = x;
+        }
+    }
+    if (tid == 0) dst[nw] = 0u;
+}
+
 __device__ __forceinline__ uint32_t kslot(uint32_t key) { return (key * 2654435761u) >> 21; }
 
 struct SeqReq { unsigned long long src; uint32_t nbytes; uint32_t dst16; };
@@ -136,56 +131,14 @@
 
 
 
-__device__ __forceinline__ int match_count(const uint8_t* a, const uint8_t* b, long n) {
-    const uint32_t sa = ((uintptr_t)a & 3) * 8, sb = ((uintptr_t)b & 3) * 8;
-    const uint32_t* wa = reinterpret_cast<const uint32_t*>((uintptr_t)a & ~(uintptr_t)3); const uint32_t* wb = reinterpret_cast<const uint32_t*>((uintptr_t)b & ~(uintptr_t)3);
-    uint32_t alo = wa[0], blo = wb[0]; int mt = 0;
-    long q = 0;
-    #pragma unroll 2
-    for (; q + 4 <= n; q += 4) {
-        const uint32_t ahi = *++wa, bhi = *++wb;
-        const uint32_t x = __funnelshift_r(alo, ahi, sa) ^ __funnelshift_r(blo, bhi, sb);
-        mt += __popc(~(((x & 0x7f7f7f7fu) + 0x7f7f7f7fu) | x) & 0x80808080u);
-        alo = ahi; blo = bhi;
-    }
-    if (q < n) {
-        const uint32_t ahi = *++wa, bhi = *++wb;
-        const uint32_t x = __funnelshift_r(alo, ahi, sa) ^ __funnelshift_r(blo, bhi, sb);
-        mt += __popc(~(((x & 0x7f7f7f7fu) + 0x7f7f7f7fu) | x) & 0x80808080u & ((1u << (8 * (n - q))) - 1u));
-    }
-    return mt;
-}
-__device__ __forceinline__ void copy_bytes(uint8_t* dst, const uint8_t* src, long n) {
-    long q = 0;
-    while (q < n && ((uintptr_t)(dst + q) & 3)) { dst[q] = src[q]; ++q; }
-    if (q + 4 <= n) {
-        const uint8_t* s0 = src + q; const uint32_t sh = ((uintptr_t)s0 & 3) * 8;
-        const uint32_t* ws = reinterpret_cast<const uint32_t*>((uintptr_t)s0 & ~(uintptr_t)3); uint32_t lo = ws[0];
-        uint32_t* wd = reinterpret_cast<uint32_t*>(dst + q);
-        #pragma unroll 4
-        for (; q + 4 <= n; q += 4) { const uint32_t hi = *++ws; *wd++ = __funnelshift_r(lo, hi, sh); lo = hi; }
-    }
-    for (; q < n; ++q) dst[q] = src[q];
-}
-__device__ __forceinline__ void fill_dash(uint8_t* dst, long n) {
-    long q = 0;
-    while (q < n && ((uintptr_t)(dst + q) & 3)) dst[q++] = DASH;
-    for (; q + 4 <= n; q += 4) *reinterpret_cast<uint32_t*>(dst + q) = 0xffffffffu;
-    for (; q < n; ++q) dst[q] = DASH;
-}
-
-__device__ __forceinline__ uint32_t load_u32_unaligned(const uint8_t* p) {
-    const uintptr_t A = (uintptr_t)p; const uint32_t* w = reinterpret_cast<const uint32_t*>(A & ~(uintptr_t)3);
-    return __funnelshift_r(w[0], w[1], (uint32_t)(A & 3) * 8);
-}
 template <int G>
-__device__ __forceinline__ int group_match(const uint8_t* a, const uint8_t* b, long n, int sub) {
+__device__ __forceinline__ int group_match(const uint32_t* a, int pa, const uint32_t* b, int pb, int n, int sub) {
     int mt = 0;
     #pragma unroll 2
-    for (long q = 4L * sub; q < n; q += 4L * G) {
-        const uint32_t x = load_u32_unaligned(a + q) ^ load_u32_unaligned(b + q);
-        uint32_t eq = ~(((x & 0x7f7f7f7fu) + 0x7f7f7f7fu) | x) & 0x80808080u;
-        if (n - q < 4) eq &= (1u << (8 * (n - q))) - 1u;
+    for (int q = 8 * sub; q < n; q += 8 * G) {
+        const uint32_t x = pk8(a, pa + q) ^ pk8(b, pb + q);
+        uint32_t eq = ~(((x & 0x77777777u) + 0x77777777u) | x) & 0x88888888u;
+        if (n - q < 8) eq &= (1u << (4 * (n - q))) - 1u;
         mt += __popc(eq);
     }
     return mt;
@@ -254,7 +207,7 @@
 };
 
 template <int G>
-__device__ __forceinline__ long segments_pass(const int* hi, const int* hj, int* hcl, int na, long c0, long j0, long L, const uint8_t* rd, const uint8_t* best, int tid, int nthr) {
+__device__ __forceinline__ long segments_pass(const int* hi, const int* hj, int* hcl, int na, long c0, long j0, long L, const uint32_t* rd, const uint32_t* best, int tid, int nthr) {
     const int PER = nthr / G; const int grp = tid / G, sub = tid % G; long span = 0;
     for (int mb = 1; mb < na; mb += PER) {
         const int m = mb + grp; const bool v = m < na;
@@ -263,21 +216,32 @@
         const long d = j - lj; long fwd_j = d; if (cs + fwd_j > L) fwd_j = L - cs;
         const bool el = v && i - li == fwd_j && fwd_j > 0;
         long nc = 0; if (el) { nc = L - 1 - li; if (nc > d) nc = d; if (nc < 0) nc = 0; }
-        const int mt = group_sum<G>(group_match<G>(rd + lj + 1, best + li + 1, nc, sub));
+        const int mt = group_sum<G>(group_match<G>(rd, (int)lj + 1, best, (int)li + 1, (int)nc, sub));
         int st = -1; bool second = false;
         if (el) { if (sub == 0) span += d; if (__ddiv_rn((double)mt, (double)d) >= 0.5) { if (cs == li && fwd_j == d && nc == d) st = mt; else second = true; } }
-        const int m2 = group_sum<G>(group_match<G>(rd + lj, best + cs, second ? fwd_j : 0, sub));
+        const int m2 = group_sum<G>(group_match<G>(rd, (int)lj, best, (int)cs, second ? (int)fwd_j : 0, sub));
         if (second) st = m2;
         if (v && sub == 0) hcl[m] = st;
     }
     return span;
 }
 
-struct Layout { uint8_t* best; uint8_t* oth; uint8_t* rows; uint8_t* acc; uint32_t Ls; };
+constexpr uint32_t DESC_DASHED = 0x80000000u;
+struct Layout { uint32_t* best; uint32_t* oth; uint4* desc; uint32_t* mask; uint8_t* acc; uint32_t mw; };
 __device__ __forceinline__ Layout cand_layout(const C& c, uint32_t ci, uint32_t L, uint32_t no) {
-    Layout y; y.best = c.scr + (size_t)c.scr_off[ci] * 16; y.oth = y.best + ((L + 7u) & ~7u);
-    y.rows = reinterpret_cast<uint8_t*>(((uintptr_t)(y.oth + c.plan_otot[ci]) + 3) & ~(uintptr_t)3); y.Ls = (L + 3u) & ~3u; y.acc = y.rows + (size_t)no * y.Ls;
+    Layout y; uint8_t* s = c.scr + (size_t)c.scr_off[ci] * 16;
+    y.best = reinterpret_cast<uint32_t*>(s); y.oth = reinterpret_cast<uint32_t*>(s + pk_bytes(L));
+    y.desc = reinterpret_cast<uint4*>(((uintptr_t)(s + pk_bytes(L) + c.plan_otot[ci]) + 15) & ~(uintptr_t)15);
+    y.mw = (L + 31u) / 32u; y.mask = reinterpret_cast<uint32_t*>(y.desc + no); y.acc = reinterpret_cast<uint8_t*>(y.mask + (size_t)no * y.mw);
     return y;
+}
+__device__ __forceinline__ void dash_bits(uint32_t* m, int a, int b) {
+    const int wa = a >> 5, wb = (b - 1) >> 5;
+    const uint32_t fa = ~0u << (a & 31), fb = ~0u >> (31 - ((b - 1) & 31));
+    atomicOr(&m[wa], wa == wb ? fa & fb : fa);
+    if (wa == wb) return;
+    for (int w = wa + 1; w < wb; ++w) m[w] = ~0u;
+    atomicOr(&m[wb], fb);
 }
 __device__ __forceinline__ uint8_t* cand_table(const C& c, uint32_t ci, uint32_t** keys, int** pos) {
     uint8_t* scr = c.scr + (size_t)c.scr_off[ci] * 16;
@@ -298,15 +262,15 @@
         const uint32_t L = c.alt_len[ci];
         if ((unsigned long long)c.alt_off[ci] + L > c.alt_cap || (unsigned long long)c.scr_off[ci] + c.scr_len[ci] > c.scr_cap16) { if (threadIdx.x == 0) atomicAdd(&c.ctr->scratch_overflow, 1ULL); continue; }
         const snfb_cand cd = c.cand[ci];
-        uint32_t* tk; int* tp; uint8_t* best = cand_table(c, ci, &tk, &tp);
-        unpack_lead(c, cd.lead_off + c.plan_best[ci], best, threadIdx.x, blockDim.x);
+        uint32_t* tk; int* tp; uint32_t* best = reinterpret_cast<uint32_t*>(cand_table(c, ci, &tk, &tp));
+        pack_lead(c, cd.lead_off + c.plan_best[ci], L, best, threadIdx.x, blockDim.x);
         const uint32_t no = c.plan_nother[ci];
-        if (no == 0 || L == 0) { __syncthreads(); uint8_t* out = c.alt + c.alt_off[ci]; for (uint32_t h = threadIdx.x; h < L; h += blockDim.x) out[h] = (uint8_t)CODE[best[h]]; continue; }
+        if (no == 0 || L == 0) { __syncthreads(); uint8_t* out = c.alt + c.alt_off[ci]; for (uint32_t h = threadIdx.x; h < L; h += blockDim.x) out[h] = (uint8_t)CODE[(best[h >> 3] >> (4 * (h & 7))) & 15u]; continue; }
         for (int i = threadIdx.x; i < TAB; i += blockDim.x) { tk[i] = 0xffffffffu; tp[i] = -1; }
         __syncthreads();
         const long skip = c.cfg.consensus_kmer_skip_base + (long)__dmul_rn((double)L, c.cfg.consensus_kmer_skip_seqlen_mult);
         for (long i = (long)threadIdx.x * skip; i < (long)L - 6; i += (long)blockDim.x * skip) {
-            const uint32_t key = kmer6_u(best + i); uint32_t s = kslot(key);
+            const uint32_t key = pk8(best, (int)i) & 0xffffffu; uint32_t s = kslot(key);
             for (;;) { const uint32_t old = atomicCAS(&tk[s], 0xffffffffu, key); if (old == 0xffffffffu || old == key) break; s = (s + 1) & (TAB - 1); }
             if (atomicCAS(&tp[s], -1, (int)i) != -1) tp[s] = -2;
         }
@@ -321,19 +285,19 @@
     const snfb_cand* cd = &c.cand[ci];
     uint32_t* t_key; int* t_pos; cand_table(c, ci, &t_key, &t_pos);
     const uint32_t no = c.plan_nother[ci];
-    const Layout y = cand_layout(c, ci, L, no);
-    uint8_t* best = y.best; uint8_t* acc = y.acc;
+    const uint32_t* best; uint32_t* rd;
+    { const Layout y = cand_layout(c, ci, L, no); best = y.best; rd = y.oth + it.rd_off / 4u; }
     const snfb_lead* l = &c.cand_leads[cd->lead_off + it.k];
-    const long Lo = l->seq_len; uint8_t* rd = y.oth + it.rd_off; uint8_t* row = y.rows + (size_t)it.row * y.Ls;
+    const long Lo = l->seq_len;
     const long skip = c.cfg.consensus_kmer_skip_base + (long)__dmul_rn((double)L, c.cfg.consensus_kmer_skip_seqlen_mult);
-    unpack_lead(c, cd->lead_off + it.k, rd, tid, NT);
+    pack_lead(c, cd->lead_off + it.k, (uint32_t)Lo, rd, tid, NT);
     g.sync();
     int nh = 0;
     const long nk = Lo - klen > 0 ? (Lo - klen + skip - 1) / skip : 0;
     for (long kb = 0; kb < nk; kb += 4 * NT) {
         uint32_t key[4], sl[4], tk[4]; int ai[4];
         #pragma unroll
-        for (int u = 0; u < 4; ++u) { const long kk = kb + u * NT + tid; key[u] = kk < nk ? kmer6_u(rd + kk * skip) : 0u; sl[u] = kslot(key[u]); }
+        for (int u = 0; u < 4; ++u) { const long kk = kb + u * NT + tid; key[u] = kk < nk ? pk8(rd, (int)(kk * skip)) & 0xffffffu : 0u; sl[u] = kslot(key[u]); }
         #pragma unroll
         for (int u = 0; u < 4; ++u) tk[u] = kb + u * NT + tid < nk ? t_key[sl[u]] : 0xffffffffu;
         #pragma unroll
@@ -390,35 +354,29 @@
     }
     {
         long cl = 0; if (na) { cl = c0 + hj[na - 1] - j0; if (cl > (long)L) cl = (long)L; }
-        const uint8_t* src0 = rd + (j0 - c0);
-        #pragma unroll 4
-        for (long X = 4L * tid; X < (long)L; X += 4L * NT) {
-            uint32_t v = 0xffffffffu;
-            if (X + 4 > c0 && X < cl) {
-                v = load_u32_unaligned(src0 + X);
-                if (X < c0) v |= (1u << (8 * (c0 - X))) - 1u;
-                if (X + 4 > cl) v |= ~((1u << (8 * (cl - X))) - 1u);
-            }
-            *reinterpret_cast<uint32_t*>(row + X) = v;
-        }
+        const Layout y = cand_layout(c, ci, L, no);
+        uint32_t* dm = y.mask + (size_t)it.row * y.mw;
+        for (uint32_t w = tid; w < y.mw; w += NT) dm[w] = 0u;
         g.sync();
+        long nd = 0;
         for (int m = 1 + tid; m < na; m += NT) {
             if (hcl[m] >= 0) continue;
             const long lj = hj[m - 1]; long cs = c0 + lj - j0; if (cs > (long)L) cs = (long)L;
             long len = hj[m] - lj; if (cs + len > (long)L) len = (long)L - cs;
-            if (len > 0) fill_dash(row + cs, len);
-        }
-    }
-    if (tid == 0) acc[it.row] = __ddiv_rn((double)span, (double)L) > 0.2;
+            if (len > 0) { dash_bits(dm, (int)cs, (int)(cs + len)); ++nd; }
+        }
+        nd = g.sum(nd);
+        if (tid == 0) { y.desc[it.row] = make_uint4(it.rd_off / 4u, (uint32_t)(j0 - c0), (uint32_t)c0 | (nd ? DESC_DASHED : 0u), (uint32_t)cl); y.acc[it.row] = __ddiv_rn((double)span, (double)L) > 0.2; }
+    }
     g.sync();
 }
 
 constexpr int ALIGN_WARPS = 4;
 __global__ void __launch_bounds__(ALIGN_WARPS * 32, 7) k_align(C c) {
-    __shared__ int sm[5][ALIGN_WARPS * MAXHIT_LIGHT]; __shared__ int s_red[2 * ALIGN_WARPS]; __shared__ uint32_t s_q;
+    __shared__ int sm[5][ALIGN_WARPS * MAXHIT_LIGHT]; __shared__ int s_red[2 * ALIGN_WARPS]; __shared__ uint32_t s_q, s_ns;
     static_assert(ALIGN_WARPS * MAXHIT_LIGHT >= MAXHIT, "a block item needs MAXHIT entries");
     const int lane = lane_id(), warp = threadIdx.x >> 5;
-    const uint32_t nb = (uint32_t)min((unsigned long long)c.work_ctr[4], c.item_cap), ns = (uint32_t)min((unsigned long long)c.work_ctr[5], c.item_cap);
+    const uint32_t nb = (uint32_t)min((unsigned long long)c.work_ctr[4], c.item_cap);
     for (;;) {
         __syncthreads();
         if (threadIdx.x == 0) s_q = atomicAdd(&c.work_ctr[6], 1u);
@@ -427,17 +385,33 @@
         BlockGrp<ALIGN_WARPS> g; g.tid = threadIdx.x; g.red = s_red;
         align_item(c, c.items_big[q], g, sm[0], sm[1], sm[2], sm[3], sm[4], ALIGN_WARPS * MAXHIT_LIGHT);
     }
+    if (threadIdx.x == 0) s_ns = (uint32_t)min((unsigned long long)c.work_ctr[5], c.item_cap);
     __syncthreads();
     for (;;) {
         uint32_t q = 0; if (lane == 0) q = atomicAdd(&c.work_ctr[7], 1u);
         q = __shfl_sync(FULL, q, 0);
-        if (q >= ns) break;
+        if (q >= s_ns) break;
         WarpGrp g; g.tid = lane; const int o = warp * MAXHIT_LIGHT;
         align_item(c, c.items_small[q], g, sm[0] + o, sm[1] + o, sm[2] + o, sm[3] + o, sm[4] + o, MAXHIT_LIGHT);
     }
 }
 
 constexpr int VOTE_LIST = 256;
+__device__ __forceinline__ uint32_t byte_mask4(uint32_t b) { return (((b & 15u) * 0x00204081u) & 0x01010101u) * 0xffu; }
+__device__ __forceinline__ uint2 row_word8(const uint32_t* oth, const uint4 d, const uint32_t* dm, uint32_t h) {
+    const uint32_t c0 = d.z & ~DESC_DASHED;
+    if (h + 8u <= c0 || h >= d.w) return make_uint2(0xffffffffu, 0xffffffffu);
+    const uint32_t x = pk8(oth + d.x, (int)h + (int)d.y);
+    const uint32_t lo = c0 > h ? c0 - h : 0u, hi = d.w - h < 8u ? d.w - h : 8u;
+    uint32_t km = ((1u << hi) - 1u) & ~((1u << lo) - 1u);
+    if (d.z & DESC_DASHED) km &= ~(dm[h >> 5] >> (h & 31u));
+    const uint32_t k0 = byte_mask4(km), k1 = byte_mask4(km >> 4);
+    return make_uint2((spread4(x & 0xffffu) & k0) | ~k0, (spread4(x >> 16) & k1) | ~k1);
+}
+__device__ __forceinline__ uint32_t row_word(const uint32_t* oth, const uint4 d, const uint32_t* dm, uint32_t h) {
+    const uint2 v = row_word8(oth, d, dm, h & ~7u);
+    return (h & 4u) ? v.y : v.x;
+}
 __device__ __forceinline__ void vote_add(unsigned long long (&cnt)[4], uint32_t code) {
     const unsigned long long inc = 1ull << (16 * (code & 3u)); const uint32_t sel = (code >> 2) & 3u;
     #pragma unroll
@@ -445,7 +419,7 @@
 }
 constexpr int VOTE_THREADS = 64;
 __global__ void __launch_bounds__(VOTE_THREADS) k_vote(C c) {
-    __shared__ uint2 s_tile; __shared__ int s_nacc, s_nlist; __shared__ uint16_t s_rows[VOTE_LIST];
+    __shared__ uint2 s_tile; __shared__ int s_nacc, s_nlist; __shared__ uint16_t s_rows[VOTE_LIST]; __shared__ uint4 s_desc[VOTE_LIST];
     static const char CODE[17] = "=ACMGRSVTWYHKDBN";
     for (;;) {
         __syncthreads();
@@ -455,11 +429,11 @@
         const uint32_t L = c.alt_len[ci], no = c.plan_nother[ci];
         if ((unsigned long long)c.alt_off[ci] + L > c.alt_cap || (unsigned long long)c.scr_off[ci] + c.scr_len[ci] > c.scr_cap16) continue;
         const Layout y = cand_layout(c, ci, L, no);
-        const uint8_t* best = y.best; const uint8_t* rows = y.rows; const uint8_t* acc = y.acc; const uint32_t Ls = y.Ls;
+        const uint32_t* best = y.best; const uint32_t* oth = y.oth; const uint8_t* acc = y.acc; const uint32_t mw = y.mw;
         if (threadIdx.x < 32) {
             int cnt = 0, extra = 0; const uint32_t lim = no < (uint32_t)VOTE_LIST ? no : (uint32_t)VOTE_LIST;
             for (uint32_t r0 = 0; r0 < lim; r0 += 32) { const uint32_t r = r0 + threadIdx.x; const bool a = r < lim && acc[r]; const unsigned bm = __ballot_sync(FULL, a);
-                if (a) s_rows[cnt + __popc(bm & lanemask_lt())] = (uint16_t)r; cnt += __popc(bm); }
+                if (a) { const int i = cnt + __popc(bm & lanemask_lt()); s_rows[i] = (uint16_t)r; s_desc[i] = y.desc[r]; } cnt += __popc(bm); }
             for (uint32_t r = lim + threadIdx.x; r < no; r += 32) extra += acc[r] ? 1 : 0;
             extra = (int)__reduce_add_sync(FULL, (unsigned)extra);
             if (threadIdx.x == 0) { s_nlist = cnt; s_nacc = cnt + extra; }
@@ -467,33 +441,42 @@
         __syncthreads();
         const double maxal = (double)(1 + s_nacc); const int nlist = s_nlist;
         uint8_t* out = c.alt + c.alt_off[ci];
-        const uint32_t h_end = min(L, (s_tile.y + 1u) * 4096u);
-        for (uint32_t h = s_tile.y * 4096u + threadIdx.x * 4u; h < h_end; h += blockDim.x * 4u) {
-            const uint32_t bw = *reinterpret_cast<const uint32_t*>(best + h);
+        const uint32_t h_end = min(L, (s_tile.y + 1u) * VOTE_TILE);
+        for (uint32_t h8 = s_tile.y * VOTE_TILE + threadIdx.x * 8u; h8 < h_end; h8 += blockDim.x * 8u) {
+            const uint32_t bx = best[h8 >> 3];
+            uint32_t done = 0;
             if (nlist == s_nacc && nlist < 255) {
-                uint32_t cA = 0, cC = 0, cG = 0, cT = 0, cD = 0, multi = 0;
+                uint32_t cA[2] = {0, 0}, cC[2] = {0, 0}, cG[2] = {0, 0}, cT[2] = {0, 0}, cD[2] = {0, 0}, multi[2] = {0, 0};
                 for (int r0 = 0; r0 < nlist; r0 += 8) {
-                    uint32_t cv[8];
+                    uint2 cv[8];
                     #pragma unroll
-                    for (int u = 0; u < 8; ++u) cv[u] = r0 + u < nlist ? *reinterpret_cast<const uint32_t*>(rows + (size_t)s_rows[r0 + u] * Ls + h) : 0xffffffffu;
+                    for (int u = 0; u < 8; ++u) cv[u] = r0 + u < nlist ? row_word8(oth, s_desc[r0 + u], y.mask + (size_t)s_rows[r0 + u] * mw, h8) : make_uint2(0xffffffffu, 0xffffffffu);
                     #pragma unroll
                     for (int u = 0; u < 8; ++u) {
-                        const uint32_t hb = cv[u] & 0x80808080u, d1 = hb >> 7, t = cv[u] & ~(hb | (hb - d1));
-                        cD += d1; multi |= ((t | 0x10101010u) - 0x01010101u) & t;
-                        cA += t & 0x01010101u; cC += (t >> 1) & 0x01010101u; cG += (t >> 2) & 0x01010101u; cT += (t >> 3) & 0x01010101u;
+                        #pragma unroll
+                        for (int b = 0; b < 2; ++b) {
+                            const uint32_t w = b ? cv[u].y : cv[u].x;
+                            const uint32_t hb = w & 0x80808080u, d1 = hb >> 7, t = w & ~(hb | (hb - d1));
+                            cD[b] += d1; multi[b] |= ((t | 0x10101010u) - 0x01010101u) & t;
+                            cA[b] += t & 0x01010101u; cC[b] += (t >> 1) & 0x01010101u; cG[b] += (t >> 2) & 0x01010101u; cT[b] += (t >> 3) & 0x01010101u;
+                        }
                     }
                 }
                 const uint32_t padded = (uint32_t)((nlist + 7) & ~7);
-                const uint32_t tot = cA + cC + cG + cT + cD;
-                const bool best_ok = (((bw | 0x10101010u) - 0x01010101u) & bw) == 0 && ((bw - 0x01010101u) & ~bw & 0x80808080u) == 0;
-                if (multi == 0 && best_ok && padded <= 248 && tot == padded * 0x01010101u) {
+                #pragma unroll
+                for (int b = 0; b < 2; ++b) {
+                    const uint32_t h = h8 + 4u * b; if (h >= h_end) break;
+                    const uint32_t bw = spread4((bx >> (16 * b)) & 0xffffu);
+                    const uint32_t tot = cA[b] + cC[b] + cG[b] + cT[b] + cD[b];
+                    const bool best_ok = (((bw | 0x10101010u) - 0x01010101u) & bw) == 0 && ((bw - 0x01010101u) & ~bw & 0x80808080u) == 0;
+                    if (!(multi[b] == 0 && best_ok && padded <= 248 && tot == padded * 0x01010101u)) continue;
                     #pragma unroll
                     for (int b2 = 0; b2 < 4; ++b2) {
                         if (h + b2 >= h_end) break;
                         const uint32_t bc = (bw >> (8 * b2)) & 255u; uint32_t res = bc;
-                        const int nal = (int)padded - (int)((cD >> (8 * b2)) & 255u);
+                        const int nal = (int)padded - (int)((cD[b] >> (8 * b2)) & 255u);
                         if (!(nal < 2 || __ddiv_rn((double)nal, maxal) < 0.25)) {
-                            int v4[4] = { (int)((cA >> (8 * b2)) & 255u), (int)((cC >> (8 * b2)) & 255u), (int)((cG >> (8 * b2)) & 255u), (int)((cT >> (8 * b2)) & 255u) };
+                            int v4[4] = { (int)((cA[b] >> (8 * b2)) & 255u), (int)((cC[b] >> (8 * b2)) & 255u), (int)((cG[b] >> (8 * b2)) & 255u), (int)((cT[b] >> (8 * b2)) & 255u) };
                             int t0 = -1, t1 = -1, c0 = 0, nd = 0;
                             #pragma unroll
                             for (int k = 0; k < 4; ++k) { const int v = v4[k] + ((bc >> k) & 1u); if (!v) continue; ++nd; if (v > t0) { t1 = t0; t0 = v; c0 = 1 << k; } else if (v > t1) t1 = v; }
@@ -501,42 +484,47 @@
                         }
                         out[h + b2] = (uint8_t)CODE[res];
                     }
-                    continue;
+                    done |= 1u << b;
                 }
             }
-            unsigned long long cnt[4][4]; int nal[4];
-            #pragma unroll
-            for (int b2 = 0; b2 < 4; ++b2) { nal[b2] = 0; cnt[b2][0] = cnt[b2][1] = cnt[b2][2] = cnt[b2][3] = 0; }
-            for (int r0 = 0; r0 < nlist; r0 += 8) {
-                uint32_t cv[8];
+            for (int b = 0; b < 2; ++b) {
+                const uint32_t h = h8 + 4u * b; if (h >= h_end) break;
+                if (done & (1u << b)) continue;
+                const uint32_t bw = spread4((bx >> (16 * b)) & 0xffffu);
+                unsigned long long cnt[4][4]; int nal[4];
                 #pragma unroll
-                for (int u = 0; u < 8; ++u) cv[u] = r0 + u < nlist ? *reinterpret_cast<const uint32_t*>(rows + (size_t)s_rows[r0 + u] * Ls + h) : 0xffffffffu;
+                for (int b2 = 0; b2 < 4; ++b2) { nal[b2] = 0; cnt[b2][0] = cnt[b2][1] = cnt[b2][2] = cnt[b2][3] = 0; }
+                for (int r0 = 0; r0 < nlist; r0 += 8) {
+                    uint32_t cv[8];
+                    #pragma unroll
+                    for (int u = 0; u < 8; ++u) cv[u] = r0 + u < nlist ? row_word(oth, s_desc[r0 + u], y.mask + (size_t)s_rows[r0 + u] * mw, h) : 0xffffffffu;
+                    #pragma unroll
+                    for (int u = 0; u < 8; ++u) {
+                        #pragma unroll
+                        for (int b2 = 0; b2 < 4; ++b2) { const uint32_t cc = (cv[u] >> (8 * b2)) & 255u; if (cc != DASH) { vote_add(cnt[b2], cc); ++nal[b2]; } }
+                    }
+                }
+                for (uint32_t r = VOTE_LIST; r < no; ++r) if (acc[r]) {
+                    const uint32_t v = row_word(oth, y.desc[r], y.mask + (size_t)r * mw, h);
+                    #pragma unroll
+                    for (int b2 = 0; b2 < 4; ++b2) { const uint32_t cc = (v >> (8 * b2)) & 255u; if (cc != DASH) { vote_add(cnt[b2], cc); ++nal[b2]; } }
+                }
                 #pragma unroll
-                for (int u = 0; u < 8; ++u) {
-                    #pragma unroll
-                    for (int b2 = 0; b2 < 4; ++b2) { const uint32_t cc = (cv[u] >> (8 * b2)) & 255u; if (cc != DASH) { vote_add(cnt[b2], cc); ++nal[b2]; } }
+                for (int b2 = 0; b2 < 4; ++b2) {
+                    if (h + b2 >= h_end) break;
+                    const uint32_t bc = (bw >> (8 * b2)) & 255u; uint32_t res = bc;
+                    if (!(nal[b2] < 2 || __ddiv_rn((double)nal[b2], maxal) < 0.25)) {
+                        vote_add(cnt[b2], bc);
+                        int t0 = -1, t1 = -1, c0 = 0, nd = 0;
+                        #pragma unroll
+                        for (int code = 0; code < 16; ++code) { const int v = (int)((cnt[b2][code >> 2] >> (16 * (code & 3))) & 0xffff); if (!v) continue; ++nd; if (v > t0) { t1 = t0; t0 = v; c0 = code; } else if (v > t1) t1 = v; }
+                        if (nd > 1 && t0 - t1 >= 3) res = (uint32_t)c0;
+                    }
+                    out[h + b2] = (uint8_t)CODE[res];
                 }
             }
-            for (uint32_t r = VOTE_LIST; r < no; ++r) if (acc[r]) {
-                const uint32_t v = *reinterpret_cast<const uint32_t*>(rows + (size_t)r * Ls + h);
-                #pragma unroll
-                for (int b2 = 0; b2 < 4; ++b2) { const uint32_t cc = (v >> (8 * b2)) & 255u; if (cc != DASH) { vote_add(cnt[b2], cc); ++nal[b2]; } }
-            }
-            #pragma unroll
-            for (int b2 = 0; b2 < 4; ++b2) {
-                if (h + b2 >= h_end) break;
-                const uint32_t bc = (bw >> (8 * b2)) & 255u; uint32_t res = bc;
-                if (!(nal[b2] < 2 || __ddiv_rn((double)nal[b2], maxal) < 0.25)) {
-                    vote_add(cnt[b2], bc);
-                    int t0 = -1, t1 = -1, c0 = 0, nd = 0;
-                    #pragma unroll
-                    for (int code = 0; code < 16; ++code) { const int v = (int)((cnt[b2][code >> 2] >> (16 * (code & 3))) & 0xffff); if (!v) continue; ++nd; if (v > t0) { t1 = t0; t0 = v; c0 = code; } else if (v > t1) t1 = v; }
-                    if (nd > 1 && t0 - t1 >= 3) res = (uint32_t)c0;
-                }
-                out[h + b2] = (uint8_t)CODE[res];
-            }
-        }
-    }
-}
-
-}
+        }
+    }
+}
+
+}
```

After: 9981, median of 6. 1.02x the previous value.
